# ali-vilab/VGen

Measured on AMD Instinct MI355X. Metric: denoise_steps_per_sec, higher is better.
Workload: dtype fp16

## Files before the change

### include/vgen_hip.h

```cpp
#ifndef VGEN_HIP_H
#define VGEN_HIP_H

#include <stddef.h>
#include <stdint.h>

#ifdef __cplusplus
extern "C" {
#endif

#define VGEN_ABI_VERSION 7

enum { VGEN_BF16 = 0, VGEN_F16 = 1, VGEN_F32 = 2 };

enum {
  VGEN_E_BADARG = -1,
  VGEN_E_UNSUPPORTED = -2,
  VGEN_E_WORKSPACE = -3
};

int vgen_version(void);
const char* vgen_last_error(void);

size_t vgen_groupnorm_ws_bytes(int64_t nb, int64_t S);
int vgen_groupnorm(const float* x1, int32_t C1, const float* x2, int32_t C2,
                   int64_t nb, int64_t S, int32_t groups, float eps,
                   const float* gamma, const float* beta, int32_t silu,
                   void* y, void* raw, int32_t raw_split, int32_t dtype,
                   float* ws, size_t ws_bytes, void* stream);

int vgen_groupnorm_cs(const float* x1, int32_t C1, const float* cs1,
                      const float* x2, int32_t C2, const float* cs2,
                      int64_t nb, int64_t S, int32_t groups, float eps,
                      const float* gamma, const float* beta, int32_t silu,
                      void* y, void* raw, int32_t raw_split, int32_t dtype,
                      float* ws, size_t ws_bytes, void* stream);

int vgen_embed_tokens(const int64_t* tokens, int64_t rows, int32_t L, int32_t d, int32_t vocab,
                      const float* table, const float* pos, float* out, void* stream);

int vgen_layernorm(const float* x, int64_t M, int32_t d, float eps,
                   const float* gamma, const float* beta,
                   void* y, int32_t dtype, void* stream);

enum { VGEN_TAP_LINEAR = 0, VGEN_TAP_CONV3X3 = 1, VGEN_TAP_TEMPORAL3 = 2 };
enum { VGEN_EPI_NONE = 0, VGEN_EPI_GEGLU = 1 };

typedef struct vgen_tapgemm_args {
  int64_t M;
  int32_t N;
  int32_t dtype;
  const void* A;
  int64_t lda;
  int32_t C1;
  int32_t taps;
  int32_t mode;
  int32_t Hi, Wi, Ho, Wo, stride, pad_t, pad_l, ups;
  int32_t F;
  int64_t S;
  const void* A2;
  int64_t lda2;
  int32_t C2;
  const void* W;
  int64_t ldw;
  const float* bias;
  const float* rowbias;
  int64_t rowbias_ld;
  int64_t rows_per_rb;
  const float* residual;
  int64_t ldr;
  void* out;
  int64_t ldo;
  int32_t out_dtype;
  int32_t epilogue;
  void* ws;
  size_t ws_bytes;
  int32_t crop_t;
  float* colstats;
  int32_t dualw;
  int32_t split_out;
} vgen_tapgemm_args;

size_t vgen_tapgemm_ws_bytes(const vgen_tapgemm_args* args);
int vgen_tapgemm(const vgen_tapgemm_args* args, void* stream);

int vgen_tapgemm_query_plan(const vgen_tapgemm_args* args, int32_t* out3);
int vgen_tapgemm_set_plans(const int64_t* rows, int32_t n);

typedef struct vgen_attn_args {
  const void* q;
  const void* k;
  const void* v;
  void* out;
  int32_t dtype;
  int32_t heads;
  int32_t nq, nk;
  int64_t nbatch;
  int64_t inner;
  int64_t q_rs, q_bo, q_bi;
  int64_t k_rs, k_bo, k_bi;
  int64_t v_rs, v_bo, v_bi;
  int64_t o_rs, o_bo, o_bi;
  float scale;
  int32_t causal;
} vgen_attn_args;

int vgen_attention(const vgen_attn_args* args, void* stream);

int vgen_attention_d80(const vgen_attn_args* args, void* stream);

int vgen_softmax_rows(const float* S, int64_t rows, int32_t cols, int64_t lds, float scale,
                      void* P, int64_t ldp, int32_t dtype, void* stream);


int vgen_act_cast(const float* x, void* y, int64_t n, int32_t act, int32_t dtype, void* stream);

int vgen_cast_split(const float* x, int64_t M, int32_t C, int64_t ldx, void* out, int64_t ldo, int32_t lo_off,
                    int32_t dtype, void* stream);

int vgen_timestep_embedding(const float* t, int32_t B, int32_t dim, void* out, int32_t dtype,
                            void* stream);

int vgen_linear_f32(const float* x, int32_t n, int32_t K, const float* W, const float* bias, int32_t N,
                    int32_t act_in, const float* add, float* out, void* stream);

int vgen_im2col3x3_small(const float* src, int64_t nimg, int32_t Fi, int32_t Cin, int32_t H,
                         int32_t W, int64_t s_bo, int64_t s_fi, int64_t s_c, int64_t s_y,
                         int64_t s_x, void* out, int32_t Kpad, int32_t dtype, int32_t split, void* stream);

int vgen_pointwise_small(const float* src, int64_t nimg, int32_t Fi, int32_t Cin, int32_t H,
                         int32_t W, int64_t s_bo, int64_t s_fi, int64_t s_c, int64_t s_y,
                         int64_t s_x, const float* Wm, const float* b, int32_t Cout, float* dst,
                         int64_t d_bo, int64_t d_fi, int64_t d_c, int64_t d_y, int64_t d_x,
                         void* stream);

int vgen_cfg_ddim_step(const float* xt, const float* y, const float* u, const float* noise,
                       const float* coef, float guide, int32_t use_guide, int32_t mean_type,
                       int64_t B, int64_t per_b, float* xt_1, float* x0_out, void* stream);

int vgen_cfg_ddim_step_units(const float* xt, int64_t xt_bstride, const float* y, const float* u,
                             const float* noise, const float* coef, const int64_t* t_idx, float guide,
                             int32_t use_guide, int32_t mean_type, int64_t B, int64_t per_b, float* xt_1,
                             float* x0_out, float* rep, int32_t nrep, int64_t rep_gstride,
                             int64_t rep_bstride, void* stream);

int vgen_gaussian_sample(const float* moments, const float* noise, int64_t nimg, int32_t zc,
                         int64_t HW, float scale, float* z, void* stream);

int vgen_lowfreq_filter(const float* x, int64_t nimg, int32_t H, int32_t W, int32_t C, float scale,
                        float* y, float* ws, size_t ws_bytes, void* stream);
int vgen_scale_channels(float* x, int64_t M, int32_t C, int32_t c0, int32_t c1, float s, void* stream);

int vgen_patchify(const float* x, int64_t B, int32_t C, int32_t H, int32_t W, int32_t P, int32_t Kpad, int32_t cls,
                  void* out, int32_t dtype, void* stream);

int vgen_conv3x3_small(const float* x, int64_t n, int32_t Cin, int32_t H, int32_t W, const float* w,
                       const float* b, int32_t Cout, int32_t stride, int32_t act, float* y, void* stream);
int vgen_adaptive_avgpool2d(const float* x, int64_t planes, int32_t H, int32_t W, int32_t Ho, int32_t Wo,
                            float* y, void* stream);
int vgen_frame_transformer(const float* x, int64_t B, int32_t F, int32_t d, int64_t HW, int32_t heads,
                           int32_t dim_head, int32_t hidden, const float* ln_w, const float* ln_b,
                           const float* wqkv, const float* wout, const float* bout, const float* w1,
                           const float* b1, const float* w2, const float* b2, float* y, int32_t last,
                           float out_scale, int32_t accumulate, void* stream);

int vgen_frames_u8(const float* x, int64_t rows, int32_t C, int64_t ldx, const float* mean,
                   const float* stdv, void* out, void* stream);

int vgen_adapter(const float* x, int64_t ldx, int64_t M, int32_t d, int32_t h, int32_t hp, const void* Wd,
                 const void* Wu, const float* bu, const float* hb, int64_t ldhb, int64_t rows_per_hb, float* out,
                 int64_t ldo, int32_t dtype, void* stream);

int vgen_sketch_stem(const float* x, int64_t n, int32_t H, int32_t W, int32_t flip, float mean, float stdv,
                     const float* w, const float* b, void* out, int64_t ldo, int32_t dtype, void* stream);
int vgen_relu_shuffle16(const void* in, int64_t ldi, int64_t M, int32_t C, int32_t g, int32_t Hin, int32_t Win,
                        void* out, int64_t ldo, int32_t dtype, void* stream);
int vgen_sketch_head(const void* a, int64_t lda, int64_t n, int32_t H, int32_t W, int32_t C, const float* w,
                     float bias, int32_t flip, float* out, int32_t dtype, void* stream);

int vgen_dwconv_relu(const float* x, int64_t ldx, int64_t n, int32_t H, int32_t W, int32_t Cp, const float* w,
                     int32_t k, int32_t pool, float* xp, void* xp16, void* y, int32_t dtype, void* stream);
int vgen_cdcm_head(const void* t, int64_t ldt, int64_t n, int32_t H, int32_t W, const void* Wd, const float* Wa,
                   const float* ba, const float* wr, float* out, int64_t ldo, int32_t dtype, void* stream);
int vgen_pidinet_emap(const float* mr, int64_t ld, int64_t n, int32_t H, int32_t W, const float* w2, float br,
                      float* e, void* stream);
int vgen_pidinet_fuse(const float* e0, const float* e1, const float* e2, const float* e3, int64_t n, int32_t H,
                      int32_t W, float wc0, float wc1, float wc2, float wc3, float bc, float* out, void* stream);

int vgen_repeat_rows(const void* src, int64_t bytes, int32_t G, void* dst, void* stream);
int vgen_gather_rows_f32(const float* table, int64_t nrows_table, int64_t cols, const int64_t* idx, int64_t rows,
                         float* out, void* stream);

size_t vgen_cfg_stats_ws_bytes(int64_t B);
int vgen_cfg_stats(const float* y, const float* u, float guide, int32_t use_guide, int64_t B,
                   int64_t per_b, float* out, void* ws, size_t ws_bytes, void* stream);
int vgen_gauss_x0(const float* xt, const float* out, const void* ws, float rescale, const float* coef,
                  int32_t pred_type, int64_t B, int64_t per_b, float* x0, float* eps, void* stream);
int vgen_lincomb4(const float* a, const float* b, const float* c, const float* d, float ca, float cb,
                  float cc, float cd, float* out, int64_t n, void* stream);
int vgen_dpmpp2m_sde_step(const float* x, const float* denoised, const float* old_denoised, const float* noise,
                          float ca, float cb, float cc, float cn1, float cn2, float cn3, float* out, int64_t n,
                          void* stream);

#ifdef __cplusplus
}
#endif
#endif
```

### vgen_amd/csrc/norms.hip

```cpp
#include "common.h"
#include <stdlib.h>
#include <type_traits>

namespace {

constexpr int GN_THREADS = 256;
constexpr int GN_MAX_SLOTS = 3;
constexpr int GN_G = 32;

struct GnGeom {
  int C, C1, C2;
  int nslots;
  int tpr;
  int rpb;
  int spt;
  int cpg;
};

__device__ __forceinline__ GnGeom gn_geom(int C1, int C2, int groups) {
  GnGeom g;
  g.C1 = C1;
  g.C2 = C2;
  g.C = C1 + C2;
  g.nslots = g.C >> 2;
  if (g.nslots <= GN_THREADS) {
    g.tpr = g.nslots;
    g.rpb = GN_THREADS / g.nslots;
    g.spt = 1;
  } else {
    g.tpr = GN_THREADS;
    g.rpb = 1;
    g.spt = (g.nslots + GN_THREADS - 1) / GN_THREADS;
  }
  g.cpg = g.C / groups;
  return g;
}

__device__ __forceinline__ f32x4 gn_load(const float* x1, const float* x2, const GnGeom& g,
                                         int64_t row, int c) {
  if (c < g.C1) return *(const f32x4*)(x1 + row * g.C1 + c);
  return *(const f32x4*)(x2 + row * g.C2 + (c - g.C1));
}

__global__ __launch_bounds__(GN_THREADS) void gn_stats_kernel(
    const float* __restrict__ x1, int C1, const float* __restrict__ x2, int C2, int64_t S,
    int groups, int nsplit, float* __restrict__ part) {
  __shared__ float red[2][3072];
  const GnGeom g = gn_geom(C1, C2, groups);
  const int tid = threadIdx.x;
  const int split = blockIdx.x;
  const int64_t nb = blockIdx.y;
  const int64_t rows_per = (S + nsplit - 1) / nsplit;
  const int64_t r_begin = (int64_t)split * rows_per;
  const int64_t r_end = min(S, r_begin + rows_per);
  const int nrows = r_end > r_begin ? (int)(r_end - r_begin) : 0;
  const int rowlane = tid / g.tpr;
  const int slot0 = tid - rowlane * g.tpr;

  if (rowlane < g.rpb) {
    const int cnt = nrows > rowlane ? (nrows - rowlane + g.rpb - 1) / g.rpb : 0;
    f32x4 s[GN_MAX_SLOTS], ss[GN_MAX_SLOTS], pv[GN_MAX_SLOTS];
#pragma unroll
    for (int k = 0; k < GN_MAX_SLOTS; ++k) {
      s[k] = f32x4{0, 0, 0, 0};
      ss[k] = f32x4{0, 0, 0, 0};
      pv[k] = f32x4{0, 0, 0, 0};
    }
    bool first = true;
#pragma unroll 4
    for (int64_t r = r_begin + rowlane; r < r_end; r += g.rpb) {
      const int64_t row = nb * S + r;
#pragma unroll
      for (int k = 0; k < GN_MAX_SLOTS; ++k) {
        const int slot = slot0 + k * GN_THREADS;
        if (k < g.spt && slot < g.nslots) {
          const f32x4 x = gn_load(x1, x2, g, row, slot * 4);
          if (first) pv[k] = x;
          const f32x4 v = x - pv[k];
          s[k] += v;
          ss[k] += v * v;
        }
      }
      first = false;
    }
    const float inv = cnt > 0 ? 1.0f / (float)cnt : 0.f;
#pragma unroll
    for (int k = 0; k < GN_MAX_SLOTS; ++k) {
      const int slot = slot0 + k * GN_THREADS;
      if (k < g.spt && slot < g.nslots) {
        const int o = rowlane * g.C + slot * 4;
        const f32x4 dm = s[k] * inv;
        f32x4 m2 = ss[k] - s[k] * dm;
#pragma unroll
        for (int e = 0; e < 4; ++e) m2[e] = fmaxf(m2[e], 0.f);
        *(f32x4*)&red[0][o] = pv[k] + dm;
        *(f32x4*)&red[1][o] = m2;
      }
    }
  }
  __syncthreads();
  if (tid < groups) {
    const float n = (float)nrows * (float)g.cpg;
    float mean = 0.f, m2 = 0.f;
    if (nrows > 0) {
      const float ref = red[0][tid * g.cpg];
      float a = 0.f;
      for (int rl = 0; rl < g.rpb; ++rl) {
        const float cnt = nrows > rl ? (float)((nrows - rl + g.rpb - 1) / g.rpb) : 0.f;
        const int o = rl * g.C + tid * g.cpg;
        float t = 0.f;
        for (int c = 0; c < g.cpg; ++c) t += red[0][o + c] - ref;
        a += cnt * t;
      }
      mean = ref + a / n;
      for (int rl = 0; rl < g.rpb; ++rl) {
        const float cnt = nrows > rl ? (float)((nrows - rl + g.rpb - 1) / g.rpb) : 0.f;
        const int o = rl * g.C + tid * g.cpg;
        float t = 0.f, q = 0.f;
        for (int c = 0; c < g.cpg; ++c) {
          const float d = red[0][o + c] - mean;
          t += d * d;
          q += red[1][o + c];
        }
        m2 += q + cnt * t;
      }
    }
    float* o = part + ((nb * nsplit + split) * groups + tid) * 3;
    o[0] = n;
    o[1] = mean;
    o[2] = m2;
  }
}

__global__ __launch_bounds__(64) void gn_finalize_kernel(const float* __restrict__ part,
                                                         int groups, int nsplit, float eps, int C,
                                                         const float* __restrict__ gamma,
                                                         const float* __restrict__ beta,
                                                         float* __restrict__ stat) {
  const int lane = threadIdx.x;
  const int grp = blockIdx.x;
  const int64_t nb = blockIdx.y;
  float n = 0.f, mean = 0.f, m2 = 0.f;
  for (int sp = lane; sp < nsplit; sp += 64) {
    const float* p = part + ((nb * nsplit + sp) * groups + grp) * 3;
    const float nb_ = p[0], mb = p[1], m2b = p[2];
    if (nb_ > 0.f) {
      const float nt = n + nb_;
      const float d = mb - mean;
      mean += d * (nb_ / nt);
      m2 += m2b + d * d * (n * nb_ / nt);
      n = nt;
    }
  }
#pragma unroll
  for (int o = 1; o < 64; o <<= 1) {
    const float n2 = __shfl_xor(n, o, 64), mean2 = __shfl_xor(mean, o, 64),
                m22 = __shfl_xor(m2, o, 64);
    const float nt = n + n2;
    if (nt > 0.f) {
      const float lo_n = (lane & o) ? n2 : n, hi_n = (lane & o) ? n : n2;
      const float lo_m = (lane & o) ? mean2 : mean, hi_m = (lane & o) ? mean : mean2;
      const float d = hi_m - lo_m;
      const float w = hi_n / nt;
      m2 = m2 + m22 + d * d * (lo_n * w);
      mean = lo_m + d * w;
    }
    n = nt;
  }
  const float rstd = 1.0f / sqrtf((n > 0.f ? m2 / n : 0.f) + eps);
  const int cpg = C / groups;
  for (int j = lane; j < cpg; j += 64) {
    const int c = grp * cpg + j;
    const float a = gamma[c] * rstd;
    stat[(nb * C + c) * 2 + 0] = a;
    stat[(nb * C + c) * 2 + 1] = beta[c] - mean * a;
  }
}

__device__ __forceinline__ void chan_merge(float& n, float& mean, float& m2, float nb_, float mb, float m2b) {
  const float nt = n + nb_;
  if (nt > 0.f) {
    const float d = mb - mean;
    const float w = nb_ / nt;
    m2 = m2 + m2b + d * d * (n * w);
    mean = mean + d * w;
  }
  n = nt;
}

constexpr float GN_CS_GUARD = 128.f;

template <int NT>
__global__ __launch_bounds__(NT) void gn_finalize_cs_kernel(const float* __restrict__ cs1, int C1,
                                                             const float* __restrict__ cs2, int C2,
                                                             const float* __restrict__ x1, const float* __restrict__ x2,
                                                             int64_t S, int groups, float eps,
                                                             const float* __restrict__ gamma,
                                                             const float* __restrict__ beta,
                                                             float* __restrict__ stat) {
  constexpr int NW = NT / 64;
  __shared__ float red[NW][3];
  __shared__ float mr[3];
  const int tid = threadIdx.x, lane = tid & 63, w = tid >> 6;
  const int grp = blockIdx.x;
  const int64_t nb = blockIdx.y;
  const int cpg = (C1 + C2) / groups;
  const int slabs = (int)(S / 64);
  const int items = slabs * cpg;
  const int64_t srow0 = nb * slabs;
  float n = 0.f, mean = 0.f, m2 = 0.f;
  auto fetch = [&](int it, float& sm, float& sq) __attribute__((always_inline)) {
    const int sl = it / cpg;
    const int c = grp * cpg + (it - sl * cpg);
    const int64_t srow = srow0 + sl;
    if (c < C1) {
      sm = cs1[(srow * 2) * C1 + c];
      sq = cs1[(srow * 2 + 1) * C1 + c];
    } else {
      sm = cs2[(srow * 2) * C2 + (c - C1)];
      sq = cs2[(srow * 2 + 1) * C2 + (c - C1)];
    }
  };
  int it = tid;
  for (; it + 3 * NT < items; it += 4 * NT) {
    float sm[4], sq[4];
#pragma unroll
    for (int u = 0; u < 4; ++u) fetch(it + u * NT, sm[u], sq[u]);
#pragma unroll
    for (int u = 0; u < 4; ++u) {
      const float mb = sm[u] * (1.0f / 64.f);
      chan_merge(n, mean, m2, 64.f, mb, fmaxf(sq[u] - sm[u] * mb, 0.f));
    }
  }
  for (; it < items; it += NT) {
    float sm, sq;
    fetch(it, sm, sq);
    const float mb = sm * (1.0f / 64.f);
    chan_merge(n, mean, m2, 64.f, mb, fmaxf(sq - sm * mb, 0.f));
  }
#pragma unroll
  for (int o = 1; o < 64; o <<= 1) {
    const float n2 = __shfl_xor(n, o, 64), mean2 = __shfl_xor(mean, o, 64),
                m22 = __shfl_xor(m2, o, 64);
    const float nt = n + n2;
    if (nt > 0.f) {
      const float lo_n = (lane & o) ? n2 : n, hi_n = (lane & o) ? n : n2;
      const float lo_m = (lane & o) ? mean2 : mean, hi_m = (lane & o) ? mean : mean2;
      const float d = hi_m - lo_m;
      const float wgt = hi_n / nt;
      m2 = m2 + m22 + d * d * (lo_n * wgt);
      mean = lo_m + d * wgt;
    }
    n = nt;
  }
  if (lane == 0) {
    red[w][0] = n;
    red[w][1] = mean;
    red[w][2] = m2;
  }
  __syncthreads();
  if (tid == 0) {
    float N = red[0][0], M = red[0][1], Q = red[0][2];
    for (int k = 1; k < NW; ++k) chan_merge(N, M, Q, red[k][0], red[k][1], red[k][2]);
    const float var = N > 0.f ? Q / N : 0.f;
    mr[0] = M;
    mr[1] = 1.0f / sqrtf(var + eps);
    mr[2] = N * M * M > GN_CS_GUARD * Q ? 1.f : 0.f;
  }
  __syncthreads();
  if (mr[2] != 0.f) {
    const float M = mr[0];
    const int64_t tot = S * cpg;
    float d = 0.f, q = 0.f;
    for (int64_t i = tid; i < tot; i += NT) {
      const int64_t r = i / cpg;
      const int c = grp * cpg + (int)(i - r * cpg);
      const int64_t row = nb * S + r;
      const float e = (c < C1 ? x1[row * C1 + c] : x2[row * C2 + (c - C1)]) - M;
      d += e;
      q += e * e;
    }
#pragma unroll
    for (int o = 1; o < 64; o <<= 1) {
      d += __shfl_xor(d, o, 64);
      q += __shfl_xor(q, o, 64);
    }
    __syncthreads();
    if (lane == 0) {
      red[w][0] = d;
      red[w][1] = q;
    }
    __syncthreads();
    if (tid == 0) {
      float D = red[0][0], Q = red[0][1];
      for (int k = 1; k < NW; ++k) {
        D += red[k][0];
        Q += red[k][1];
      }
      const float nf = (float)tot;
      const float dm = D / nf;
      mr[0] = M + dm;
      mr[1] = 1.0f / sqrtf(fmaxf(Q - D * dm, 0.f) / nf + eps);
    }
    __syncthreads();
  }
  const int C = C1 + C2;
  for (int j = tid; j < cpg; j += NT) {
    const int c = grp * cpg + j;
    const float a = gamma[c] * mr[1];
    stat[(nb * C + c) * 2 + 0] = a;
    stat[(nb * C + c) * 2 + 1] = beta[c] - mr[0] * a;
  }
}

template <typename T>
__device__ __forceinline__ void store_raw4(uint16_t* raw, int64_t off, int raw_lo, const f32x4& v) {
  const u32x2 h = pack4<T>(v.x, v.y, v.z, v.w);
  *(u32x2*)(raw + off) = h;
  if (raw_lo > 0) {
    *(u32x2*)(raw + off + raw_lo) =
        pack4<T>(v.x - T::to_f32((uint16_t)(h.x & 0xffffu)), v.y - T::to_f32((uint16_t)(h.x >> 16)),
                 v.z - T::to_f32((uint16_t)(h.y & 0xffffu)), v.w - T::to_f32((uint16_t)(h.y >> 16)));
  }
}
template <typename T>
__device__ __forceinline__ void store_raw2(uint16_t* raw, int64_t off, int raw_lo, float a, float b) {
  const uint32_t h = T::pack2(a, b);
  *(uint32_t*)(raw + off) = h;
  if (raw_lo > 0) *(uint32_t*)(raw + off + raw_lo) = T::pack2(a - T::to_f32((uint16_t)(h & 0xffffu)), b - T::to_f32((uint16_t)(h >> 16)));
}

template <typename T>
__global__ __launch_bounds__(GN_THREADS) void gn_apply_kernel(
    const float* __restrict__ x1, int C1, const float* __restrict__ x2, int C2, int64_t S,
    int groups, int nsplit, const float* __restrict__ stat, const float* __restrict__ gamma,
    const float* __restrict__ beta, int silu, uint16_t* __restrict__ y,
    uint16_t* __restrict__ raw, int raw_lo) {
  const GnGeom g = gn_geom(C1, C2, groups);
  const int raw_ld = raw_lo > 0 ? 2 * g.C : g.C;
  const int tid = threadIdx.x;
  const int split = blockIdx.x;
  const int64_t nb = blockIdx.y;
  const int64_t rows_per = (S + nsplit - 1) / nsplit;
  const int64_t r_begin = (int64_t)split * rows_per;
  const int64_t r_end = min(S, r_begin + rows_per);
  const int rowlane = tid / g.tpr;
  const int slot0 = tid - rowlane * g.tpr;
  if (rowlane >= g.rpb) return;

  f32x4 sc[GN_MAX_SLOTS], sh[GN_MAX_SLOTS];
#pragma unroll
  for (int k = 0; k < GN_MAX_SLOTS; ++k) {
    const int slot = slot0 + k * GN_THREADS;
    if (k < g.spt && slot < g.nslots) {
      const f32x4 p0 = *(const f32x4*)(stat + (nb * g.C + slot * 4) * 2);
      const f32x4 p1 = *(const f32x4*)(stat + (nb * g.C + slot * 4) * 2 + 4);
      sc[k] = f32x4{p0.x, p0.z, p1.x, p1.z};
      sh[k] = f32x4{p0.y, p0.w, p1.y, p1.w};
    }
  }
  if (g.spt == 1) {
    constexpr int U = 4;
    const int c = slot0 * 4;
    const bool from1 = c < g.C1;
    const float* src = from1 ? x1 + c : x2 + (c - g.C1);
    const int64_t ld = from1 ? g.C1 : g.C2;
    f32x4 cur[U], nxt[U];
    int64_t r = r_begin + rowlane;
    auto load = [&](int64_t r0, f32x4* dst) __attribute__((always_inline)) {
#pragma unroll
      for (int u = 0; u < U; ++u) {
        const int64_t rr = r0 + (int64_t)u * g.rpb;
        const int64_t row = nb * S + (rr < r_end ? rr : r_end - 1);
        dst[u] = *(const f32x4*)(src + row * ld);
      }
    };
    if (r < r_end) load(r, nxt);
    for (; r < r_end; r += (int64_t)U * g.rpb) {
#pragma unroll
      for (int u = 0; u < U; ++u) cur[u] = nxt[u];
      if (r + (int64_t)U * g.rpb < r_end) load(r + (int64_t)U * g.rpb, nxt);
#pragma unroll
      for (int u = 0; u < U; ++u) {
        const int64_t rr = r + (int64_t)u * g.rpb;
        if (rr < r_end) {
          const int64_t row = nb * S + rr;
          f32x4 o = cur[u] * sc[0] + sh[0];
          if (silu) {
#pragma unroll
            for (int e = 0; e < 4; ++e) o[e] = silu_f(o[e]);
          }
          *(u32x2*)(y + row * g.C + c) = pack4<T>(o.x, o.y, o.z, o.w);
          if (raw) store_raw4<T>(raw, row * raw_ld + c, raw_lo, cur[u]);
        }
      }
    }
    return;
  }
#pragma unroll 4
  for (int64_t r = r_begin + rowlane; r < r_end; r += g.rpb) {
    const int64_t row = nb * S + r;
#pragma unroll
    for (int k = 0; k < GN_MAX_SLOTS; ++k) {
      const int slot = slot0 + k * GN_THREADS;
      if (k < g.spt && slot < g.nslots) {
        const f32x4 v = gn_load(x1, x2, g, row, slot * 4);
        f32x4 o = v * sc[k] + sh[k];
        if (silu) {
#pragma unroll
          for (int e = 0; e < 4; ++e) o[e] = silu_f(o[e]);
        }
        *(u32x2*)(y + row * g.C + slot * 4) = pack4<T>(o.x, o.y, o.z, o.w);
        if (raw) store_raw4<T>(raw, row * raw_ld + slot * 4, raw_lo, v);
      }
    }
  }
}

constexpr int GNF_THREADS = 512;
constexpr int GNF_LDS_FLOATS = 24576;

__device__ __forceinline__ float gnf_block_sum(float v, float* red) {
  v = wave_sum(v);
  const int lane = threadIdx.x & 63, w = threadIdx.x >> 6;
  __syncthreads();
  if (lane == 0) red[w] = v;
  __syncthreads();
  float t = 0.f;
#pragma unroll
  for (int i = 0; i < GNF_THREADS / 64; ++i) t += red[i];
  return t;
}

template <typename T>
__global__ __launch_bounds__(GNF_THREADS) void gn_fused_kernel(
    const float* __restrict__ x1, int C1, const float* __restrict__ x2, int C2, int64_t S, int groups,
    float eps, const float* __restrict__ gamma, const float* __restrict__ beta, int silu,
    uint16_t* __restrict__ y, uint16_t* __restrict__ raw, int raw_lo) {
  extern __shared__ __attribute__((aligned(16))) float gnf_stage[];
  __shared__ float red[GNF_THREADS / 64];
  const int C = C1 + C2;
  const int cpg = C / groups;
  const int I = cpg >> 1;
  const int rpi = GNF_THREADS / I;
  const int tid = threadIdx.x;
  const int r0 = tid / I;
  const int i = tid - r0 * I;
  const bool active = r0 < rpi;
  const int c = blockIdx.x * cpg + 2 * i;
  const int64_t row0 = (int64_t)blockIdx.y * S;
  const bool from1 = c < C1;
  const float* src = from1 ? x1 + row0 * C1 + c : x2 + row0 * C2 + (c - C1);
  const int64_t lds = from1 ? C1 : C2;
  const int nit = active ? (int)((S - r0 + rpi - 1) / rpi) : 0;
  f32x2* const st = (f32x2*)gnf_stage + r0 * I + i;
  const int sstep = rpi * I;

  float a = 0.f;
  {
    const float* p = src + (int64_t)r0 * lds;
    const int64_t step = (int64_t)rpi * lds;
#pragma unroll 8
    for (int k = 0; k < nit; ++k) {
      const f32x2 v = *(const f32x2*)(p + k * step);
      st[k * sstep] = v;
      a += v.x + v.y;
    }
  }
  const float n = (float)S * (float)cpg;
  const float mean = gnf_block_sum(a, red) / n;
  float q = 0.f;
  for (int k = 0; k < nit; ++k) {
    const f32x2 v = st[k * sstep];
    const float d0 = v.x - mean, d1 = v.y - mean;
    q += d0 * d0 + d1 * d1;
  }
  const float rstd = 1.0f / sqrtf(gnf_block_sum(q, red) / n + eps);
  if (!active) return;
  const float sc0 = gamma[c] * rstd, sc1 = gamma[c + 1] * rstd;
  const float sh0 = beta[c] - mean * sc0, sh1 = beta[c + 1] - mean * sc1;
  const int raw_ld = raw_lo > 0 ? 2 * C : C;
  uint16_t* yo = y + (row0 + r0) * C + c;
  uint16_t* ro = raw ? raw + (row0 + r0) * raw_ld + c : nullptr;
  const int64_t ostep = (int64_t)rpi * C, rstep = (int64_t)rpi * raw_ld;
#pragma unroll 4
  for (int k = 0; k < nit; ++k) {
    const f32x2 v = st[k * sstep];
    float o0 = v.x * sc0 + sh0, o1 = v.y * sc1 + sh1;
    if (silu) {
      o0 = silu_f(o0);
      o1 = silu_f(o1);
    }
    *(uint32_t*)(yo + k * ostep) = T::pack2(o0, o1);
    if (ro) store_raw2<T>(ro, k * rstep, raw_lo, v.x, v.y);
  }
}

constexpr int GNR_THREADS = 1024;
constexpr int GNR_NIT = 36;

__device__ __forceinline__ float gnr_block_sum(float v, float* red) {
  v = wave_sum(v);
  const int lane = threadIdx.x & 63, w = threadIdx.x >> 6;
  __syncthreads();
  if (lane == 0) red[w] = v;
  __syncthreads();
  float t = 0.f;
#pragma unroll
  for (int i = 0; i < GNR_THREADS / 64; ++i) t += red[i];
  return t;
}

template <typename T>
__global__ __launch_bounds__(GNR_THREADS) void gn_regs_kernel(
    const float* __restrict__ x1, int C1, const float* __restrict__ x2, int C2, int64_t S, int groups,
    float eps, const float* __restrict__ gamma, const float* __restrict__ beta, int silu,
    uint16_t* __restrict__ y, uint16_t* __restrict__ raw, int raw_lo) {
  __shared__ float red[GNR_THREADS / 64];
  const int C = C1 + C2;
  const int cpg = C / groups;
  const int I = cpg >> 1;
  const int rpi = GNR_THREADS / I;
  const int tid = threadIdx.x;
  const int r0 = tid / I;
  const int i = tid - r0 * I;
  const bool active = r0 < rpi;
  const int c = blockIdx.x * cpg + 2 * i;
  const int64_t row0 = (int64_t)blockIdx.y * S;
  const bool from1 = c < C1;
  const float* src = from1 ? x1 + row0 * C1 + c : x2 + row0 * C2 + (c - C1);
  const int64_t lds = from1 ? C1 : C2;
  const int nit = active ? (int)((S - r0 + rpi - 1) / rpi) : 0;

  f32x2 v[GNR_NIT];
  float a = 0.f;
  {
    const float* p = src + (int64_t)r0 * lds;
    const int64_t step = (int64_t)rpi * lds;
#pragma unroll
    for (int k = 0; k < GNR_NIT; ++k) {
      v[k] = f32x2{0.f, 0.f};
      if (k < nit) v[k] = *(const f32x2*)(p + k * step);
    }
#pragma unroll
    for (int k = 0; k < GNR_NIT; ++k) a += v[k].x + v[k].y;
  }
  const float n = (float)S * (float)cpg;
  const float mean = gnr_block_sum(a, red) / n;
  float q = 0.f;
#pragma unroll
  for (int k = 0; k < GNR_NIT; ++k) {
    if (k < nit) {
      const float d0 = v[k].x - mean, d1 = v[k].y - mean;
      q += d0 * d0 + d1 * d1;
    }
  }
  const float rstd = 1.0f / sqrtf(gnr_block_sum(q, red) / n + eps);
  if (!active) return;
  const float sc0 = gamma[c] * rstd, sc1 = gamma[c + 1] * rstd;
  const float sh0 = beta[c] - mean * sc0, sh1 = beta[c + 1] - mean * sc1;
  const int raw_ld = raw_lo > 0 ? 2 * C : C;
  uint16_t* yo = y + (row0 + r0) * C + c;
  uint16_t* ro = raw ? raw + (row0 + r0) * raw_ld + c : nullptr;
  const int64_t ostep = (int64_t)rpi * C, rstep = (int64_t)rpi * raw_ld;
#pragma unroll
  for (int k = 0; k < GNR_NIT; ++k) {
    if (k < nit) {
      float o0 = v[k].x * sc0 + sh0, o1 = v[k].y * sc1 + sh1;
      if (silu) {
        o0 = silu_f(o0);
        o1 = silu_f(o1);
      }
      *(uint32_t*)(yo + k * ostep) = T::pack2(o0, o1);
      if (ro) store_raw2<T>(ro, k * rstep, raw_lo, v[k].x, v[k].y);
    }
  }
}

int gn_nsplit(int64_t nb, int64_t S, int C) {
  int64_t rows = 16384 / C;
  if (rows < 2) rows = 2;
  int64_t ns = (S + rows - 1) / rows;
  const int64_t want = (1024 + nb - 1) / nb;
  if (ns < want) ns = want;
  const int64_t cap = (S + 1) / 2;
  if (ns > cap) ns = cap;
  if (ns < 1) ns = 1;
  if (ns > 1024) ns = 1024;
  return (int)ns;
}

constexpr int LN_MAX_SLOTS = 8;

template <typename T, int LPR>
__global__ __launch_bounds__(256) void layernorm_kernel(const float* __restrict__ x, int64_t M,
                                                        int d, float eps,
                                                        const float* __restrict__ gamma,
                                                        const float* __restrict__ beta,
                                                        void* __restrict__ y) {
  constexpr int RPB = 256 / LPR;
  const int sub = threadIdx.x % LPR;
  const int64_t row = (int64_t)blockIdx.x * RPB + threadIdx.x / LPR;
  const bool live = row < M;
  const int nslots = d >> 2;
  const float* xr = x + (live ? row : 0) * d;
  f32x4 v[LN_MAX_SLOTS];
  float s = 0.f;
#pragma unroll
  for (int k = 0; k < LN_MAX_SLOTS; ++k) {
    const int slot = sub + LPR * k;
    v[k] = f32x4{0, 0, 0, 0};
    if (slot < nslots) {
      v[k] = *(const f32x4*)(xr + slot * 4);
      s += (v[k].x + v[k].y) + (v[k].z + v[k].w);
    }
  }
#pragma unroll
  for (int o = LPR / 2; o > 0; o >>= 1) s += __shfl_xor(s, o, 64);
  const float mean = s / (float)d;
  float q = 0.f;
#pragma unroll
  for (int k = 0; k < LN_MAX_SLOTS; ++k) {
    const int slot = sub + LPR * k;
    if (slot < nslots) {
      const f32x4 c = v[k] - mean;
      q += (c.x * c.x + c.y * c.y) + (c.z * c.z + c.w * c.w);
    }
  }
#pragma unroll
  for (int o = LPR / 2; o > 0; o >>= 1) q += __shfl_xor(q, o, 64);
  const float rstd = 1.0f / sqrtf(q / (float)d + eps);
  if (!live) return;
#pragma unroll
  for (int k = 0; k < LN_MAX_SLOTS; ++k) {
    const int slot = sub + LPR * k;
    if (slot < nslots) {
      const f32x4 ga = *(const f32x4*)(gamma + slot * 4);
      const f32x4 be = *(const f32x4*)(beta + slot * 4);
      const f32x4 o = (v[k] - mean) * rstd * ga + be;
      if constexpr (std::is_same<T, F32Out>::value) {
        *(f32x4*)((float*)y + row * d + slot * 4) = o;
      } else {
        *(u32x2*)((uint16_t*)y + row * d + slot * 4) = pack4<T>(o.x, o.y, o.z, o.w);
      }
    }
  }
}

template <typename T, int LPR, int NS>
__global__ __launch_bounds__(256) void layernorm_stream_kernel(const float* __restrict__ x, int64_t M,
                                                               float eps, const float* __restrict__ gamma,
                                                               const float* __restrict__ beta,
                                                               uint16_t* __restrict__ y) {
  constexpr int RPB = 256 / LPR;
  constexpr int D = NS * 4 * LPR;
  const int sub = threadIdx.x % LPR;
  const int rl = threadIdx.x / LPR;
  const int64_t ngroups = (M + RPB - 1) / RPB;
  f32x4 ga[NS], be[NS], v[NS], nx[NS];
#pragma unroll
  for (int k = 0; k < NS; ++k) {
    ga[k] = *(const f32x4*)(gamma + (sub + LPR * k) * 4);
    be[k] = *(const f32x4*)(beta + (sub + LPR * k) * 4);
  }
  int64_t g = blockIdx.x;
  auto load = [&](int64_t grp, f32x4* dst) __attribute__((always_inline)) {
    const int64_t row = grp * RPB + rl;
    const float* xr = x + (row < M ? row : M - 1) * D;
#pragma unroll
    for (int k = 0; k < NS; ++k) dst[k] = *(const f32x4*)(xr + (sub + LPR * k) * 4);
  };
  if (g < ngroups) load(g, nx);
  for (; g < ngroups; g += gridDim.x) {
#pragma unroll
    for (int k = 0; k < NS; ++k) v[k] = nx[k];
    if (g + gridDim.x < ngroups) load(g + gridDim.x, nx);
    float s = 0.f;
#pragma unroll
    for (int k = 0; k < NS; ++k) s += (v[k].x + v[k].y) + (v[k].z + v[k].w);
#pragma unroll
    for (int o = LPR / 2; o > 0; o >>= 1) s += __shfl_xor(s, o, 64);
    const float mean = s / (float)D;
    float q = 0.f;
#pragma unroll
    for (int k = 0; k < NS; ++k) {
      const f32x4 c = v[k] - mean;
      q += (c.x * c.x + c.y * c.y) + (c.z * c.z + c.w * c.w);
    }
#pragma unroll
    for (int o = LPR / 2; o > 0; o >>= 1) q += __shfl_xor(q, o, 64);
    const float rstd = 1.0f / sqrtf(q / (float)D + eps);
    const int64_t row = g * RPB + rl;
    if (row < M) {
      uint16_t* yr = y + row * D;
#pragma unroll
      for (int k = 0; k < NS; ++k) {
        const f32x4 o = (v[k] - mean) * rstd * ga[k] + be[k];
        *(u32x2*)(yr + (sub + LPR * k) * 4) = pack4<T>(o.x, o.y, o.z, o.w);
      }
    }
  }
}

template <typename T, int LPR, int NS>
void launch_ln_stream(const float* x, int64_t M, float eps, const float* gamma, const float* beta,
                      uint16_t* y, hipStream_t s) {
  const int64_t ngroups = (M + 256 / LPR - 1) / (256 / LPR);
  const int64_t grid = ngroups < 2048 ? ngroups : 2048;
  hipLaunchKernelGGL((layernorm_stream_kernel<T, LPR, NS>), dim3((unsigned)grid), dim3(256), 0, s, x, M, eps,
                     gamma, beta, y);
}

template <typename T, int LPR>
void launch_ln(const float* x, int64_t M, int d, float eps, const float* gamma, const float* beta,
               void* y, hipStream_t s) {
  const int64_t grid = (M + 256 / LPR - 1) / (256 / LPR);
  hipLaunchKernelGGL((layernorm_kernel<T, LPR>), dim3((unsigned)grid), dim3(256), 0, s, x, M, d, eps,
                     gamma, beta, y);
}

template <typename T>
void dispatch_ln(const float* x, int64_t M, int d, float eps, const float* gamma, const float* beta,
                 uint16_t* y, hipStream_t s) {
  switch (d) {
    case 320: return launch_ln_stream<T, 16, 5>(x, M, eps, gamma, beta, y, s);
    case 512: return launch_ln_stream<T, 16, 8>(x, M, eps, gamma, beta, y, s);
    case 640: return launch_ln_stream<T, 32, 5>(x, M, eps, gamma, beta, y, s);
    case 1024: return launch_ln_stream<T, 32, 8>(x, M, eps, gamma, beta, y, s);
    case 1280: return launch_ln_stream<T, 64, 5>(x, M, eps, gamma, beta, y, s);
    case 2048: return launch_ln_stream<T, 64, 8>(x, M, eps, gamma, beta, y, s);
    default: break;
  }
  if (d <= 512) launch_ln<T, 16>(x, M, d, eps, gamma, beta, y, s);
  else if (d <= 1024) launch_ln<T, 32>(x, M, d, eps, gamma, beta, y, s);
  else launch_ln<T, 64>(x, M, d, eps, gamma, beta, y, s);
}

}

extern "C" size_t vgen_groupnorm_ws_bytes(int64_t nb, int64_t S) {
  const int ns = 1024;
  return (size_t)(nb * ns * GN_G * 3 + nb * 3072 * 2) * sizeof(float);
}

static int groupnorm_impl(const float* x1, int32_t C1, const float* cs1, const float* x2, int32_t C2,
                          const float* cs2, int64_t nb, int64_t S, int32_t groups, float eps,
                          const float* gamma, const float* beta, int32_t silu, void* y,
                          void* raw, int32_t raw_split, int32_t dtype, float* ws, size_t ws_bytes,
                          void* stream) {
  const int C = C1 + C2;
  const int raw_lo = (raw != nullptr && raw_split) ? C : 0;
  VGEN_REQUIRE(dtype == VGEN_BF16 || dtype == VGEN_F16, "groupnorm: dtype");
  VGEN_REQUIRE(groups > 0 && groups <= GN_G && C % groups == 0, "groupnorm: C=%d groups=%d", C,
               groups);
  VGEN_REQUIRE(C1 > 0 && C1 % 4 == 0 && C2 >= 0 && C2 % 4 == 0 && C <= 3072,
               "groupnorm: C1=%d C2=%d (need %%4, total <= 3072)", C1, C2);
  VGEN_REQUIRE(C2 == 0 || x2 != nullptr, "groupnorm: x2 null with C2 > 0");
  VGEN_REQUIRE(vgen_aligned16(x1) && vgen_aligned16(x2) && vgen_aligned16(y) &&
                   vgen_aligned16(raw) && vgen_aligned16(ws),
               "groupnorm: alignment");
  VGEN_REQUIRE(nb > 0 && S > 0 && nb <= 65535, "groupnorm: nb=%lld S=%lld", (long long)nb,
               (long long)S);
  if (ws_bytes < vgen_groupnorm_ws_bytes(nb, S)) {
    vgen_set_error("groupnorm: workspace %zu < %zu", ws_bytes, vgen_groupnorm_ws_bytes(nb, S));
    return VGEN_E_WORKSPACE;
  }
  hipStream_t s = (hipStream_t)stream;
  {
    static const int env_max = getenv("VGEN_GN_FUSED_MAX_MB") ? atoi(getenv("VGEN_GN_FUSED_MAX_MB")) : -1;
    const int64_t fused_max = (int64_t)(env_max >= 0 ? env_max : (C / groups >= 16 ? 96 : 24)) << 20;
    const int cpg = C / groups;
    if (nb * S * C * 4 <= fused_max && cpg % 2 == 0 && C1 % 2 == 0 && cpg / 2 <= GNF_THREADS && S * cpg <= GNF_LDS_FLOATS) {
      const size_t lds = (size_t)S * cpg * sizeof(float);
      static bool done_bf16[VGEN_MAX_DEVICES] = {false}, done_f16[VGEN_MAX_DEVICES] = {false};
      if (vgen_lds_optin((const void*)gn_fused_kernel<BF16>, GNF_LDS_FLOATS * 4, done_bf16, "groupnorm") ||
          vgen_lds_optin((const void*)gn_fused_kernel<F16>, GNF_LDS_FLOATS * 4, done_f16, "groupnorm"))
        return VGEN_E_BADARG;
      dim3 fgrid((unsigned)groups, (unsigned)nb);
      if (dtype == VGEN_BF16) {
        hipLaunchKernelGGL(gn_fused_kernel<BF16>, fgrid, dim3(GNF_THREADS), lds, s, x1, C1, x2, C2, S, groups, eps,
                           gamma, beta, silu, (uint16_t*)y, (uint16_t*)raw, raw_lo);
      } else {
        hipLaunchKernelGGL(gn_fused_kernel<F16>, fgrid, dim3(GNF_THREADS), lds, s, x1, C1, x2, C2, S, groups, eps,
                           gamma, beta, silu, (uint16_t*)y, (uint16_t*)raw, raw_lo);
      }
      return vgen_check_launch("gn_fused");
    }
  }
  {
    static const int regs_on = getenv("VGEN_GN_REGS") ? atoi(getenv("VGEN_GN_REGS")) : 1;
    const int cpg = C / groups;
    const int I = cpg / 2;
    if (regs_on && cs1 == nullptr && cpg % 2 == 0 && C1 % 2 == 0 && I > 0 && I <= GNR_THREADS &&
        (S + (GNR_THREADS / I) - 1) / (GNR_THREADS / I) <= GNR_NIT && nb * groups <= 1024 && S * cpg > GNF_LDS_FLOATS) {
      dim3 fgrid((unsigned)groups, (unsigned)nb);
      if (dtype == VGEN_BF16) {
        hipLaunchKernelGGL(gn_regs_kernel<BF16>, fgrid, dim3(GNR_THREADS), 0, s, x1, C1, x2, C2, S, groups, eps, gamma, beta,
                           silu, (uint16_t*)y, (uint16_t*)raw, raw_lo);
      } else {
        hipLaunchKernelGGL(gn_regs_kernel<F16>, fgrid, dim3(GNR_THREADS), 0, s, x1, C1, x2, C2, S, groups, eps, gamma, beta,
                           silu, (uint16_t*)y, (uint16_t*)raw, raw_lo);
      }
      return vgen_check_launch("gn_regs");
    }
  }
  const int nslots = C / 4;
  const int rpb = nslots <= GN_THREADS ? GN_THREADS / nslots : 1;
  VGEN_REQUIRE(rpb * C <= 3072, "groupnorm: internal LDS bound");
  const int ns = gn_nsplit(nb, S, C);
  float* part = ws;
  float* stat = ws + nb * ns * GN_G * 3;
  dim3 grid((unsigned)ns, (unsigned)nb);
  int rc;
  if (cs1 != nullptr) {
    if ((S / 64) * (C / groups) > 2048) {
      hipLaunchKernelGGL(gn_finalize_cs_kernel<1024>, dim3((unsigned)groups, (unsigned)nb), dim3(1024), 0, s, cs1, C1,
                         cs2, C2, x1, x2, S, groups, eps, gamma, beta, stat);
    } else {
      hipLaunchKernelGGL(gn_finalize_cs_kernel<256>, dim3((unsigned)groups, (unsigned)nb), dim3(256), 0, s, cs1, C1,
                         cs2, C2, x1, x2, S, groups, eps, gamma, beta, stat);
    }
    rc = vgen_check_launch("gn_finalize_cs");
    if (rc) return rc;
  } else {
    hipLaunchKernelGGL(gn_stats_kernel, grid, dim3(GN_THREADS), 0, s, x1, C1, x2, C2, S, groups, ns,
                       part);
    rc = vgen_check_launch("gn_stats");
    if (rc) return rc;
    hipLaunchKernelGGL(gn_finalize_kernel, dim3((unsigned)groups, (unsigned)nb), dim3(64), 0, s, part,
                       groups, ns, eps, C, gamma, beta, stat);
    rc = vgen_check_launch("gn_finalize");
    if (rc) return rc;
  }
  if (dtype == VGEN_BF16) {
    hipLaunchKernelGGL(gn_apply_kernel<BF16>, grid, dim3(GN_THREADS), 0, s, x1, C1, x2, C2, S,
                       groups, ns, stat, gamma, beta, silu, (uint16_t*)y, (uint16_t*)raw, raw_lo);
  } else {
    hipLaunchKernelGGL(gn_apply_kernel<F16>, grid, dim3(GN_THREADS), 0, s, x1, C1, x2, C2, S,
                       groups, ns, stat, gamma, beta, silu, (uint16_t*)y, (uint16_t*)raw, raw_lo);
  }
  return vgen_check_launch("gn_apply");
}

extern "C" int vgen_groupnorm(const float* x1, int32_t C1, const float* x2, int32_t C2,
                              int64_t nb, int64_t S, int32_t groups, float eps,
                              const float* gamma, const float* beta, int32_t silu, void* y,
                              void* raw, int32_t raw_split, int32_t dtype, float* ws, size_t ws_bytes,
                              void* stream) {
  return groupnorm_impl(x1, C1, nullptr, x2, C2, nullptr, nb, S, groups, eps, gamma, beta, silu, y, raw, raw_split,
                        dtype, ws, ws_bytes, stream);
}

extern "C" int vgen_groupnorm_cs(const float* x1, int32_t C1, const float* cs1, const float* x2,
                                 int32_t C2, const float* cs2, int64_t nb, int64_t S, int32_t groups,
                                 float eps, const float* gamma, const float* beta, int32_t silu,
                                 void* y, void* raw, int32_t raw_split, int32_t dtype, float* ws, size_t ws_bytes,
                                 void* stream) {
  VGEN_REQUIRE(cs1 != nullptr && (C2 == 0 || cs2 != nullptr), "groupnorm_cs: missing column statistics");
  VGEN_REQUIRE(S % 64 == 0, "groupnorm_cs: S=%lld must be a multiple of the 64-row slab", (long long)S);
  return groupnorm_impl(x1, C1, cs1, x2, C2, cs2, nb, S, groups, eps, gamma, beta, silu, y, raw, raw_split, dtype,
                        ws, ws_bytes, stream);
}

extern "C" int vgen_layernorm(const float* x, int64_t M, int32_t d, float eps, const float* gamma,
                              const float* beta, void* y, int32_t dtype, void* stream) {
  VGEN_REQUIRE(dtype == VGEN_BF16 || dtype == VGEN_F16 || dtype == VGEN_F32, "layernorm: dtype");
  VGEN_REQUIRE(d > 0 && d % 4 == 0 && d <= 64 * 4 * LN_MAX_SLOTS, "layernorm: d=%d", d);
  VGEN_REQUIRE(vgen_aligned16(x) && vgen_aligned16(y) && vgen_aligned16(gamma) &&
                   vgen_aligned16(beta),
               "layernorm: alignment");
  if (M <= 0) return 0;
  VGEN_REQUIRE(M < (1LL << 32), "layernorm: M too large");
  hipStream_t s = (hipStream_t)stream;
  if (dtype == VGEN_F32) {
    if (d <= 512) launch_ln<F32Out, 16>(x, M, d, eps, gamma, beta, y, s);
    else if (d <= 1024) launch_ln<F32Out, 32>(x, M, d, eps, gamma, beta, y, s);
    else launch_ln<F32Out, 64>(x, M, d, eps, gamma, beta, y, s);
    return vgen_check_launch("layernorm");
  }
  if (dtype == VGEN_BF16) dispatch_ln<BF16>(x, M, d, eps, gamma, beta, (uint16_t*)y, s);
  else dispatch_ln<F16>(x, M, d, eps, gamma, beta, (uint16_t*)y, s);
  return vgen_check_launch("layernorm");
}
```

### vgen_amd/csrc/tapgemm.hip

```cpp
#include "common.h"
#include "tapgemm_plan.h"
#include <stdio.h>
#include <stdlib.h>
#include <type_traits>

int vgen_panel_launch(const vgen_tapgemm_args& a, hipStream_t s);

namespace {

struct RowState {
  int base;
  int a;
  int b;
};

constexpr int INVALID = -(1 << 24);

__device__ __attribute__((aligned(128))) unsigned char g_zeros[ZERO_BYTES];

typedef const __attribute__((address_space(1))) void* gptr_t;
typedef __attribute__((address_space(3))) void* lptr_t;


__device__ __forceinline__ void glds16(const void* src, unsigned char* lds_wave_base) {
  __builtin_amdgcn_global_load_lds((gptr_t)src, (lptr_t)lds_wave_base, 16, 0, 0);
}


template <int N>
__device__ __forceinline__ void wait_vmcnt() {
  asm volatile("s_waitcnt vmcnt(%0)" ::"n"(N) : "memory");
}

template <int CPR>
__device__ __forceinline__ int swz_key(int row) {
  if constexpr (CPR == 8) {
    return row & 7;
  } else {
    const int q = (row >> 2) & 3;
    return (4 - q) & 3;
  }
}

#ifdef VGEN_TUNING
#define VGEN_ABLATE_ARG(x) (x)
#else
#define VGEN_ABLATE_ARG(x) 0
#endif

template <typename T, int BM, int BN, int BK, int WM, int WN, int STAGES, bool PP, bool DW>
__global__ __launch_bounds__(WM* WN * 64, (WM * WN == 4) ? 2 : 1) void tapgemm_kernel(
    const vgen_tapgemm_args p, const int splitk, float* __restrict__ ws, const int ablate_arg, const int stagger,
    const int first_round) {
  static_assert(!PP || (WM * WN == 8 && STAGES == 3), "ping-pong needs 8 waves and a 3-stage ring");
  static_assert(!DW || (PP && BK == 64), "dual-W K-steps are built on the ping-pong schedule, 64-element K-tiles");
  const int ablate = VGEN_ABLATE_ARG(ablate_arg);
  constexpr int WPA = DW ? 2 : 1;
  constexpr int NT = WM * WN * 64;
  constexpr int ROW_BYTES = BK * 2;
  constexpr int CPR = ROW_BYTES / 16;
  constexpr int RPI = 64 / CPR;
  constexpr int RPP = NT / CPR;
  constexpr int KS = BK / 32;
  constexpr int WTM = BM / WM, WTN = BN / WN;
  constexpr int MF = WTM / 16, NF = WTN / 16;
  constexpr int RA = BM / RPP;
  constexpr int RBF = BN / RPP;
  constexpr int RBT = BN % RPP;
  constexpr int STAGE_BYTES = (BM + BN) * ROW_BYTES;
  constexpr int LPT = RA + RBF;
  static_assert(BM % RPP == 0 && RBT % RPI == 0, "tile rows must split into whole DMA instructions");

  extern __shared__ __attribute__((aligned(16))) unsigned char smem[];

  const int tid = threadIdx.x;
  const int lane = tid & 63;
  const int wave = __builtin_amdgcn_readfirstlane(tid >> 6);
  const int wm = wave / WN;
  const int wn = wave % WN;
  const int lr = lane & 15;
  const int lq = lane >> 4;
  const bool w_tail = RBT > 0 && wave * RPI < RBT;

  if (stagger > 0 && (int)(blockIdx.x + gridDim.x * blockIdx.y) < first_round && wave == 0) {
    const unsigned hw = __builtin_amdgcn_s_getreg((3 << 11) | ((WM * WN == 8 ? 8 : 0) << 6) | 4);
    if (hw & 1u)
      for (int i = 0; i < stagger; ++i) __builtin_amdgcn_s_sleep(16);
  }

  const int tiles_n = (p.N + BN - 1) / BN;
  int64_t tile;
  {
    const unsigned nwg = gridDim.x, bid = blockIdx.x;
    const unsigned xcd = bid & 7u, q = nwg >> 3, r = nwg & 7u;
    tile = (xcd < r ? xcd * (q + 1) : r * (q + 1) + (xcd - r) * q) + (bid >> 3);
  }
  const int64_t m0 = (tile / tiles_n) * BM;
  const int n0 = (int)(tile % tiles_n) * BN;
  const int64_t lm0 = (ablate & 8) ? 0 : m0;
  const int ln0 = (ablate & 8) ? 0 : n0;

  const uint16_t* __restrict__ A = (const uint16_t*)p.A;
  const uint16_t* __restrict__ A2 = (const uint16_t*)p.A2;
  const uint16_t* __restrict__ W = (const uint16_t*)p.W;
  const int64_t ldw = p.ldw ? p.ldw : ((int64_t)p.taps * p.C1 + p.C2) * WPA;

  const int ld_c = tid % CPR;
  const int ld_r = tid / CPR;

  RowState rs[RA];
  unsigned mvalid = 0;
#pragma unroll
  for (int i = 0; i < RA; ++i) {
    const unsigned m = (unsigned)lm0 + ld_r + RPP * i;
    const bool ok = m < (unsigned)p.M;
    if (ok) mvalid |= 1u << i;
    if (p.mode == VGEN_TAP_CONV3X3) {
      const unsigned hw = p.Ho * p.Wo;
      const unsigned img = m / hw;
      const unsigned rem = m - img * hw;
      const unsigned oy = rem / (unsigned)p.Wo;
      const unsigned ox = rem - oy * p.Wo;
      rs[i].base = img * p.Hi * p.Wi;
      rs[i].a = ok ? (int)oy * p.stride - p.pad_t : INVALID;
      rs[i].b = (int)ox * p.stride - p.pad_l;
    } else if (p.mode == VGEN_TAP_TEMPORAL3) {
      const unsigned fs = m / (unsigned)p.S;
      rs[i].base = (int)m;
      rs[i].a = ok ? (int)(fs % (unsigned)p.F) : INVALID;
      rs[i].b = 0;
    } else {
      rs[i].base = ok ? (int)m : -1;
      rs[i].a = 0;
      rs[i].b = 0;
    }
  }

  const int cpt1 = p.C1 / BK;
  const int T1 = p.taps * cpt1;
  const int KT = T1 + p.C2 / BK;
  const int split = blockIdx.y;
  const int kt_begin = (int)(((int64_t)KT * split) / splitk);
  const int kt_end = (int)(((int64_t)KT * (split + 1)) / splitk);
  const int nk = (ablate & 1) ? 0 : (kt_end - kt_begin) * WPA;

  constexpr int NP = LPT + (RBT > 0 ? 1 : 0);
  const char* pc[NP];
  const char* const zline = (const char*)g_zeros;
  const int src_cb = (ld_c ^ swz_key<CPR>(ld_r)) * 16;
  const int wave_row0 = wave * RPI;
  int kt_next = kt_begin;
  int left;

  const unsigned lda_b = (unsigned)p.lda * 2u, lda2_b = (unsigned)p.lda2 * 2u;
  const char* const zl = zline + src_cb;
  auto gather_a = [&](int kt) __attribute__((always_inline)) {
    if (kt < T1) {
      const int tap = kt / cpt1;
      const int cch = kt - tap * cpt1;
      left = cpt1 - cch;
      const char* const a_cb = (const char*)A + (cch * BK * 2 + src_cb);
      if (p.mode == VGEN_TAP_CONV3X3) {
        const int d0 = tap / 3, d1 = tap - 3 * d0;
        const unsigned Hv = (unsigned)((p.Hi << p.ups) - 2 * p.crop_t), Wv = (unsigned)(p.Wi << p.ups);
#pragma unroll
        for (int i = 0; i < RA; ++i) {
          const int iy = rs[i].a + d0, ix = rs[i].b + d1;
          const bool ok = ((unsigned)iy < Hv) & ((unsigned)ix < Wv);
          const unsigned row = (unsigned)rs[i].base + (unsigned)((iy + p.crop_t) >> p.ups) * (unsigned)p.Wi + (unsigned)(ix >> p.ups);
          const char* const real = a_cb + (uint64_t)row * lda_b;
          pc[i] = ok ? real : zl;
        }
      } else if (p.mode == VGEN_TAP_TEMPORAL3) {
        const int dt_ = tap - 1;
#pragma unroll
        for (int i = 0; i < RA; ++i) {
          const bool ok = (unsigned)(rs[i].a + dt_) < (unsigned)p.F;
          const unsigned row = (unsigned)(rs[i].base + dt_ * p.S);
          const char* const real = a_cb + (uint64_t)row * lda_b;
          pc[i] = ok ? real : zl;
        }
      } else {
#pragma unroll
        for (int i = 0; i < RA; ++i) {
          const bool ok = rs[i].base >= 0;
          const char* const real = a_cb + (uint64_t)(unsigned)rs[i].base * lda_b;
          pc[i] = ok ? real : zl;
        }
      }
    } else {
      left = KT - kt + 1;
      const char* const a_cb = (const char*)A2 + ((kt - T1) * BK * 2 + src_cb);
#pragma unroll
      for (int i = 0; i < RA; ++i) {
        const bool ok = (mvalid >> i) & 1u;
        const char* const real = a_cb + (uint64_t)((unsigned)lm0 + ld_r + RPP * i) * lda2_b;
        pc[i] = ok ? real : zl;
      }
    }
  };
  gather_a(kt_begin);
#pragma unroll
  for (int i = 0; i < NP - RA; ++i) {
    const int n = ln0 + ld_r + RPP * i;
    const bool ok = n < p.N;
    pc[RA + i] = (ok ? (const char*)(W + (int64_t)n * ldw + (int64_t)kt_begin * WPA * BK) : zline) + src_cb;
  }
  auto advance_a = [&]() __attribute__((always_inline)) {
    ++kt_next;
    if (--left == 0) {
      if (kt_next < KT) gather_a(kt_next);
    } else {
#pragma unroll
      for (int i = 0; i < RA; ++i) pc[i] += ROW_BYTES;
    }
  };
  auto advance_w = [&]() __attribute__((always_inline)) {
#pragma unroll
    for (int i = RA; i < NP; ++i) pc[i] += ROW_BYTES;
  };
  auto advance = [&]() __attribute__((always_inline)) {
    advance_a();
    advance_w();
  };
  auto piece_dst = [&](int stage, int j) __attribute__((always_inline)) -> unsigned char* {
    unsigned char* const base = smem + stage * STAGE_BYTES + wave_row0 * ROW_BYTES;
    return j < RA ? base + j * RPP * ROW_BYTES : base + (BM + (j - RA) * RPP) * ROW_BYTES;
  };
  auto dma = [&](int j, int stage) __attribute__((always_inline)) {
    glds16(pc[j], piece_dst(stage, j));
  };
  auto load_tile = [&](int stage) __attribute__((always_inline)) {
#pragma unroll
    for (int j = 0; j < LPT; ++j)
      dma(j, stage);
    if (RBT > 0 && w_tail) dma(NP - 1, stage);
    advance();
  };
  auto load_tile_w = [&](int stage) __attribute__((always_inline)) {
#pragma unroll
    for (int j = RA; j < LPT; ++j) dma(j, stage);
    if (RBT > 0 && w_tail) dma(NP - 1, stage);
    advance_w();
  };

  const bool geglu = p.epilogue == VGEN_EPI_GEGLU;
  const int n_out = geglu ? p.N / 2 : p.N;
  const bool vec = ((n_out & 3) == 0) && ((p.ldo & 3) == 0) &&
                   (p.residual == nullptr || (p.ldr & 3) == 0) &&
                   (p.rowbias == nullptr || (p.rowbias_ld & 3) == 0);
  const bool res_folded = p.residual != nullptr && splitk == 1 && vec && !geglu;
  f32x4 acc[NF][MF];
#pragma unroll
  for (int ni = 0; ni < NF; ++ni)
#pragma unroll
    for (int mi = 0; mi < MF; ++mi) acc[ni][mi] = f32x4{0.f, 0.f, 0.f, 0.f};
  if (res_folded) {
#pragma unroll
    for (int mi = 0; mi < MF; ++mi) {
      const int64_t m = m0 + wm * WTM + mi * 16 + lr;
#pragma unroll
      for (int ni = 0; ni < NF; ++ni) {
        const int n = n0 + wn * WTN + ni * 16 + lq * 4;
        if (m < p.M && n < p.N) acc[ni][mi] = *(const f32x4*)(p.residual + m * p.ldr + n);
      }
    }
  }

  const int rd_row = lr * ROW_BYTES;
  const int sw = swz_key<CPR>(lr);

  constexpr int MH = MF > 4 ? MF / 4 : 1;
  constexpr int MFH = MF / MH;
  u32x4 wf[KS][NF], xf[KS][MFH];
  auto read_w = [&](int stage) __attribute__((always_inline)) {
    const unsigned char* b = smem + stage * STAGE_BYTES + BM * ROW_BYTES + wn * WTN * ROW_BYTES + rd_row;
#pragma unroll
    for (int ks = 0; ks < KS; ++ks) {
      const int co = ((ks * 4 + lq) ^ sw) << 4;
#pragma unroll
      for (int ni = 0; ni < NF; ++ni) wf[ks][ni] = *(const u32x4*)(b + ni * 16 * ROW_BYTES + co);
    }
  };
  auto read_x = [&](int stage, int mh) __attribute__((always_inline)) {
    const unsigned char* a = smem + stage * STAGE_BYTES + (wm * WTM + mh * MFH * 16) * ROW_BYTES + rd_row;
#pragma unroll
    for (int ks = 0; ks < KS; ++ks) {
      const int co = ((ks * 4 + lq) ^ sw) << 4;
#pragma unroll
      for (int mi = 0; mi < MFH; ++mi) xf[ks][mi] = *(const u32x4*)(a + mi * 16 * ROW_BYTES + co);
    }
  };

  auto compute = [&](int stage, auto prefetch_tag, int stage_pf) __attribute__((always_inline)) {
    constexpr bool prefetch = decltype(prefetch_tag)::value;
    constexpr int NMF = KS * NF * MF;
    constexpr int NMH = NMF / MH;
    constexpr int GRP = NMF / NP;
    static_assert(GRP >= 1 && (NMF + GRP - 1) / GRP >= NP, "not enough MFMA groups for the DMA pieces");
    read_w(stage);
    int piece = 0;
#pragma unroll
    for (int mh = 0; mh < MH; ++mh) {
      read_x(stage, mh);
#pragma unroll
      for (int j = 0; j < NMH; ++j) {
        const int i = mh * NMH + j;
        const int ks = j / (NF * MFH), r = j % (NF * MFH), ni = r / MFH, mi = r % MFH;
        if (i % GRP == 0) {
          if (prefetch) {
            if (piece < LPT) {
              dma(piece, stage_pf);
            } else if (RBT > 0 && piece == NP - 1 && w_tail) {
              dma(NP - 1, stage_pf);
            }
          }
          ++piece;
          __builtin_amdgcn_sched_barrier(0);
        }
        acc[ni][mh * MFH + mi] = T::mfma32(wf[ks][ni], xf[ks][mi], acc[ni][mh * MFH + mi]);
      }
      if (MH > 1) __builtin_amdgcn_sched_barrier(0);
    }
    if (prefetch) advance();
  };

  auto read_phase = [&](int stage, auto prefetch_tag, int stage_pf, auto odd_tag) __attribute__((always_inline)) {
    constexpr bool prefetch = decltype(prefetch_tag)::value;
    constexpr bool odd = decltype(odd_tag)::value;
    static_assert(!PP || MH == 1, "ping-pong keeps a whole K-tile of fragments in registers");
    const unsigned char* bw = smem + stage * STAGE_BYTES + BM * ROW_BYTES + wn * WTN * ROW_BYTES + rd_row;
    const unsigned char* bx = smem + stage * STAGE_BYTES + (wm * WTM) * ROW_BYTES + rd_row;
    constexpr int P0 = odd ? RA : 0;
    constexpr int NPI = NP - P0;
    constexpr int NRF = odd ? NF : NF + MF;
    constexpr int NR = KS * NRF;
    constexpr int EVERY = (NR + NPI) / (NPI + 1) > 0 ? (NR + NPI) / (NPI + 1) : 1;
    int piece = P0;
#pragma unroll
    for (int r = 0; r < NR; ++r) {
      const int ks = r / NRF, q = r % NRF;
      const int co = ((ks * 4 + lq) ^ sw) << 4;
      if (q < NF) wf[ks][q] = *(const u32x4*)(bw + q * 16 * ROW_BYTES + co);
      else xf[ks][q - NF] = *(const u32x4*)(bx + (q - NF) * 16 * ROW_BYTES + co);
      if (prefetch && (r % EVERY) == EVERY - 1 && piece < NP) {
        __builtin_amdgcn_sched_barrier(0);
        if (piece < LPT) {
          dma(piece, stage_pf);
        } else if (RBT > 0 && w_tail) {
          dma(NP - 1, stage_pf);
        }
        ++piece;
        __builtin_amdgcn_sched_barrier(0);
      }
    }
    if (prefetch) {
#pragma unroll
      for (int j = 0; j < NP; ++j)
        if (j >= piece) {
          if (j < LPT) {
            dma(j, stage_pf);
          } else if (RBT > 0 && w_tail) {
            dma(NP - 1, stage_pf);
          }
        }
    }
  };
  auto mfma_phase = [&]() __attribute__((always_inline)) {
#pragma unroll
    for (int ks = 0; ks < KS; ++ks)
#pragma unroll
      for (int ni = 0; ni < NF; ++ni)
#pragma unroll
        for (int mi = 0; mi < MF; ++mi) acc[ni][mi] = T::mfma32(wf[ks][ni], xf[ks][mi], acc[ni][mi]);
  };

  constexpr int AHEAD = STAGES - 1;
  if constexpr (DW) {
    if (nk > 0) {
      load_tile(0);
      load_tile_w(1);
    }
  } else {
    for (int i = 0; i < AHEAD; ++i)
      if (nk > i) load_tile(i);
  }
  int st_c = 0, st_l = AHEAD;
  const int nk_main = nk > AHEAD ? nk - AHEAD : 0;
  auto rotate = [&]() __attribute__((always_inline)) {
    st_c = st_c == STAGES - 1 ? 0 : st_c + 1;
    st_l = st_l == STAGES - 1 ? 0 : st_l + 1;
  };
  auto wait_next = [&]() __attribute__((always_inline)) {
    if (w_tail) wait_vmcnt<LPT + 1>();
    else wait_vmcnt<LPT>();
  };
  auto wait_next_w = [&]() __attribute__((always_inline)) {
    if (w_tail) wait_vmcnt<LPT - RA + 1>();
    else wait_vmcnt<LPT - RA>();
  };
  if constexpr (PP && DW) {
    const bool follower = wave >= 4;
    if (nk > 0) {
      wait_next_w();
      __builtin_amdgcn_s_barrier();
      if (follower) __builtin_amdgcn_s_barrier();
      asm volatile("" ::: "memory");
      auto dw_step = [&](auto prefetch_tag, auto odd_tag) __attribute__((always_inline)) {
        constexpr bool pf = decltype(prefetch_tag)::value;
        constexpr bool odd = decltype(odd_tag)::value;
        read_phase(st_c, prefetch_tag, st_l, odd_tag);
        if constexpr (pf) {
          if constexpr (odd) wait_next_w();
          else wait_next();
        } else {
          wait_vmcnt<0>();
        }
        asm volatile("s_waitcnt lgkmcnt(0)" ::: "memory");
        __builtin_amdgcn_s_barrier();
        __builtin_amdgcn_sched_barrier(0);
        mfma_phase();
        __builtin_amdgcn_sched_barrier(0);
        if constexpr (pf) {
          if constexpr (!odd) advance_a();
          advance_w();
        }
        __builtin_amdgcn_s_barrier();
        asm volatile("" ::: "memory");
        rotate();
      };
      for (int it = 0; it + 2 < nk; it += 2) {
        dw_step(std::true_type{}, std::false_type{});
        dw_step(std::true_type{}, std::true_type{});
      }
      dw_step(std::false_type{}, std::false_type{});
      dw_step(std::false_type{}, std::true_type{});
      if (!follower) __builtin_amdgcn_s_barrier();
    }
  } else if constexpr (PP) {
    const bool follower = wave >= 4;
    if (nk > 1) wait_next();
    else wait_vmcnt<0>();
    __builtin_amdgcn_s_barrier();
    if (follower) __builtin_amdgcn_s_barrier();
    asm volatile("" ::: "memory");
    auto pp_step = [&](auto prefetch_tag, bool more) __attribute__((always_inline)) {
      read_phase(st_c, prefetch_tag, st_l, std::false_type{});
      if (more) wait_next();
      else wait_vmcnt<0>();
      asm volatile("s_waitcnt lgkmcnt(0)" ::: "memory");
      __builtin_amdgcn_s_barrier();
      __builtin_amdgcn_sched_barrier(0);
      mfma_phase();
      __builtin_amdgcn_sched_barrier(0);
      if (decltype(prefetch_tag)::value) advance();
      __builtin_amdgcn_s_barrier();
      asm volatile("" ::: "memory");
      rotate();
    };
    for (int it = 0; it < nk_main; ++it) pp_step(std::true_type{}, true);
    for (int it = nk_main; it < nk; ++it) pp_step(std::false_type{}, false);
    if (!follower) __builtin_amdgcn_s_barrier();
  } else {
    for (int it = 0; it < nk_main; ++it) {
      if (STAGES == 3) wait_next();
      else wait_vmcnt<0>();
      __builtin_amdgcn_s_barrier();
      asm volatile("" ::: "memory");
      compute(st_c, std::true_type{}, st_l);
      rotate();
    }
    for (int it = nk_main; it < nk; ++it) {
      if (STAGES == 3 && it + 1 < nk) wait_next();
      else wait_vmcnt<0>();
      __builtin_amdgcn_s_barrier();
      asm volatile("" ::: "memory");
      compute(st_c, std::false_type{}, st_l);
      rotate();
    }
  }

  if (splitk > 1) {
    float* const wsp = ws + (int64_t)split * p.M * p.N;
#pragma unroll
    for (int mi = 0; mi < MF; ++mi) {
      const int64_t m = m0 + wm * WTM + mi * 16 + lr;
      if (m >= p.M) continue;
#pragma unroll
      for (int ni = 0; ni < NF; ++ni) {
        const int n = n0 + wn * WTN + ni * 16 + lq * 4;
        if (n < p.N) *(f32x4*)(wsp + m * p.N + n) = acc[ni][mi];
      }
    }
    return;
  }

  if (ablate & 2) {
    f32x4 t = {0.f, 0.f, 0.f, 0.f};
#pragma unroll
    for (int ni = 0; ni < NF; ++ni)
#pragma unroll
      for (int mi = 0; mi < MF; ++mi) t += acc[ni][mi];
    if (t.x + t.y + t.z + t.w == 1.2345e30f) ((float*)p.out)[0] = t.x;
    return;
  }
  float* const of = (float*)p.out;
  uint16_t* const oh = (uint16_t*)p.out;

  f32x4 bv[NF];
  if (vec || geglu) {
#pragma unroll
    for (int ni = 0; ni < NF; ++ni) {
      const int n = n0 + wn * WTN + ni * 16 + lq * 4;
      bv[ni] = (p.bias && n < p.N) ? *(const f32x4*)(p.bias + n) : f32x4{0.f, 0.f, 0.f, 0.f};
    }
  }
  if (vec && p.out_dtype != VGEN_F32 && (p.ldo & 7) == 0 && (!geglu || NF % 4 == 0) && !(ablate & 4)) {
#pragma unroll
    for (int mi = 0; mi < MF; ++mi) {
      __builtin_amdgcn_sched_barrier(0);
      const int64_t m = m0 + wm * WTM + mi * 16 + lr;
      if (m >= p.M) continue;
      const float* rbp = p.rowbias ? p.rowbias + (m / p.rows_per_rb) * p.rowbias_ld : nullptr;
    auto store_pair16 = [&](int frag0_col, bool pair_ok, const f32x4& va, const f32x4& vb, int64_t m_) __attribute__((always_inline)) {
      u32x2 pa = pack4<T>(va.x, va.y, va.z, va.w);
      u32x2 pb = pack4<T>(vb.x, vb.y, vb.z, vb.w);
      if (pair_ok) {
        const auto sx = __builtin_amdgcn_permlane16_swap(pa.x, pb.x, false, false);
        const auto sy = __builtin_amdgcn_permlane16_swap(pa.y, pb.y, false, false);
        const u32x4 q = {sx[0], sy[0], sx[1], sy[1]};
        *(u32x4*)(oh + m_ * p.ldo + frag0_col + (lq & 1) * 16 + (lq >> 1) * 8) = q;
      } else {
        if (frag0_col + lq * 4 < n_out) *(u32x2*)(oh + m_ * p.ldo + frag0_col + lq * 4) = pa;
        if (frag0_col + 16 + lq * 4 < n_out) *(u32x2*)(oh + m_ * p.ldo + frag0_col + 16 + lq * 4) = pb;
      }
    };
      if (!geglu) {
        auto final_val = [&](int ni) __attribute__((always_inline)) -> f32x4 {
          const int n = n0 + wn * WTN + ni * 16 + lq * 4;
          f32x4 v = acc[ni][mi];
          if (n < p.N) {
            v += bv[ni];
            if (rbp) v += *(const f32x4*)(rbp + n);
            if (p.residual && !res_folded) v += *(const f32x4*)(p.residual + m * p.ldr + n);
          }
          return v;
        };
        auto lo_of = [&](const f32x4& v) __attribute__((always_inline)) -> f32x4 {
          const u32x2 h = pack4<T>(v.x, v.y, v.z, v.w);
          return f32x4{v.x - T::to_f32((uint16_t)(h.x & 0xffffu)), v.y - T::to_f32((uint16_t)(h.x >> 16)),
                       v.z - T::to_f32((uint16_t)(h.y & 0xffffu)), v.w - T::to_f32((uint16_t)(h.y >> 16))};
        };
#pragma unroll
        for (int ni = 0; ni + 1 < NF; ni += 2) {
          const int c0 = n0 + wn * WTN + ni * 16;
          const f32x4 va = final_val(ni), vb = final_val(ni + 1);
          store_pair16(c0, c0 + 32 <= p.N, va, vb, m);
          if (p.split_out) store_pair16(p.N + c0, c0 + 32 <= p.N, lo_of(va), lo_of(vb), m);
        }
        if constexpr (NF % 2 == 1) {
          const int n = n0 + wn * WTN + (NF - 1) * 16 + lq * 4;
          if (n < p.N) {
            const f32x4 v = final_val(NF - 1);
            *(u32x2*)(oh + m * p.ldo + n) = pack4<T>(v.x, v.y, v.z, v.w);
            if (p.split_out) {
              const f32x4 l = lo_of(v);
              *(u32x2*)(oh + m * p.ldo + p.N + n) = pack4<T>(l.x, l.y, l.z, l.w);
            }
          }
        }
      } else if constexpr (NF % 4 == 0) {
        auto gated = [&](int np) __attribute__((always_inline)) -> f32x4 {
          const int pn = n0 + wn * WTN + np * 32 + lq * 4;
          const int j = (n0 + wn * WTN) / 2 + np * 16 + lq * 4;
          f32x4 o = {0.f, 0.f, 0.f, 0.f};
          if (pn < p.N) {
            const f32x4 val = acc[2 * np][mi] + bv[2 * np];
            const f32x4 gat = acc[2 * np + 1][mi] + bv[2 * np + 1];
            o = geglu4(val, gat);
            if (p.residual) o += *(const f32x4*)(p.residual + m * p.ldr + j);
          }
          return o;
        };
#pragma unroll
        for (int np = 0; np < NF / 2; np += 2) {
          const int j0 = (n0 + wn * WTN) / 2 + np * 16;
          store_pair16(j0, j0 + 32 <= n_out, gated(np), gated(np + 1), m);
        }
      }
    }
    return;
  }
  if constexpr (NF > 5) return;
  const bool do_cs = p.colstats != nullptr && vec && !geglu;
  f32x4 cs_s[NF], cs_q[NF];
#pragma unroll
  for (int ni = 0; ni < NF; ++ni) cs_s[ni] = cs_q[ni] = f32x4{0.f, 0.f, 0.f, 0.f};
  if (do_cs) __syncthreads();
  auto flush_cs = [&](int slab) __attribute__((always_inline)) {
    constexpr int NC = NF * 16;
    constexpr int NRES = 2 * NC;
    float* const cb = (float*)smem + wave * (NRES * 16);
    const int64_t srow = (m0 + wm * WTM) / 64 + slab;
    const bool slab_live = srow * 64 < p.M;
#pragma unroll
    for (int ni = 0; ni < NF; ++ni) {
#pragma unroll
      for (int r = 0; r < 4; ++r) {
        const int cw = ni * 16 + lq * 4 + r;
        cb[cw * 16 + lr] = cs_s[ni][r];
        cb[(NC + cw) * 16 + lr] = cs_q[ni][r];
      }
      cs_s[ni] = cs_q[ni] = f32x4{0.f, 0.f, 0.f, 0.f};
    }
    asm volatile("s_waitcnt lgkmcnt(0)" ::: "memory");
#pragma unroll
    for (int res = lane; res < NRES; res += 64) {
      const f32x4* q = (const f32x4*)(cb + res * 16);
      const f32x4 a = q[0], b = q[1], c = q[2], d = q[3];
      const float t = (((a.x + a.y) + (a.z + a.w)) + ((b.x + b.y) + (b.z + b.w))) +
                      (((c.x + c.y) + (c.z + c.w)) + ((d.x + d.y) + (d.z + d.w)));
      const int plane = res >= NC ? 1 : 0;
      const int n = n0 + wn * WTN + (res - plane * NC);
      if (slab_live && n < p.N) p.colstats[(srow * 2 + plane) * (int64_t)p.N + n] = t;
    }
    asm volatile("s_waitcnt lgkmcnt(0)" ::: "memory");
  };
#pragma unroll
  for (int mi = 0; mi < MF; ++mi) {
    __builtin_amdgcn_sched_barrier(0);
    const int64_t m = m0 + wm * WTM + mi * 16 + lr;
    if constexpr (MF % 4 == 0) {
      if (do_cs && mi % 4 == 0 && mi > 0) flush_cs(mi / 4 - 1);
    }
    if (m >= p.M) continue;
    const float* rbp = p.rowbias ? p.rowbias + (m / p.rows_per_rb) * p.rowbias_ld : nullptr;
    if (!geglu) {
#pragma unroll
      for (int ni = 0; ni < NF; ++ni) {
        const int n = n0 + wn * WTN + ni * 16 + lq * 4;
        if (n >= p.N) continue;
        f32x4 v = acc[ni][mi];
        if (vec) {
          v += bv[ni];
          if (rbp) v += *(const f32x4*)(rbp + n);
          if (p.residual && !res_folded) v += *(const f32x4*)(p.residual + m * p.ldr + n);
          if (do_cs) {
            cs_s[ni] += v;
            cs_q[ni] += v * v;
          }
          if (p.out_dtype == VGEN_F32) {
            *(f32x4*)(of + m * p.ldo + n) = v;
          } else {
            *(u32x2*)(oh + m * p.ldo + n) = pack4<T>(v.x, v.y, v.z, v.w);
          }
        } else {
#pragma unroll
          for (int r = 0; r < 4; ++r) {
            if (n + r >= p.N) break;
            float s = v[r];
            if (p.bias) s += p.bias[n + r];
            if (rbp) s += rbp[n + r];
            if (p.residual) s += p.residual[m * p.ldr + n + r];
            if (p.out_dtype == VGEN_F32) of[m * p.ldo + n + r] = s;
            else oh[m * p.ldo + n + r] = T::from_f32(s);
          }
        }
      }
    } else if constexpr (NF % 2 == 0) {
      auto gated = [&](int np) __attribute__((always_inline)) -> f32x4 {
        const int pn = n0 + wn * WTN + np * 32 + lq * 4;
        const int j = (n0 + wn * WTN) / 2 + np * 16 + lq * 4;
        f32x4 o = {0.f, 0.f, 0.f, 0.f};
        if (pn < p.N) {
          const f32x4 val = acc[2 * np][mi] + bv[2 * np];
          const f32x4 gat = acc[2 * np + 1][mi] + bv[2 * np + 1];
          o = geglu4(val, gat);
          if (p.residual) o += *(const f32x4*)(p.residual + m * p.ldr + j);
        }
        return o;
      };
#pragma unroll
      for (int np = 0; np < NF / 2; ++np) {
        const int pn = n0 + wn * WTN + np * 32 + lq * 4;
        if (pn >= p.N) continue;
        const int j = (n0 + wn * WTN) / 2 + np * 16 + lq * 4;
        const f32x4 o = gated(np);
        if (p.out_dtype == VGEN_F32) {
          *(f32x4*)(of + m * p.ldo + j) = o;
        } else {
          *(u32x2*)(oh + m * p.ldo + j) = pack4<T>(o.x, o.y, o.z, o.w);
        }
      }
    }
  }
  if constexpr (MF % 4 == 0) {
    if (do_cs) flush_cs(MF / 4 - 1);
  }
}

template <typename T>
__global__ __launch_bounds__(256) void splitk_reduce_kernel(const vgen_tapgemm_args p, const int splitk,
                                                            const float* __restrict__ ws) {
  const bool geglu = p.epilogue == VGEN_EPI_GEGLU;
  const int n_out = geglu ? p.N / 2 : p.N;
  const int ng = n_out >> 2;
  const int64_t idx = (int64_t)blockIdx.x * 256 + threadIdx.x;
  if (idx >= p.M * ng) return;
  const int64_t m = idx / ng;
  const int j = (int)(idx - m * ng) * 4;
  const int64_t plane = p.M * (int64_t)p.N;
  const int pn = geglu ? 32 * (j >> 4) + (j & 15) : j;
  f32x4 v = {0, 0, 0, 0}, gt = {0, 0, 0, 0};
  for (int s = 0; s < splitk; ++s) {
    v += *(const f32x4*)(ws + s * plane + m * p.N + pn);
    if (geglu) gt += *(const f32x4*)(ws + s * plane + m * p.N + pn + 16);
  }
  if (p.bias) {
    v += *(const f32x4*)(p.bias + pn);
    if (geglu) gt += *(const f32x4*)(p.bias + pn + 16);
  }
  if (geglu) {
#pragma unroll
    for (int r = 0; r < 4; ++r) v[r] = v[r] * gelu_erf_f(gt[r]);
  } else if (p.rowbias) {
    v += *(const f32x4*)(p.rowbias + (m / p.rows_per_rb) * p.rowbias_ld + j);
  }
  if (p.residual) v += *(const f32x4*)(p.residual + m * p.ldr + j);
  if (p.out_dtype == VGEN_F32) *(f32x4*)((float*)p.out + m * p.ldo + j) = v;
  else *(u32x2*)((uint16_t*)p.out + m * p.ldo + j) = pack4<T>(v.x, v.y, v.z, v.w);
}

constexpr int STAGGER_PCT_PP = 50;
constexpr int STAGGER_PCT_DUAL = 50;
constexpr int STAGGER_MIN_ROUNDS = 2;

template <typename T, int S, int BN, bool DW>
int launch(const vgen_tapgemm_args& a, int splitk, hipStream_t stream) {
  constexpr ShapeDesc d = kShapes[S];
  constexpr int BM = d.bm, BK = d.bk, WM = d.wm, WN = d.wn, STAGES = 3;
  constexpr int BPC = d.bpc;
  static_assert(BPC == ((WM * WN == 4) ? 2 : 1), "kShapes' blocks per CU is the kernel's __launch_bounds__ rule");
  const auto kernel = tapgemm_kernel<T, BM, BN, BK, WM, WN, STAGES, d.pp, DW>;
  constexpr size_t lds = (size_t)STAGES * (BM + BN) * BK * 2;
  static bool attr_done[VGEN_MAX_DEVICES] = {false};
  if (const int rc = vgen_lds_optin((const void*)kernel, lds, attr_done, "tapgemm")) return rc;
  const int64_t tiles_m = (a.M + BM - 1) / BM;
  const int64_t tiles_n = (a.N + BN - 1) / BN;
  const int64_t grid = tiles_m * tiles_n;
  if (grid <= 0) return 0;
  if (grid > 0x7fffffffLL) {
    vgen_set_error("tapgemm: grid too large");
    return VGEN_E_BADARG;
  }
  if (splitk > 1 && (a.ws == nullptr || a.ws_bytes < (size_t)splitk * a.M * a.N * sizeof(float)))
    splitk = 1;
#ifdef VGEN_TUNING
  const char* ab = getenv("VGEN_TAPGEMM_ABLATE");
  const int ablate = ab ? atoi(ab) : 0;
#else
  const int ablate = 0;
#endif
  const int cus = vgen_device_cus();
  int stagger = 0;
  {
    int pct = BPC == 1 ? STAGGER_PCT_PP : STAGGER_PCT_DUAL, min_rounds = STAGGER_MIN_ROUNDS;
#ifdef VGEN_TUNING
    if (const char* e = getenv("VGEN_TAPGEMM_STAGGER")) {
      int a1 = 0, a2 = 0, a3 = min_rounds;
      if (sscanf(e, "%d,%d,%d", &a1, &a2, &a3) >= 2) {
        pct = BPC == 1 ? a1 : a2;
        min_rounds = a3;
      }
    }
#endif
    const int64_t blocks = grid * splitk;
    const double rounds = (double)blocks / ((double)cus * BPC);
    if (pct > 0 && rounds >= (double)min_rounds) {
      const int kts = (tap_kt(a) + splitk - 1) / splitk;
      const double tile_us = kts * (a.dualw ? DUALW_KSTEP_FACTOR : 1.0) * (d.stagger_us * BN) + 7.0;
      stagger = (int)(tile_us * pct / 100.0 * 2400.0 / 1024.0 + 0.5);
    }
  }
  hipLaunchKernelGGL(kernel, dim3((unsigned)grid, (unsigned)splitk), dim3(WM * WN * 64), lds, stream, a, splitk, (float*)a.ws,
                     ablate, stagger, cus * BPC);
  int rc = vgen_check_launch("tapgemm");
  if (rc || splitk == 1) return rc;
  const int64_t threads = a.M * (tap_n_out(a) / 4);
  hipLaunchKernelGGL((splitk_reduce_kernel<T>), dim3((unsigned)((threads + 255) / 256)), dim3(256), 0,
                     stream, a, splitk, (const float*)a.ws);
  return vgen_check_launch("tapgemm(splitk reduce)");
}

template <typename T, int S, bool DW>
int launch_bn(const vgen_tapgemm_args& a, const Plan& pl, hipStream_t s) {
  switch (pl.bn) {
    case 128: return launch<T, S, 128, DW>(a, pl.splitk, s);
    case 160: return launch<T, S, 160, DW>(a, pl.splitk, s);
    default: return launch<T, S, 64, DW>(a, pl.splitk, s);
  }
}

template <typename T>
int dispatch(const vgen_tapgemm_args& a, hipStream_t s) {
  const Plan pl = full_plan(a);
  if (pl.shape == SHAPE_PANEL) return vgen_panel_launch(a, s);
  if (a.dualw)
    return pl.shape == SHAPE_PP128 ? launch_bn<T, SHAPE_PP128, true>(a, pl, s) : launch_bn<T, SHAPE_PP, true>(a, pl, s);
  switch (pl.shape) {
    case SHAPE_PP: return launch_bn<T, SHAPE_PP, false>(a, pl, s);
    case SHAPE_PP128: return launch_bn<T, SHAPE_PP128, false>(a, pl, s);
    case SHAPE_PP256: return launch<T, SHAPE_PP256, 256, false>(a, pl.splitk, s);
    case SHAPE_Q128: return launch_bn<T, SHAPE_Q128, false>(a, pl, s);
    default: return launch_bn<T, SHAPE_DUAL, false>(a, pl, s);
  }
}

}

extern "C" int vgen_tapgemm(const vgen_tapgemm_args* args, void* stream) {
  if (!args) {
    vgen_set_error("tapgemm: null args");
    return VGEN_E_BADARG;
  }
  if (const int rc = vgen_tapgemm_validate(*args)) return rc;
  hipStream_t s = (hipStream_t)stream;
  return args->dtype == VGEN_BF16 ? dispatch<BF16>(*args, s) : dispatch<F16>(*args, s);
}
```

### vgen_amd/lib.py

```python
from __future__ import annotations

import ctypes as C
import os

HERE = os.path.dirname(os.path.abspath(__file__))
LIB_PATH = os.environ.get("VGEN_HIP_LIB") or os.path.join(HERE, "libvgen_hip.so")

VGEN_BF16, VGEN_F16, VGEN_F32 = 0, 1, 2
TAP_LINEAR, TAP_CONV3X3, TAP_TEMPORAL3 = 0, 1, 2
EPI_NONE, EPI_GEGLU = 0, 1
ABI_VERSION = 7


class VgenHipError(RuntimeError):
    pass


class TapGemmArgs(C.Structure):
    _fields_ = [
        ("M", C.c_int64), ("N", C.c_int32), ("dtype", C.c_int32),
        ("A", C.c_void_p), ("lda", C.c_int64), ("C1", C.c_int32), ("taps", C.c_int32),
        ("mode", C.c_int32),
        ("Hi", C.c_int32), ("Wi", C.c_int32), ("Ho", C.c_int32), ("Wo", C.c_int32),
        ("stride", C.c_int32), ("pad_t", C.c_int32), ("pad_l", C.c_int32), ("ups", C.c_int32),
        ("F", C.c_int32), ("S", C.c_int64),
        ("A2", C.c_void_p), ("lda2", C.c_int64), ("C2", C.c_int32),
        ("W", C.c_void_p), ("ldw", C.c_int64),
        ("bias", C.c_void_p), ("rowbias", C.c_void_p), ("rowbias_ld", C.c_int64),
        ("rows_per_rb", C.c_int64), ("residual", C.c_void_p), ("ldr", C.c_int64),
        ("out", C.c_void_p), ("ldo", C.c_int64), ("out_dtype", C.c_int32),
        ("epilogue", C.c_int32),
        ("ws", C.c_void_p), ("ws_bytes", C.c_size_t), ("crop_t", C.c_int32),
        ("colstats", C.c_void_p), ("dualw", C.c_int32), ("split_out", C.c_int32),
    ]


class AttnArgs(C.Structure):
    _fields_ = [
        ("q", C.c_void_p), ("k", C.c_void_p), ("v", C.c_void_p), ("out", C.c_void_p),
        ("dtype", C.c_int32), ("heads", C.c_int32), ("nq", C.c_int32), ("nk", C.c_int32),
        ("nbatch", C.c_int64), ("inner", C.c_int64),
        ("q_rs", C.c_int64), ("q_bo", C.c_int64), ("q_bi", C.c_int64),
        ("k_rs", C.c_int64), ("k_bo", C.c_int64), ("k_bi", C.c_int64),
        ("v_rs", C.c_int64), ("v_bo", C.c_int64), ("v_bi", C.c_int64),
        ("o_rs", C.c_int64), ("o_bo", C.c_int64), ("o_bi", C.c_int64),
        ("scale", C.c_float), ("causal", C.c_int32),
    ]


_i32, _i64, _f32, _vp, _sz = C.c_int32, C.c_int64, C.c_float, C.c_void_p, C.c_size_t
SYMBOLS = {
    "vgen_version": (C.c_int, []),
    "vgen_last_error": (C.c_char_p, []),
    "vgen_groupnorm_ws_bytes": (_sz, [_i64, _i64]),
    "vgen_groupnorm": (C.c_int, [_vp, _i32, _vp, _i32, _i64, _i64, _i32, _f32, _vp, _vp, _i32,
                                 _vp, _vp, _i32, _i32, _vp, _sz, _vp]),
    "vgen_groupnorm_cs": (C.c_int, [_vp, _i32, _vp, _vp, _i32, _vp, _i64, _i64, _i32, _f32, _vp, _vp, _i32,
                                    _vp, _vp, _i32, _i32, _vp, _sz, _vp]),
    "vgen_layernorm": (C.c_int, [_vp, _i64, _i32, _f32, _vp, _vp, _vp, _i32, _vp]),
    "vgen_tapgemm_ws_bytes": (_sz, [C.POINTER(TapGemmArgs)]),
    "vgen_tapgemm": (C.c_int, [C.POINTER(TapGemmArgs), _vp]),
    "vgen_tapgemm_query_plan": (C.c_int, [C.POINTER(TapGemmArgs), _vp]),
    "vgen_tapgemm_set_plans": (C.c_int, [_vp, _i32]),
    "vgen_attention": (C.c_int, [C.POINTER(AttnArgs), _vp]),
    "vgen_attention_d80": (C.c_int, [C.POINTER(AttnArgs), _vp]),
    "vgen_softmax_rows": (C.c_int, [_vp, _i64, _i32, _i64, _f32, _vp, _i64, _i32, _vp]),
    "vgen_act_cast": (C.c_int, [_vp, _vp, _i64, _i32, _i32, _vp]),
    "vgen_cast_split": (C.c_int, [_vp, _i64, _i32, _i64, _vp, _i64, _i32, _i32, _vp]),
    "vgen_timestep_embedding": (C.c_int, [_vp, _i32, _i32, _vp, _i32, _vp]),
    "vgen_conv3x3_small": (C.c_int, [_vp, _i64, _i32, _i32, _i32, _vp, _vp, _i32, _i32, _i32, _vp, _vp]),
    "vgen_patchify": (C.c_int, [_vp, _i64, _i32, _i32, _i32, _i32, _i32, _i32, _vp, _i32, _vp]),
    "vgen_adaptive_avgpool2d": (C.c_int, [_vp, _i64, _i32, _i32, _i32, _i32, _vp, _vp]),
    "vgen_frame_transformer": (C.c_int, [_vp, _i64, _i32, _i32, _i64, _i32, _i32, _i32, _vp, _vp, _vp, _vp, _vp, _vp,
                                         _vp, _vp, _vp, _vp, _i32, _f32, _i32, _vp]),
    "vgen_embed_tokens": (C.c_int, [_vp, _i64, _i32, _i32, _i32, _vp, _vp, _vp, _vp]),
    "vgen_linear_f32": (C.c_int, [_vp, _i32, _i32, _vp, _vp, _i32, _i32, _vp, _vp, _vp]),
    "vgen_im2col3x3_small": (C.c_int, [_vp, _i64, _i32, _i32, _i32, _i32, _i64, _i64, _i64, _i64,
                                       _i64, _vp, _i32, _i32, _i32, _vp]),
    "vgen_pointwise_small": (C.c_int, [_vp, _i64, _i32, _i32, _i32, _i32, _i64, _i64, _i64, _i64,
                                       _i64, _vp, _vp, _i32, _vp, _i64, _i64, _i64, _i64, _i64,
                                       _vp]),
    "vgen_cfg_ddim_step_units": (C.c_int, [_vp, _i64, _vp, _vp, _vp, _vp, _vp, _f32, _i32, _i32, _i64, _i64, _vp,
                                           _vp, _vp, _i32, _i64, _i64, _vp]),
    "vgen_cfg_ddim_step": (C.c_int, [_vp, _vp, _vp, _vp, _vp, _f32, _i32, _i32, _i64, _i64, _vp,
                                     _vp, _vp]),
    "vgen_gaussian_sample": (C.c_int, [_vp, _vp, _i64, _i32, _i64, _f32, _vp, _vp]),
    "vgen_lowfreq_filter": (C.c_int, [_vp, _i64, _i32, _i32, _i32, _f32, _vp, _vp, _sz, _vp]),
    "vgen_scale_channels": (C.c_int, [_vp, _i64, _i32, _i32, _i32, _f32, _vp]),
    "vgen_frames_u8": (C.c_int, [_vp, _i64, _i32, _i64, _vp, _vp, _vp, _vp]),
    "vgen_cfg_stats_ws_bytes": (_sz, [_i64]),
    "vgen_cfg_stats": (C.c_int, [_vp, _vp, _f32, _i32, _i64, _i64, _vp, _vp, _sz, _vp]),
    "vgen_gauss_x0": (C.c_int, [_vp, _vp, _vp, _f32, _vp, _i32, _i64, _i64, _vp, _vp, _vp]),
    "vgen_lincomb4": (C.c_int, [_vp, _vp, _vp, _vp, _f32, _f32, _f32, _f32, _vp, _i64, _vp]),
    "vgen_repeat_rows": (C.c_int, [_vp, _i64, _i32, _vp, _vp]),
    "vgen_gather_rows_f32": (C.c_int, [_vp, _i64, _i64, _vp, _i64, _vp, _vp]),
    "vgen_adapter": (C.c_int, [_vp, _i64, _i64, _i32, _i32, _i32, _vp, _vp, _vp, _vp, _i64, _i64, _vp, _i64, _i32, _vp]),
    "vgen_sketch_stem": (C.c_int, [_vp, _i64, _i32, _i32, _i32, _f32, _f32, _vp, _vp, _vp, _i64, _i32, _vp]),
    "vgen_relu_shuffle16": (C.c_int, [_vp, _i64, _i64, _i32, _i32, _i32, _i32, _vp, _i64, _i32, _vp]),
    "vgen_sketch_head": (C.c_int, [_vp, _i64, _i64, _i32, _i32, _i32, _vp, _f32, _i32, _vp, _i32, _vp]),
    "vgen_dwconv_relu": (C.c_int, [_vp, _i64, _i64, _i32, _i32, _i32, _vp, _i32, _i32, _vp, _vp, _vp, _i32, _vp]),
    "vgen_cdcm_head": (C.c_int, [_vp, _i64, _i64, _i32, _i32, _vp, _vp, _vp, _vp, _vp, _i64, _i32, _vp]),
    "vgen_pidinet_emap": (C.c_int, [_vp, _i64, _i64, _i32, _i32, _vp, _f32, _vp, _vp]),
    "vgen_pidinet_fuse": (C.c_int, [_vp, _vp, _vp, _vp, _i64, _i32, _i32, _f32, _f32, _f32, _f32, _f32, _vp, _vp]),
    "vgen_dpmpp2m_sde_step": (C.c_int, [_vp, _vp, _vp, _vp, _f32, _f32, _f32, _f32, _f32, _f32, _vp, _i64, _vp]),
}

_lib = None


def load(path: str | None = None):
    global _lib
    if _lib is not None and path is None:
        return _lib
    p = path or LIB_PATH
    import torch
    if not os.path.exists(p):
        raise VgenHipError(
            f"{p} not found: build it with `python -m vgen_amd.build` (hipcc, gfx950). "
            "There is no CPU fallback for the hot path.")
    try:
        lib = C.CDLL(p)
    except OSError as e:
        raise VgenHipError(f"cannot load {p}: {e}") from e
    for name, (res, args) in SYMBOLS.items():
        try:
            fn = getattr(lib, name)
        except AttributeError as e:
            raise VgenHipError(f"{p} does not export {name}") from e
        fn.restype = res
        fn.argtypes = args
    v = lib.vgen_version()
    if v != ABI_VERSION:
        raise VgenHipError(f"ABI version mismatch: library {v}, binding {ABI_VERSION}")
    _lib = lib
    return lib


def check(rc: int, what: str):
    if rc != 0:
        msg = _lib.vgen_last_error().decode("utf-8", "replace") if _lib is not None else "?"
        raise VgenHipError(f"{what} failed (rc={rc}): {msg}")
```

### vgen_amd/ops.py

```python
from __future__ import annotations

import os

import ctypes as C
from dataclasses import dataclass
from typing import Optional

import torch

from . import lib as _lib

_ENUM = {torch.bfloat16: _lib.VGEN_BF16, torch.float16: _lib.VGEN_F16, torch.float32: _lib.VGEN_F32}


_COLSTATS_ON = os.environ.get("VGEN_COLSTATS", "1") != "0"
COLSTATS_MIN_ROWS = int(os.environ.get("VGEN_COLSTATS_MIN_ROWS", "8192"))
CS_ROWS = 64


def colstats_of(t, rows):
    cs = getattr(t, "vgen_cs", None)
    if cs is None or t.dim() != 2 or not t.is_contiguous():
        return None
    if cs.shape != ((rows + CS_ROWS - 1) // CS_ROWS, 2, t.shape[1]) or t.shape[0] != rows:
        return None
    return cs


def drop_colstats(t):
    if hasattr(t, "vgen_cs"):
        del t.vgen_cs


@dataclass
class TapGemm:
    A: torch.Tensor
    W: torch.Tensor
    M: int
    N: int
    C1: int
    mode: int = _lib.TAP_LINEAR
    taps: int = 1
    Hi: int = 0
    Wi: int = 0
    Ho: int = 0
    Wo: int = 0
    stride: int = 1
    pad_t: int = 1
    pad_l: int = 1
    ups: int = 0
    crop_t: int = 0
    F: int = 0
    S: int = 0
    A2: Optional[torch.Tensor] = None
    C2: int = 0
    bias: Optional[torch.Tensor] = None
    rowbias: Optional[torch.Tensor] = None
    rows_per_rb: int = 0
    residual: Optional[torch.Tensor] = None
    out_dtype: torch.dtype = torch.float32
    epilogue: int = _lib.EPI_NONE
    out: Optional[torch.Tensor] = None
    colstats: bool = False
    split_out: bool = False
    ws: Optional[torch.Tensor] = None
    alg_k: int = 0


@dataclass
class Attn:
    q: torch.Tensor
    k: torch.Tensor
    v: torch.Tensor
    out: torch.Tensor
    heads: int
    nq: int
    nk: int
    nbatch: int
    inner: int
    q_s: tuple
    k_s: tuple
    v_s: tuple
    o_s: tuple
    scale: float
    causal: bool = False


def _ptr(t: Optional[torch.Tensor]):
    return None if t is None else C.c_void_p(t.data_ptr())


def _mat(t: torch.Tensor, name: str):
    if t.dim() != 2 or t.stride(1) != 1:
        raise ValueError(f"{name}: expected a 2-D view with unit inner stride, got {tuple(t.shape)} "
                         f"strides {t.stride()}")
    return t


DW_TILE = 64


def split_weight(p32: torch.Tensor, dt) -> torch.Tensor:
    N, K = p32.shape
    assert K % DW_TILE == 0, f"packed K = {K} must be a multiple of {DW_TILE}"
    hi = p32.to(dt).contiguous()
    lo = (p32.float() - hi.float()).to(dt)
    hi.vgen_dw = torch.stack([hi.view(N, K // DW_TILE, DW_TILE), lo.view(N, K // DW_TILE, DW_TILE)], 2) \
        .reshape(N, 2 * K).contiguous()
    return hi


def dw_terms(dw: torch.Tensor):
    N, K2 = dw.shape
    v = dw.view(N, K2 // (2 * DW_TILE), 2, DW_TILE)
    return v[:, :, 0].reshape(N, K2 // 2), v[:, :, 1].reshape(N, K2 // 2)


class HipBackend:
    name = "hip"

    def __init__(self):
        self.lib = _lib.load()

    @staticmethod
    def _stream(t: torch.Tensor):
        if not t.is_cuda:
            raise _lib.VgenHipError(
                "vgen_amd hot path needs device tensors (got %s); there is no CPU fallback" % t.device)
        return C.c_void_p(torch.cuda.current_stream(t.device).cuda_stream)

    class _Prof:
        def __init__(self, name, work, meta, extra=None):
            self.rec = KERNEL_PROFILE
            self.name, self.work, self.meta, self.extra = name, work, meta, extra

        def __enter__(self):
            if self.rec is not None:
                self.e0 = torch.cuda.Event(enable_timing=True)
                self.e1 = torch.cuda.Event(enable_timing=True)
                self.e0.record()
            return self

        def __exit__(self, *exc):
            if self.rec is not None:
                self.e1.record()
                self.rec.append((self.name, self.e0, self.e1, self.work, self.meta, self.extra))
            return False

    def groupnorm(self, x1, x2, nb, S, groups, eps, gamma, beta, silu, want_raw, dt):
        C1 = x1.shape[1]
        C2 = 0 if x2 is None else x2.shape[1]
        rows = nb * S
        assert x1.dtype == torch.float32 and x1.is_contiguous() and x1.shape[0] == rows
        assert x2 is None or (x2.dtype == torch.float32 and x2.is_contiguous() and x2.shape[0] == rows)
        y = torch.empty((rows, C1 + C2), dtype=dt, device=x1.device)
        rsplit = want_raw == "split"
        raw = (torch.empty((rows, 2 * (C1 + C2)), dtype=dt, device=x1.device) if rsplit else torch.empty_like(y)) if want_raw else None
        nbytes = self.lib.vgen_groupnorm_ws_bytes(nb, S)
        ws = torch.empty((nbytes + 3) // 4, dtype=torch.float32, device=x1.device)
        cs1 = colstats_of(x1, rows)
        cs2 = colstats_of(x2, rows) if x2 is not None else None
        use_cs = S % CS_ROWS == 0 and cs1 is not None and (x2 is None or cs2 is not None)
        nbytes_moved = rows * (C1 + C2) * ((4 if use_cs else 8) + 2 + ((4 if rsplit else 2) if want_raw else 0))
        with self._Prof("groupnorm", nbytes_moved, (nb, S, C1 + C2, int(bool(want_raw)) + int(rsplit))):
            if use_cs:
                rc = self.lib.vgen_groupnorm_cs(_ptr(x1), C1, _ptr(cs1), _ptr(x2), C2, _ptr(cs2), nb, S, groups,
                                                float(eps), _ptr(gamma), _ptr(beta), int(bool(silu)), _ptr(y),
                                                _ptr(raw), int(rsplit), _ENUM[dt], _ptr(ws), nbytes, self._stream(x1))
            else:
                rc = self.lib.vgen_groupnorm(_ptr(x1), C1, _ptr(x2), C2, nb, S, groups, float(eps),
                                             _ptr(gamma), _ptr(beta), int(bool(silu)), _ptr(y), _ptr(raw), int(rsplit),
                                             _ENUM[dt], _ptr(ws), nbytes, self._stream(x1))
        _lib.check(rc, "vgen_groupnorm")
        return y, raw

    def layernorm(self, x, gamma, beta, eps, dt):
        assert x.dtype == torch.float32 and x.is_contiguous() and x.dim() == 2
        y = torch.empty(x.shape, dtype=dt, device=x.device)
        with self._Prof("layernorm", x.numel() * 6, tuple(x.shape)):
            rc = self.lib.vgen_layernorm(_ptr(x), x.shape[0], x.shape[1], float(eps), _ptr(gamma),
                                         _ptr(beta), _ptr(y), _ENUM[dt], self._stream(x))
        _lib.check(rc, "vgen_layernorm")
        return y

    def tapgemm_plan(self, g: TapGemm):
        a = self._tapgemm_args(g, alloc=False)[0]
        pl = (C.c_int32 * 3)()
        _lib.check(self.lib.vgen_tapgemm_query_plan(C.byref(a), pl), "vgen_tapgemm_query_plan")
        return tuple(pl)

    def tapgemm(self, g: TapGemm):
        a, out, cs, A, W, dw, K, n_out, _keep = self._tapgemm_args(g)
        meta = (g.mode, g.M, g.N, K, g.epilogue, str(g.out_dtype) + ("+dw" if dw is not None else ""))
        if KERNEL_PROFILE is not None and PROFILE_PLANS:
            pl = (C.c_int32 * 3)()
            self.lib.vgen_tapgemm_query_plan(C.byref(a), pl)
            flags = (1 if g.residual is not None else 0) | (2 if g.rowbias is not None else 0) | (4 if cs is not None else 0)
            meta = meta + ((g.mode, g.M, g.N, g.C1, g.C2, g.taps, g.epilogue, _ENUM[g.out_dtype], flags), tuple(pl))
        src_rows = A.shape[0] if g.mode != _lib.TAP_LINEAR else g.M
        abytes = (2.0 * src_rows * g.C1 + 2.0 * g.M * g.C2 + 2.0 * g.N * K * (2 if dw is not None else 1) +
                  float(g.M) * n_out * ((4 if g.out_dtype == torch.float32 else 2) + (4 if g.residual is not None else 0)))
        k_alg = g.alg_k or K
        assert 0 < k_alg <= K
        with self._Prof("tapgemm", 2.0 * g.M * g.N * k_alg, meta, (abytes, 2.0 * g.M * g.N * K * (2 if dw is not None else 1))):
            rc = self.lib.vgen_tapgemm(C.byref(a), self._stream(A))
        _lib.check(rc, "vgen_tapgemm")
        if cs is not None:
            out.vgen_cs = cs
        return out

    _PLAN_ONLY = 0x1000

    def _tapgemm_args(self, g: TapGemm, alloc: bool = True):
        A = _mat(g.A, "A")
        dw = getattr(g.W, "vgen_dw", None)
        W = _mat(g.W if dw is None else dw, "W")
        K = g.taps * g.C1 + g.C2
        n_out = g.N // 2 if g.epilogue == _lib.EPI_GEGLU else g.N
        out = g.out
        w_out = 2 * n_out if g.split_out else n_out
        if out is None and alloc:
            out = torch.empty((g.M, w_out), dtype=g.out_dtype, device=A.device)
        if out is not None:
            _mat(out, "out")
            assert out.dtype == g.out_dtype and out.shape[0] == g.M and out.shape[1] >= w_out
        a = _lib.TapGemmArgs()
        a.M, a.N, a.dtype = g.M, g.N, _ENUM[A.dtype]
        a.A, a.lda, a.C1, a.taps, a.mode = A.data_ptr(), A.stride(0), g.C1, g.taps, g.mode
        a.Hi, a.Wi, a.Ho, a.Wo = g.Hi, g.Wi, g.Ho, g.Wo
        a.stride, a.pad_t, a.pad_l, a.ups, a.crop_t = g.stride, g.pad_t, g.pad_l, g.ups, g.crop_t
        a.F, a.S = g.F, g.S
        if g.A2 is not None:
            A2 = _mat(g.A2, "A2")
            assert A2.dtype == A.dtype
            a.A2, a.lda2, a.C2 = A2.data_ptr(), A2.stride(0), g.C2
        assert W.dtype == A.dtype and W.shape[0] >= g.N
        a.W = W.data_ptr()
        if dw is not None:
            assert W.shape[1] == 2 * K, (tuple(W.shape), K)
            a.dualw = 1
        a.ldw = 0 if W.stride(0) == K * (2 if dw is not None else 1) else W.stride(0)
        if g.bias is not None:
            assert g.bias.dtype == torch.float32 and g.bias.is_contiguous()
            a.bias = g.bias.data_ptr()
        if g.rowbias is not None:
            rb = _mat(g.rowbias, "rowbias")
            assert rb.dtype == torch.float32
            a.rowbias, a.rowbias_ld, a.rows_per_rb = rb.data_ptr(), rb.stride(0), g.rows_per_rb
        if g.residual is not None:
            r = _mat(g.residual, "residual")
            assert r.dtype == torch.float32 and r.shape[0] == g.M
            a.residual, a.ldr = r.data_ptr(), r.stride(0)
        a.out, a.ldo = (out.data_ptr(), out.stride(0)) if out is not None else (self._PLAN_ONLY, w_out)
        a.out_dtype, a.epilogue = _ENUM[g.out_dtype], g.epilogue
        a.split_out = int(bool(g.split_out))
        cs = None
        if g.colstats and _COLSTATS_ON:
            if alloc:
                cs = torch.empty(((g.M + CS_ROWS - 1) // CS_ROWS, 2, g.N), dtype=torch.float32, device=A.device)
            a.colstats = cs.data_ptr() if alloc else self._PLAN_ONLY
        need = self.lib.vgen_tapgemm_ws_bytes(C.byref(a))
        ws = g.ws
        if g.ws is not None:
            assert g.ws.is_contiguous() and g.ws.numel() * g.ws.element_size() >= need
            a.ws, a.ws_bytes = g.ws.data_ptr(), g.ws.numel() * g.ws.element_size()
        elif need:
            if alloc:
                ws = torch.empty(need // 4, dtype=torch.float32, device=A.device)
            a.ws, a.ws_bytes = (ws.data_ptr() if alloc else self._PLAN_ONLY), need
        return a, out, cs, A, W, dw, K, n_out, ws

    def attention(self, g: Attn):
        a = _lib.AttnArgs()
        a.q, a.k, a.v, a.out = g.q.data_ptr(), g.k.data_ptr(), g.v.data_ptr(), g.out.data_ptr()
        a.dtype, a.heads, a.nq, a.nk = _ENUM[g.q.dtype], g.heads, g.nq, g.nk
        a.nbatch, a.inner = g.nbatch, g.inner
        a.q_rs, a.q_bo, a.q_bi = g.q_s
        a.k_rs, a.k_bo, a.k_bi = g.k_s
        a.v_rs, a.v_bo, a.v_bi = g.v_s
        a.o_rs, a.o_bo, a.o_bi = g.o_s
        a.scale = float(g.scale)
        a.causal = int(bool(g.causal))
        with self._Prof("attention", 4.0 * g.nbatch * g.heads * g.nq * g.nk * 64,
                        (g.nbatch, g.heads, g.nq, g.nk)):
            rc = self.lib.vgen_attention(C.byref(a), self._stream(g.q))
        _lib.check(rc, "vgen_attention")
        return g.out

    def attention_d80(self, g: Attn):
        a = _lib.AttnArgs()
        a.q, a.k, a.v, a.out = g.q.data_ptr(), g.k.data_ptr(), g.v.data_ptr(), g.out.data_ptr()
        a.dtype, a.heads, a.nq, a.nk = _ENUM[g.q.dtype], g.heads, g.nq, g.nk
        a.nbatch, a.inner = g.nbatch, g.inner
        a.q_rs, a.q_bo, a.q_bi = g.q_s
        a.k_rs, a.k_bo, a.k_bi = g.k_s
        a.v_rs, a.v_bo, a.v_bi = g.v_s
        a.o_rs, a.o_bo, a.o_bi = g.o_s
        a.scale = float(g.scale)
        a.causal = int(bool(g.causal))
        with self._Prof("attention_d80", 4.0 * g.nbatch * g.heads * g.nq * g.nk * 80,
                        (g.nbatch, g.heads, g.nq, g.nk)):
            rc = self.lib.vgen_attention_d80(C.byref(a), self._stream(g.q))
        _lib.check(rc, "vgen_attention_d80")
        return g.out

    def softmax_rows(self, S, cols, scale, dt, out=None):
        S = _mat(S, "S")
        rows = S.shape[0]
        if out is None:
            out = torch.empty((rows, cols), dtype=dt, device=S.device)
        _mat(out, "P")
        rc = self.lib.vgen_softmax_rows(_ptr(S), rows, cols, S.stride(0), float(scale), _ptr(out),
                                        out.stride(0), _ENUM[dt], self._stream(S))
        _lib.check(rc, "vgen_softmax_rows")
        return out

    def act_cast(self, x, act, dt):
        assert x.dtype == torch.float32 and x.is_contiguous()
        y = torch.empty(x.shape, dtype=dt, device=x.device)
        with self._Prof("act_cast", x.numel() * 6, (x.numel(),)):
            rc = self.lib.vgen_act_cast(_ptr(x), _ptr(y), x.numel(), int(act), _ENUM[dt], self._stream(x))
        _lib.check(rc, "vgen_act_cast")
        return y

    def cast_split(self, x, dt, out=None, col=0, lo_off=None):
        assert x.dtype == torch.float32 and x.dim() == 2 and x.stride(1) == 1
        M, Cc = x.shape
        lo_off = Cc if lo_off is None else lo_off
        if out is None:
            out = torch.empty((M, col + lo_off + Cc), dtype=dt, device=x.device)
        _mat(out, "out")
        assert out.dtype == dt and out.shape[0] == M and out.shape[1] >= col + lo_off + Cc
        rc = self.lib.vgen_cast_split(_ptr(x), M, Cc, x.stride(0), C.c_void_p(out.data_ptr() + 2 * col), out.stride(0),
                                      int(lo_off), _ENUM[dt], self._stream(x))
        _lib.check(rc, "vgen_cast_split")
        return out

    def adapter(self, x, Wd, Wu, bu, hb, rows_per_hb, h, out=None):
        x = _mat(x, "x")
        hb = _mat(hb, "hb")
        M, d = x.shape
        hp = Wd.shape[0]
        assert x.dtype == torch.float32 and hb.dtype == torch.float32 and bu.dtype == torch.float32 and bu.is_contiguous()
        assert Wd.dtype == Wu.dtype and Wd.is_contiguous() and Wu.is_contiguous()
        assert Wd.shape == (hp, d) and Wu.shape == (d, hp) and bu.shape == (d,) and hb.shape[1] == hp
        assert hb.shape[0] * int(rows_per_hb) >= M, (tuple(hb.shape), rows_per_hb, M)
        if out is None:
            out = torch.empty((M, d), dtype=torch.float32, device=x.device)
        _mat(out, "out")
        assert out.dtype == torch.float32 and out.shape == (M, d)
        with self._Prof("adapter", 4.0 * M * d * hp, (M, d, hp), (8.0 * M * d + 4.0 * d * hp, 4.0 * M * d * hp)):
            rc = self.lib.vgen_adapter(_ptr(x), x.stride(0), M, d, int(h), hp, _ptr(Wd), _ptr(Wu), _ptr(bu), _ptr(hb),
                                       hb.stride(0), int(rows_per_hb), _ptr(out), out.stride(0), _ENUM[Wd.dtype],
                                       self._stream(x))
        _lib.check(rc, "vgen_adapter")
        return out

    def sketch_stem(self, x, flip, mean, std, w, b, dt):
        assert x.dtype == torch.float32 and x.is_contiguous() and x.dim() == 4 and x.shape[1] == 1
        assert w.dtype == torch.float32 and w.is_contiguous() and w.shape == (25, 64)
        assert b.dtype == torch.float32 and b.is_contiguous() and b.shape == (64,)
        n, _, H, W = x.shape
        out = torch.empty((n * (H // 2) * (W // 2), 64), dtype=dt, device=x.device)
        with self._Prof("sketch_stem", 4.0 * x.numel() + 2.0 * out.numel(), (n, H, W)):
            rc = self.lib.vgen_sketch_stem(_ptr(x), n, H, W, int(bool(flip)), float(mean), float(std), _ptr(w), _ptr(b),
                                           _ptr(out), out.stride(0), _ENUM[dt], self._stream(x))
        _lib.check(rc, "vgen_sketch_stem")
        return out

    def relu_shuffle16(self, a, C, g=1, Hin=0, Win=0, out=None):
        a = _mat(a, "a")
        M = a.shape[0]
        assert a.dtype in (torch.float16, torch.bfloat16) and a.shape[1] >= g * g * C
        if out is None:
            out = a if g == 1 else torch.empty((M * g * g, C), dtype=a.dtype, device=a.device)
        _mat(out, "out")
        assert out.dtype == a.dtype and out.shape[0] == M * g * g and out.shape[1] >= C
        with self._Prof("relu_shuffle16", 4.0 * M * g * g * C, (M, C, g)):
            rc = self.lib.vgen_relu_shuffle16(_ptr(a), a.stride(0), M, int(C), int(g), int(Hin), int(Win), _ptr(out),
                                              out.stride(0), _ENUM[a.dtype], self._stream(a))
        _lib.check(rc, "vgen_relu_shuffle16")
        return out

    def sketch_head(self, a, n, H, W, C, w, bias, flip):
        a = _mat(a, "a")
        assert a.dtype in (torch.float16, torch.bfloat16) and a.shape[0] == n * H * W and a.shape[1] >= C
        assert w.dtype == torch.float32 and w.is_contiguous() and w.shape == (9, C)
        out = torch.empty((n, 1, H, W), dtype=torch.float32, device=a.device)
        with self._Prof("sketch_head", 2.0 * a.shape[0] * C * 9 + 4.0 * out.numel(), (n, H, W, C)):
            rc = self.lib.vgen_sketch_head(_ptr(a), a.stride(0), n, H, W, int(C), _ptr(w), float(bias), int(bool(flip)),
                                           _ptr(out), _ENUM[a.dtype], self._stream(a))
        _lib.check(rc, "vgen_sketch_head")
        return out

    def dwconv_relu(self, x, n, H, W, w, k, dt, pool=False):
        x = _mat(x, "x")
        Cp = x.shape[1]
        assert x.dtype == torch.float32 and x.shape[0] == n * H * W
        assert (w is None) == (k == 1) and (w is None or (w.dtype == torch.float32 and w.is_contiguous() and w.shape == (k * k, Cp)))
        M = n * (H // 2) * (W // 2) if pool else n * H * W
        y = torch.empty((M, Cp), dtype=dt, device=x.device)
        xp = torch.empty((M, Cp), dtype=torch.float32, device=x.device) if pool else None
        xp16 = torch.empty((M, Cp), dtype=dt, device=x.device) if pool else None
        nbytes = 4.0 * x.numel() + 2.0 * y.numel() + (10.0 * M * Cp if pool else 0.0)
        with self._Prof("dwconv_relu", nbytes, (n, H, W, Cp, k, int(bool(pool)))):
            rc = self.lib.vgen_dwconv_relu(_ptr(x), x.stride(0), n, H, W, Cp, _ptr(w), int(k), int(bool(pool)), _ptr(xp),
                                           _ptr(xp16), _ptr(y), _ENUM[dt], self._stream(x))
        _lib.check(rc, "vgen_dwconv_relu")
        return (xp, xp16, y) if pool else y

    def cdcm_head(self, t, n, H, W, Wd, Wa, ba, wr, out=None):
        t = _mat(t, "t")
        assert t.dtype in (torch.float16, torch.bfloat16) and t.shape[0] == n * H * W and t.shape[1] >= 32
        assert Wd.dtype == t.dtype and Wd.is_contiguous() and Wd.shape == (4, 9, 32, 32)
        assert Wa.dtype == torch.float32 and Wa.is_contiguous() and Wa.shape == (4, 32)
        assert ba.dtype == torch.float32 and ba.shape == (4,) and wr.dtype == torch.float32 and wr.shape == (32,)
        if out is None:
            out = torch.empty((n * H * W, 8), dtype=torch.float32, device=t.device)
        _mat(out, "out")
        assert out.dtype == torch.float32 and out.shape[0] == n * H * W and out.shape[1] >= 5
        with self._Prof("cdcm_head", 2.0 * n * H * W * 36 * 32 * 32, (n, H, W)):
            rc = self.lib.vgen_cdcm_head(_ptr(t), t.stride(0), n, H, W, _ptr(Wd), _ptr(Wa), _ptr(ba), _ptr(wr), _ptr(out),
                                         out.stride(0), _ENUM[t.dtype], self._stream(t))
        _lib.check(rc, "vgen_cdcm_head")
        return out

    def pidinet_emap(self, mr, n, H, W, w2, br):
        mr = _mat(mr, "mr")
        assert mr.dtype == torch.float32 and mr.shape[0] == n * H * W and mr.shape[1] >= 5
        assert w2.dtype == torch.float32 and w2.is_contiguous() and w2.shape == (9, 4)
        e = torch.empty((n, H, W), dtype=torch.float32, device=mr.device)
        rc = self.lib.vgen_pidinet_emap(_ptr(mr), mr.stride(0), n, H, W, _ptr(w2), float(br), _ptr(e), self._stream(mr))
        _lib.check(rc, "vgen_pidinet_emap")
        return e

    def pidinet_fuse(self, es, n, H, W, wc, bc):
        assert len(es) == 4 and len(wc) == 4
        for i, e in enumerate(es):
            assert e.dtype == torch.float32 and e.is_contiguous() and tuple(e.shape) == (n, H >> i, W >> i), (i, tuple(e.shape))
        out = torch.empty((n, 1, H, W), dtype=torch.float32, device=es[0].device)
        rc = self.lib.vgen_pidinet_fuse(_ptr(es[0]), _ptr(es[1]), _ptr(es[2]), _ptr(es[3]), n, H, W, float(wc[0]),
                                        float(wc[1]), float(wc[2]), float(wc[3]), float(bc), _ptr(out), self._stream(es[0]))
        _lib.check(rc, "vgen_pidinet_fuse")
        return out

    def conv3x3_small(self, x, w, b, stride=1, act=0):
        assert x.dtype == torch.float32 and x.is_contiguous() and x.dim() == 4
        assert w.dtype == torch.float32 and w.is_contiguous() and w.shape[1] == x.shape[1] and tuple(w.shape[2:]) == (3, 3)
        n, cin, H, W = x.shape
        cout = w.shape[0]
        Ho, Wo = (H + 2 - 3) // stride + 1, (W + 2 - 3) // stride + 1
        y = torch.empty((n, cout, Ho, Wo), dtype=torch.float32, device=x.device)
        rc = self.lib.vgen_conv3x3_small(_ptr(x), n, cin, H, W, _ptr(w), _ptr(b), cout, int(stride), int(act), _ptr(y),
                                         self._stream(x))
        _lib.check(rc, "vgen_conv3x3_small")
        return y

    def patchify(self, x, P, Kpad, cls, dt):
        assert x.dtype == torch.float32 and x.is_contiguous() and x.dim() == 4
        B, Cin, H, W = x.shape
        out = torch.empty((B * (int(cls) + (H // P) * (W // P)), Kpad), dtype=dt, device=x.device)
        rc = self.lib.vgen_patchify(_ptr(x), B, Cin, H, W, int(P), int(Kpad), int(cls), _ptr(out), _ENUM[dt],
                                    self._stream(x))
        _lib.check(rc, "vgen_patchify")
        return out

    def adaptive_avgpool2d(self, x, Ho, Wo):
        assert x.dtype == torch.float32 and x.is_contiguous() and x.dim() == 4
        n, c, H, W = x.shape
        y = torch.empty((n, c, Ho, Wo), dtype=torch.float32, device=x.device)
        rc = self.lib.vgen_adaptive_avgpool2d(_ptr(x), n * c, H, W, int(Ho), int(Wo), _ptr(y), self._stream(x))
        _lib.check(rc, "vgen_adaptive_avgpool2d")
        return y

    def frame_transformer(self, x, B, F, d, HW, p, out=None, last=False, out_scale=1.0, accumulate=False):
        assert x.dtype == torch.float32 and x.is_contiguous() and x.numel() == B * F * d * HW
        if out is None:
            out = torch.empty_like(x) if not last else torch.empty((B * d * F * HW,), dtype=torch.float32, device=x.device)
        assert out.dtype == torch.float32 and out.is_contiguous() and out.numel() == x.numel()
        for k in ("ln_w", "ln_b", "wqkv", "wout", "bout", "w1", "b1", "w2", "b2"):
            assert p[k] is None or (p[k].dtype == torch.float32 and p[k].is_contiguous()), k
        rc = self.lib.vgen_frame_transformer(_ptr(x), B, F, d, HW, p["heads"], p["dim_head"], p["hidden"], _ptr(p["ln_w"]),
                                             _ptr(p["ln_b"]), _ptr(p["wqkv"]), _ptr(p["wout"]), _ptr(p["bout"]),
                                             _ptr(p["w1"]), _ptr(p["b1"]), _ptr(p["w2"]), _ptr(p["b2"]), _ptr(out),
                                             int(bool(last)), float(out_scale), int(bool(accumulate)), self._stream(x))
        _lib.check(rc, "vgen_frame_transformer")
        return out

    def embed_tokens(self, tokens, table, pos):
        assert tokens.dtype == torch.int64 and tokens.is_contiguous() and tokens.dim() == 2
        assert table.dtype == torch.float32 and table.is_contiguous() and pos.dtype == torch.float32 and pos.is_contiguous()
        B, Lk = tokens.shape
        d = table.shape[1]
        assert pos.shape == (Lk, d)
        out = torch.empty((B * Lk, d), dtype=torch.float32, device=table.device)
        rc = self.lib.vgen_embed_tokens(_ptr(tokens), B * Lk, Lk, d, table.shape[0], _ptr(table), _ptr(pos), _ptr(out),
                                        self._stream(table))
        _lib.check(rc, "vgen_embed_tokens")
        return out

    def linear_f32(self, x, W, b, act_in=0, add=None):
        for t in (x, W, b, add):
            assert t is None or (t.dtype == torch.float32 and t.is_contiguous())
        n, K = x.shape
        N = W.shape[0]
        assert W.shape[1] == K and (add is None or add.shape == (n, N))
        out = torch.empty((n, N), dtype=torch.float32, device=x.device)
        rc = self.lib.vgen_linear_f32(_ptr(x), n, K, _ptr(W), _ptr(b), N, int(act_in), _ptr(add), _ptr(out),
                                      self._stream(x))
        _lib.check(rc, "vgen_linear_f32")
        return out

    def timestep_embedding(self, t, dim, dt):
        assert t.dtype == torch.float32 and t.is_contiguous() and t.dim() == 1
        out = torch.empty((t.shape[0], dim), dtype=dt, device=t.device)
        rc = self.lib.vgen_timestep_embedding(_ptr(t), t.shape[0], dim, _ptr(out), _ENUM[dt],
                                              self._stream(t))
        _lib.check(rc, "vgen_timestep_embedding")
        return out

    def im2col3x3_small(self, src, nimg, Fi, Cin, H, W, strides, Kpad, dt, split=False):
        assert src.dtype == torch.float32
        out = torch.empty((nimg * H * W, Kpad), dtype=dt, device=src.device)
        rc = self.lib.vgen_im2col3x3_small(_ptr(src), nimg, Fi, Cin, H, W, *strides, _ptr(out), Kpad,
                                           _ENUM[dt], int(bool(split)), self._stream(src))
        _lib.check(rc, "vgen_im2col3x3_small")
        return out

    def pointwise_small(self, src, nimg, Fi, Cin, H, W, s_strides, Wm, b, Cout, dst, d_strides):
        assert src.dtype == torch.float32 and dst.dtype == torch.float32
        assert Wm.dtype == torch.float32 and Wm.is_contiguous()
        rc = self.lib.vgen_pointwise_small(_ptr(src), nimg, Fi, Cin, H, W, *s_strides, _ptr(Wm),
                                           _ptr(b), Cout, _ptr(dst), *d_strides, self._stream(src))
        _lib.check(rc, "vgen_pointwise_small")
        return dst

    def cfg_ddim_step(self, xt, y, u, noise, coef, guide, use_guide, mean_type, want_x0):
        for t in (xt, y, u, noise, coef):
            assert t is None or (t.dtype == torch.float32 and t.is_contiguous())
        B = xt.shape[0]
        per_b = xt.numel() // B
        out = torch.empty_like(xt)
        x0 = torch.empty_like(xt) if want_x0 else None
        rc = self.lib.vgen_cfg_ddim_step(_ptr(xt), _ptr(y), _ptr(u), _ptr(noise), _ptr(coef),
                                         float(guide), int(use_guide), int(mean_type), B, per_b,
                                         _ptr(out), _ptr(x0), self._stream(xt))
        _lib.check(rc, "vgen_cfg_ddim_step")
        return out, x0

    def ddim_update_units(self, x_units, G, B, C_lat, y, u, noise, coef_tab, t_idx, guide, use_guide, mean_type,
                          xt_1, x0, replicate=True):
        assert x_units.dtype == torch.float32 and x_units.is_contiguous() and x_units.shape[0] == G * B
        unit = x_units[0].numel()
        per_b = C_lat * x_units[0, 0].numel()
        for t in (y, u, noise, xt_1, x0):
            assert t is None or (t.dtype == torch.float32 and t.is_contiguous() and t.numel() == B * per_b)
        assert coef_tab.dtype == torch.float32 and coef_tab.is_contiguous() and coef_tab.shape[-1] == 7
        assert t_idx is None or (t_idx.dtype == torch.int64 and t_idx.is_contiguous() and t_idx.numel() == B)
        rc = self.lib.vgen_cfg_ddim_step_units(
            _ptr(x_units), unit, _ptr(y), _ptr(u), _ptr(noise), _ptr(coef_tab), _ptr(t_idx), float(guide),
            int(use_guide), int(mean_type), B, per_b, _ptr(xt_1), _ptr(x0),
            _ptr(x_units) if replicate else None, G if replicate else 0, B * unit, unit, self._stream(x_units))
        _lib.check(rc, "vgen_cfg_ddim_step_units")
        return xt_1, x0

    def ddim_update_strided(self, xt_rows, y, u, coef_tab, t_idx, guide, use_guide, mean_type, out_rows=None, x0_out=None,
                            rep_units=None, G=0, C_lat=0):
        B = xt_rows.shape[0]
        per_b = xt_rows[0].numel()
        assert xt_rows.dtype == torch.float32 and xt_rows[0].is_contiguous()
        for t_ in (y, u, x0_out):
            assert t_ is None or (t_.dtype == torch.float32 and t_.is_contiguous() and t_.numel() == B * per_b)
        assert coef_tab.dtype == torch.float32 and coef_tab.is_contiguous() and coef_tab.shape[-1] == 7
        assert t_idx.dtype == torch.int64 and t_idx.is_contiguous() and t_idx.numel() == B
        assert (out_rows is None) != (rep_units is None)
        if out_rows is not None:
            assert out_rows.dtype == torch.float32 and out_rows.shape[0] == B and out_rows[0].is_contiguous()
            rep, nrep, gs, bs = out_rows, 1, 0, (out_rows.stride(0) if B > 1 else per_b)
        else:
            assert rep_units.dtype == torch.float32 and rep_units.is_contiguous() and rep_units.shape[0] == G * B
            assert C_lat * rep_units[0, 0].numel() == per_b
            unit = rep_units[0].numel()
            rep, nrep, gs, bs = rep_units, G, B * unit, unit
        rc = self.lib.vgen_cfg_ddim_step_units(
            _ptr(xt_rows), xt_rows.stride(0) if B > 1 else per_b, _ptr(y), _ptr(u), None, _ptr(coef_tab), _ptr(t_idx),
            float(guide), int(use_guide), int(mean_type), B, per_b, None, _ptr(x0_out), _ptr(rep), nrep, gs, bs,
            self._stream(xt_rows))
        _lib.check(rc, "vgen_cfg_ddim_step_units")

    def lowfreq_filter(self, x, nimg, H, W, scale):
        assert x.dtype == torch.float32 and x.is_contiguous() and x.shape[0] == nimg * H * W
        C_ = x.shape[1]
        y = torch.empty_like(x)
        ws = torch.empty(7 * nimg * C_, dtype=torch.float32, device=x.device)
        rc = self.lib.vgen_lowfreq_filter(_ptr(x), nimg, H, W, C_, float(scale), _ptr(y), _ptr(ws), ws.numel() * 4,
                                          self._stream(x))
        _lib.check(rc, "vgen_lowfreq_filter")
        return y

    def scale_channels(self, x, c0, c1, s):
        assert x.dtype == torch.float32 and x.is_contiguous() and x.dim() == 2
        rc = self.lib.vgen_scale_channels(_ptr(x), x.shape[0], x.shape[1], c0, c1, float(s), self._stream(x))
        _lib.check(rc, "vgen_scale_channels")
        drop_colstats(x)
        return x

    def frames_u8(self, x, mean, std):
        x = _mat(x, "x")
        assert x.dtype == torch.float32 and mean.dtype == torch.float32 and std.dtype == torch.float32
        out = torch.empty((x.shape[0], x.shape[1]), dtype=torch.uint8, device=x.device)
        rc = self.lib.vgen_frames_u8(_ptr(x), x.shape[0], x.shape[1], x.stride(0), _ptr(mean), _ptr(std), _ptr(out),
                                     self._stream(x))
        _lib.check(rc, "vgen_frames_u8")
        return out

    def gauss_denoise(self, xt, y, u, guide, rescale, coef, pred_type, want_eps):
        for t in (xt, y, u, coef):
            assert t is None or (t.dtype == torch.float32 and t.is_contiguous())
        B = xt.shape[0]
        per_b = xt.numel() // B
        out = torch.empty_like(xt)
        nbytes = self.lib.vgen_cfg_stats_ws_bytes(B)
        ws = torch.empty(nbytes // 8, dtype=torch.float64, device=xt.device)
        st = self._stream(xt)
        rc = self.lib.vgen_cfg_stats(_ptr(y), _ptr(u), float(guide), int(u is not None), B, per_b, _ptr(out),
                                     _ptr(ws), nbytes, st)
        _lib.check(rc, "vgen_cfg_stats")
        x0 = torch.empty_like(xt)
        eps = torch.empty_like(xt) if want_eps else None
        rc = self.lib.vgen_gauss_x0(_ptr(xt), _ptr(out), _ptr(ws), -1.0 if rescale is None else float(rescale),
                                    _ptr(coef), int(pred_type), B, per_b, _ptr(x0), _ptr(eps), st)
        _lib.check(rc, "vgen_gauss_x0")
        return x0, eps

    def lincomb4(self, a, b, c, d, ca, cb, cc, cd):
        for t in (a, b, c, d):
            assert t is None or (t.dtype == torch.float32 and t.is_contiguous())
        out = torch.empty_like(a)
        rc = self.lib.vgen_lincomb4(_ptr(a), _ptr(b), _ptr(c), _ptr(d), float(ca), float(cb), float(cc), float(cd),
                                    _ptr(out), a.numel(), self._stream(a))
        _lib.check(rc, "vgen_lincomb4")
        return out

    def repeat_rows(self, t, G):
        assert t.is_contiguous() and (t.numel() * t.element_size()) % 16 == 0
        out = torch.empty((G * t.shape[0],) + tuple(t.shape[1:]), dtype=t.dtype, device=t.device)
        rc = self.lib.vgen_repeat_rows(_ptr(t), t.numel() * t.element_size(), int(G), _ptr(out), self._stream(t))
        _lib.check(rc, "vgen_repeat_rows")
        return out

    def gather_rows_f32(self, table, idx):
        assert table.dtype == torch.float32 and table.is_contiguous() and table.dim() == 2
        assert idx.dtype == torch.int64 and idx.is_contiguous() and idx.dim() == 1
        out = torch.empty((idx.shape[0], table.shape[1]), dtype=torch.float32, device=table.device)
        rc = self.lib.vgen_gather_rows_f32(_ptr(table), table.shape[0], table.shape[1], _ptr(idx), idx.shape[0],
                                           _ptr(out), self._stream(table))
        _lib.check(rc, "vgen_gather_rows_f32")
        return out

    def dpmpp2m_sde_step(self, x, denoised, old, noise, ca, cb, cc, cn):
        cn1, cn2, cn3 = cn
        for t in (x, denoised, old, noise):
            assert t is None or (t.dtype == torch.float32 and t.is_contiguous())
        out = torch.empty_like(x)
        rc = self.lib.vgen_dpmpp2m_sde_step(_ptr(x), _ptr(denoised), _ptr(old), _ptr(noise), float(ca), float(cb),
                                            float(cc), float(cn1), float(cn2), float(cn3), _ptr(out), x.numel(),
                                            self._stream(x))
        _lib.check(rc, "vgen_dpmpp2m_sde_step")
        return out

    def gaussian_sample(self, moments, noise, nimg, zc, HW, scale):
        assert moments.dtype == torch.float32 and moments.is_contiguous()
        assert noise.dtype == torch.float32 and noise.is_contiguous()
        z = torch.empty_like(noise)
        rc = self.lib.vgen_gaussian_sample(_ptr(moments), _ptr(noise), nimg, zc, HW, float(scale),
                                           _ptr(z), self._stream(moments))
        _lib.check(rc, "vgen_gaussian_sample")
        return z


_backend = None
KERNEL_PROFILE = None
PROFILE_PLANS = False


def backend():
    global _backend
    if _backend is None:
        _backend = HipBackend()
    return _backend


def set_backend(b):
    global _backend
    prev = _backend
    _backend = b
    return prev


def sixteen(dt) -> torch.dtype:
    if dt in (torch.bfloat16, "bf16", "bfloat16", None):
        return torch.bfloat16
    if dt in (torch.float16, "fp16", "f16", "float16", "half"):
        return torch.float16
    raise ValueError(f"compute dtype must be bf16 or fp16, got {dt}")
```

### vgen_amd/unet.py

```python
from __future__ import annotations

import os

import torch
import torch.nn as nn

from . import lib as L
from . import ops
from .ops import Attn, TapGemm

HEAD_DIM = 64


def _seq(*mods):
    return nn.Sequential(*[m if m is not None else nn.Identity() for m in mods])


class _TemporalConvP(nn.Module):
    def __init__(self, dim):
        super().__init__()
        self.conv1 = _seq(nn.GroupNorm(32, dim), None, nn.Conv3d(dim, dim, (3, 1, 1), padding=(1, 0, 0)))
        for i in (2, 3, 4):
            setattr(self, f"conv{i}", _seq(nn.GroupNorm(32, dim), None, None,
                                           nn.Conv3d(dim, dim, (3, 1, 1), padding=(1, 0, 0))))
        nn.init.zeros_(self.conv4[-1].weight)
        nn.init.zeros_(self.conv4[-1].bias)


class _ResBlockP(nn.Module):
    def __init__(self, cin, emb, cout):
        super().__init__()
        self.cin, self.cout = cin, cout
        self.in_layers = _seq(nn.GroupNorm(32, cin), None, nn.Conv2d(cin, cout, 3, padding=1))
        self.emb_layers = _seq(None, nn.Linear(emb, cout))
        self.out_layers = _seq(nn.GroupNorm(32, cout), None, None, nn.Conv2d(cout, cout, 3, padding=1))
        for p in self.out_layers[3].parameters():
            nn.init.zeros_(p)
        self.skip_connection = nn.Identity() if cin == cout else nn.Conv2d(cin, cout, 1)
        self.temopral_conv = _TemporalConvP(cout)


class _AttnP(nn.Module):
    def __init__(self, qdim, ctx_dim, heads):
        super().__init__()
        inner = heads * HEAD_DIM
        self.heads = heads
        self.to_q = nn.Linear(qdim, inner, bias=False)
        self.to_k = nn.Linear(ctx_dim or qdim, inner, bias=False)
        self.to_v = nn.Linear(ctx_dim or qdim, inner, bias=False)
        self.to_out = _seq(nn.Linear(inner, qdim), None)


class _GEGLUP(nn.Module):
    def __init__(self, d, inner):
        super().__init__()
        self.proj = nn.Linear(d, inner * 2)


class _FFP(nn.Module):
    def __init__(self, d):
        super().__init__()
        self.net = _seq(_GEGLUP(d, 4 * d), None, nn.Linear(4 * d, d))


class _TBlockP(nn.Module):
    def __init__(self, d, heads, ctx_dim):
        super().__init__()
        self.attn1 = _AttnP(d, None, heads)
        self.ff = _FFP(d)
        self.attn2 = _AttnP(d, ctx_dim, heads)
        self.norm1, self.norm2, self.norm3 = nn.LayerNorm(d), nn.LayerNorm(d), nn.LayerNorm(d)


class _SpatialTransformerP(nn.Module):
    def __init__(self, c, heads, ctx_dim):
        super().__init__()
        inner = heads * HEAD_DIM
        self.c, self.inner, self.heads = c, inner, heads
        self.norm = nn.GroupNorm(32, c, eps=1e-6)
        self.proj_in = nn.Linear(c, inner)
        self.transformer_blocks = nn.ModuleList([_TBlockP(inner, heads, ctx_dim)])
        self.proj_out = nn.Linear(c, inner)
        for p in self.proj_out.parameters():
            nn.init.zeros_(p)


class _TemporalTransformerP(nn.Module):
    def __init__(self, c, heads):
        super().__init__()
        inner = heads * HEAD_DIM
        self.c, self.inner, self.heads = c, inner, heads
        self.norm = nn.GroupNorm(32, c, eps=1e-6)
        self.proj_in = nn.Conv1d(c, inner, 1)
        self.transformer_blocks = nn.ModuleList([_TBlockP(inner, heads, None)])
        self.proj_out = nn.Conv1d(inner, c, 1)
        for p in self.proj_out.parameters():
            nn.init.zeros_(p)


class _DownP(nn.Module):
    def __init__(self, c, padding=1):
        super().__init__()
        self.pad = (padding, padding) if isinstance(padding, int) else tuple(padding)
        self.op = nn.Conv2d(c, c, 3, stride=2, padding=padding)


class _UpP(nn.Module):
    def __init__(self, c, crop=0):
        super().__init__()
        self.crop = crop
        self.conv = nn.Conv2d(c, c, 3, padding=1)


def _w16(p32: torch.Tensor, dt, split: bool) -> torch.Tensor:
    if split:
        return ops.split_weight(p32.float(), dt)
    return p32.to(dt).contiguous()


def _w16_cat(parts, dt, split: bool) -> torch.Tensor:
    return _w16(torch.cat([p.float() for p in parts], 1), dt, split)


def rows_conv3x3(w: torch.Tensor) -> torch.Tensor:
    return w.detach().permute(0, 2, 3, 1).reshape(w.shape[0], -1)


def rows_linear(w: torch.Tensor) -> torch.Tensor:
    return w.detach().reshape(w.shape[0], -1)


def pack_conv3x3(w: torch.Tensor, dt, split: bool) -> torch.Tensor:
    return _w16(rows_conv3x3(w), dt, split)


def pack_temporal(w: torch.Tensor, dt, split: bool) -> torch.Tensor:
    return _w16(w.detach()[:, :, :, 0, 0].permute(0, 2, 1).reshape(w.shape[0], -1), dt, split)


def pack_linear(w: torch.Tensor, dt, split: bool) -> torch.Tensor:
    return _w16(rows_linear(w), dt, split)


def pack_geglu(w: torch.Tensor, b: torch.Tensor, dt, split: bool):
    inner = w.shape[0] // 2
    assert inner % 16 == 0
    idx = torch.arange(inner, device=w.device).view(-1, 16)
    perm = torch.cat([idx, idx + inner], dim=1).reshape(-1)
    return _w16(w.detach()[perm], dt, split), b.detach()[perm].float().contiguous()


def pack_small_conv3x3(w: torch.Tensor, kpad: int, dt, split: bool = False) -> torch.Tensor:
    p = w.detach().float().permute(0, 2, 3, 1).reshape(w.shape[0], -1)
    out = torch.zeros((w.shape[0], kpad), dtype=dt, device=w.device)
    k = p.shape[1]
    hi = p.to(dt)
    out[:, :k] = hi
    if split:
        out[:, k: 2 * k] = hi
        out[:, 2 * k: 3 * k] = (p - hi.float()).to(dt)
    return out


def _f32(t):
    return t.detach().float().contiguous()


def resolve_precision(precision, calibration):
    mode, tables = precision or "mixed", {}
    if mode.startswith("mixed:"):
        import re
        spec = mode.split(":", 1)[1]
        if spec.endswith(":all") or spec == "all":
            tables.update(MIXED_SINGLE_KINDS=(), MIXED_EXTRA_KINDS={})
            spec = spec[:-4] if spec.endswith(":all") else "e0d0"
        elif spec.endswith(":noextra") or spec == "noextra":
            tables.update(MIXED_EXTRA_KINDS={})
            spec = spec[:-8] if spec.endswith(":noextra") else "e0d0"
        assert re.fullmatch(r"(?:[edmt]\d*)*", spec), f"precision={mode!r}"
        lv = {"e": (), "d": (), "m": (), "t": ()}
        for side, digits in re.findall(r"([edmt])(\d*)", spec):
            lv[side] = tuple(int(c) for c in digits)
        tables["MIXED_LEVELS"] = {"enc": lv["e"], "mid": lv["m"], "dec": lv["d"], "tx": lv["t"]}
        mode = "mixed"
    auto = None
    if isinstance(calibration, str) and (calibration == "auto" or calibration.startswith("auto:")):
        if mode != "calibrated":
            raise ValueError("calibration='auto' is only meaningful with precision='calibrated'")
        auto, calibration, mode = calibration[5:] or True, None, "high"
    if mode == "calibrated" and not calibration:
        raise ValueError("precision='calibrated' needs calibration=<file written by vgen_amd.calibrate.save_calibrated>; "
                         "to calibrate a model, build it with precision='high' and call calibrate_single_pass")
    if calibration and mode != "calibrated":
        raise ValueError(f"calibration={calibration!r} is only meaningful with precision='calibrated'")
    assert mode in ("fast", "high", "mixed", "calibrated")
    return mode, tables, calibration, auto


class UNetSD_T2VBase(nn.Module):
    _down_padding = 1
    _up_crop = 0
    @staticmethod
    def _extra_stem_channels(kwargs):
        return 0

    _freeu = None

    def __init__(self, config=None, in_dim=4, dim=512, y_dim=512, context_dim=512, hist_dim=156,
                 dim_condition=4, out_dim=6, num_tokens=4, dim_mult=[1, 2, 3, 4], num_heads=None,
                 head_dim=64, num_res_blocks=3, attn_scales=[1 / 2, 1 / 4, 1 / 8],
                 use_scale_shift_norm=True, dropout=0.1, temporal_attn_times=1,
                 temporal_attention=True, use_checkpoint=False, use_image_dataset=False,
                 use_sim_mask=False, training=True, inpainting=True, use_fps_condition=False,
                 p_all_zero=0.1, p_all_keep=0.1, zero_y=None, adapter_transformer_layers=1,
                 compute_dtype=None, precision=None, **kwargs):
        super().__init__()
        if head_dim != HEAD_DIM:
            raise NotImplementedError("vgen_amd attention kernels are built for head_dim 64")
        if not temporal_attention:
            raise NotImplementedError("temporal_attention=False is not on the t2v path")
        if use_image_dataset:
            raise NotImplementedError("use_image_dataset=True is a training-only switch")
        embed_dim = dim * 4
        num_heads = num_heads if num_heads else dim // 32
        self.zero_y = zero_y
        self.in_dim, self.dim, self.y_dim, self.context_dim = in_dim, dim, y_dim, context_dim
        self.embed_dim, self.out_dim, self.dim_mult = embed_dim, out_dim, list(dim_mult)
        self.num_heads, self.head_dim, self.num_res_blocks = num_heads, head_dim, num_res_blocks
        self.attn_scales = list(attn_scales)
        self.use_fps_condition = use_fps_condition
        self.compute_dtype = ops.sixteen(compute_dtype)
        mode, tables, self.calibration, self._auto_cal_cfg = resolve_precision(precision, kwargs.pop("calibration", None))
        self.precision, self._auto_cal = mode, self._auto_cal_cfg
        for k, v in tables.items():
            setattr(self, k, v)
        self._asplit = self.precision != "fast"

        enc_dims = [dim * u for u in [1] + list(dim_mult)]
        dec_dims = [dim * u for u in [dim_mult[-1]] + list(dim_mult)[::-1]]
        shortcut_dims = []
        scale = 1.0

        self.time_embed = _seq(nn.Linear(dim, embed_dim), None, nn.Linear(embed_dim, embed_dim))
        if use_fps_condition:
            self.fps_embedding = _seq(nn.Linear(dim, embed_dim), None, nn.Linear(embed_dim, embed_dim))
            nn.init.zeros_(self.fps_embedding[-1].weight)
            nn.init.zeros_(self.fps_embedding[-1].bias)

        self.input_blocks = nn.ModuleList()
        self.input_blocks.append(nn.ModuleList([nn.Conv2d(in_dim + self._extra_stem_channels(kwargs), dim, 3, padding=1),
                                                _TemporalTransformerP(dim, num_heads)]))
        shortcut_dims.append(dim)
        for i, (cin, cout) in enumerate(zip(enc_dims[:-1], enc_dims[1:])):
            for j in range(num_res_blocks):
                block = nn.ModuleList([_ResBlockP(cin, embed_dim, cout)])
                if scale in self.attn_scales:
                    block.append(_SpatialTransformerP(cout, cout // head_dim, context_dim))
                    block.append(_TemporalTransformerP(cout, cout // head_dim))
                cin = cout
                self.input_blocks.append(block)
                shortcut_dims.append(cout)
                if i != len(dim_mult) - 1 and j == num_res_blocks - 1:
                    self.input_blocks.append(_DownP(cout, self._down_padding))
                    shortcut_dims.append(cout)
                    scale /= 2.0
        self.middle_block = nn.ModuleList([
            _ResBlockP(cout, embed_dim, cout),
            _SpatialTransformerP(cout, cout // head_dim, context_dim),
            _TemporalTransformerP(cout, cout // head_dim),
            _ResBlockP(cout, embed_dim, cout)])
        self.output_blocks = nn.ModuleList()
        for i, (cin, cout) in enumerate(zip(dec_dims[:-1], dec_dims[1:])):
            for j in range(num_res_blocks + 1):
                block = nn.ModuleList([_ResBlockP(cin + shortcut_dims.pop(), embed_dim, cout)])
                if scale in self.attn_scales:
                    block.append(_SpatialTransformerP(cout, cout // head_dim, 1024))
                    block.append(_TemporalTransformerP(cout, cout // head_dim))
                cin = cout
                if i != len(dim_mult) - 1 and j == num_res_blocks:
                    block.append(_UpP(cout, self._up_crop))
                    scale *= 2.0
                self.output_blocks.append(block)
        self.out = _seq(nn.GroupNorm(32, cout), None, nn.Conv2d(cout, self.out_dim, 3, padding=1))
        nn.init.zeros_(self.out[-1].weight)

        self._levels = self._block_levels()
        self._packed = None
        self._epoch = 0

    def _stem_channels(self):
        return self.input_blocks[0][0].in_channels

    def _apply(self, fn, *a, **k):
        self.invalidate()
        return super()._apply(fn, *a, **k)

    def load_state_dict(self, *a, **k):
        self.invalidate()
        return super().load_state_dict(*a, **k)

    def invalidate(self):
        self._packed = None
        self._epoch = getattr(self, "_epoch", 0) + 1
        if self.precision == "calibrated" and not getattr(self, "calibration", None):
            self.precision = "high"
        if getattr(self, "_auto_cal_cfg", None) and self.precision == "high":
            self._auto_cal = self._auto_cal_cfg

    def _resblocks(self):
        for blk in list(self.input_blocks) + [self.middle_block] + list(self.output_blocks):
            if isinstance(blk, nn.ModuleList):
                for m in blk:
                    if isinstance(m, _ResBlockP):
                        yield m

    def _spatial(self):
        for blk in list(self.input_blocks) + [self.middle_block] + list(self.output_blocks):
            if isinstance(blk, nn.ModuleList):
                for m in blk:
                    if isinstance(m, _SpatialTransformerP):
                        yield m

    @torch.no_grad()
    def pack(self, device=None):
        P = self._pack(device)
        if self.precision == "calibrated":
            from .calibrate import load_calibrated
            load_calibrated(self, self.calibration)
        return P

    MIXED_LEVELS = {"enc": (0,), "mid": (), "dec": (0,), "tx": ()}
    MIXED_SINGLE_KINDS = ("ff1", "ff2", "q2")
    MIXED_EXTRA_KINDS = {1: ("conv2", "pin", "pout")}

    def _block_levels(self):
        lv, level = {}, 0
        nres, nmult = self.num_res_blocks, len(self.dim_mult)
        idx = 0
        lv["input_blocks.0"] = ("enc", 0)
        for i in range(nmult):
            for j in range(nres):
                idx += 1
                lv[f"input_blocks.{idx}"] = ("enc", level)
                if i != nmult - 1 and j == nres - 1:
                    idx += 1
                    lv[f"input_blocks.{idx}"] = ("enc", level)
                    level += 1
        lv["middle_block"] = ("mid", level)
        idx = 0
        for i in range(nmult):
            for j in range(nres + 1):
                lv[f"output_blocks.{idx}"] = ("dec", level)
                if i != nmult - 1 and j == nres:
                    level -= 1
                idx += 1
        return lv

    def _two_term(self, name, kind):
        if self.precision != "mixed":
            return self.precision == "high"
        levels = self.MIXED_LEVELS
        if name in ("kv_all", "out"):
            return 0 in levels["enc"] or 0 in levels["dec"]
        parts = name.split(".")
        side, level = self._levels[parts[0] if parts[0] == "middle_block" else ".".join(parts[:2])]
        if kind in self.MIXED_SINGLE_KINDS:
            return False
        if level in levels[side]:
            return True
        if level in levels.get("tx", ()) and kind in ("qkv", "o", "pin", "pout"):
            return True
        return side in ("enc", "dec") and kind in self.MIXED_EXTRA_KINDS.get(level, ())

    def _pack(self, device=None):
        dt = self.compute_dtype
        P = {}
        te = self.time_embed
        P["te0"] = (_f32(te[0].weight), _f32(te[0].bias))
        P["te2"] = (_f32(te[2].weight), _f32(te[2].bias))
        if self.use_fps_condition:
            fe = self.fps_embedding
            P["fe0"] = (_f32(fe[0].weight), _f32(fe[0].bias))
            P["fe2"] = (_f32(fe[2].weight), _f32(fe[2].bias))
        ws, bs, off = [], [], 0
        for rb in self._resblocks():
            ws.append(rb.emb_layers[1].weight)
            bs.append(rb.emb_layers[1].bias)
            rb._emb_off = off
            off += rb.cout
        P["emb_all"] = (_f32(torch.cat(ws, 0)), _f32(torch.cat(bs, 0)))
        ws, off = [], 0
        for st in self._spatial():
            a2 = st.transformer_blocks[0].attn2
            ws += [a2.to_k.weight, a2.to_v.weight]
            st._kv_off = off
            off += 2 * st.inner
        P["kv_all"] = pack_linear(torch.cat(ws, 0), dt, self._two_term("kv_all", "kv"))
        P["kv_width"] = off

        conv_in = self.input_blocks[0][0]
        cin0 = self._stem_channels()
        self._kpad_in = ((27 * cin0 + 63) // 64) * 64
        if cin0 % 64 == 0:
            P["conv_in"] = (pack_conv3x3(conv_in.weight, dt, self.precision == "high"), _f32(conv_in.bias))
        else:
            if cin0 > 16:
                raise NotImplementedError("stem conv input channels must be <= 16 or a multiple of 64")
            P["conv_in"] = (pack_small_conv3x3(conv_in.weight, self._kpad_in, dt, split=True), _f32(conv_in.bias))

        def pack_res(rb: _ResBlockP, name):
            d = {}
            on = lambda kind: self._two_term(name, kind)
            d["gn1"] = (_f32(rb.in_layers[0].weight), _f32(rb.in_layers[0].bias))
            d["conv1"] = (pack_conv3x3(rb.in_layers[2].weight, dt, on("conv1")), _f32(rb.in_layers[2].bias))
            d["gn2"] = (_f32(rb.out_layers[0].weight), _f32(rb.out_layers[0].bias))
            b2 = _f32(rb.out_layers[3].bias)
            if isinstance(rb.skip_connection, nn.Conv2d):
                wsk = rows_linear(rb.skip_connection.weight)
                w2 = _w16_cat([rows_conv3x3(rb.out_layers[3].weight), wsk] + ([wsk] if self._asplit else []), dt, on("conv2"))
                b2 = (b2 + _f32(rb.skip_connection.bias)).contiguous()
            else:
                w2 = pack_conv3x3(rb.out_layers[3].weight, dt, on("conv2"))
            d["conv2"] = (w2, b2)
            tc = rb.temopral_conv
            for i in (1, 2, 3, 4):
                sq = getattr(tc, f"conv{i}")
                d[f"tgn{i}"] = (_f32(sq[0].weight), _f32(sq[0].bias))
                d[f"tconv{i}"] = (pack_temporal(sq[-1].weight, dt, on("tconv")), _f32(sq[-1].bias))
            return d

        def pack_tblock(tb: _TBlockP, cross: bool, name):
            d = {}
            on = lambda kind: self._two_term(name, kind)
            for i in (1, 2, 3):
                n = getattr(tb, f"norm{i}")
                d[f"ln{i}"] = (_f32(n.weight), _f32(n.bias))
            a1, a2 = tb.attn1, tb.attn2
            d["qkv1"] = pack_linear(torch.cat([a1.to_q.weight, a1.to_k.weight, a1.to_v.weight], 0), dt, on("qkv"))
            d["o1"] = (pack_linear(a1.to_out[0].weight, dt, on("o")), _f32(a1.to_out[0].bias))
            if cross:
                d["q2"] = pack_linear(a2.to_q.weight, dt, on("q2"))
            else:
                d["qkv2"] = pack_linear(torch.cat([a2.to_q.weight, a2.to_k.weight, a2.to_v.weight], 0), dt, on("qkv"))
            d["o2"] = (pack_linear(a2.to_out[0].weight, dt, on("o")), _f32(a2.to_out[0].bias))
            d["ff1"] = pack_geglu(tb.ff.net[0].proj.weight, tb.ff.net[0].proj.bias, dt, on("ff1"))
            d["ff2"] = (pack_linear(tb.ff.net[2].weight, dt, on("ff2")), _f32(tb.ff.net[2].bias))
            return d

        def pack_tx(m, cross, name):
            d = {"gn": (_f32(m.norm.weight), _f32(m.norm.bias))}
            d["pin"] = (pack_linear(m.proj_in.weight, dt, self._two_term(name, "pin")), _f32(m.proj_in.bias))
            wpo = rows_linear(m.proj_out.weight)
            if self._asplit:
                wpo = torch.cat([wpo, wpo], 1)
            d["pout"] = (_w16(wpo, dt, self._two_term(name, "pout")), _f32(m.proj_out.bias))
            d["tb"] = pack_tblock(m.transformer_blocks[0], cross, name)
            return d

        for name, m in self.named_modules():
            if isinstance(m, _ResBlockP):
                P[name] = pack_res(m, name)
            elif isinstance(m, _SpatialTransformerP):
                P[name] = pack_tx(m, True, name)
            elif isinstance(m, _TemporalTransformerP):
                P[name] = pack_tx(m, False, name)
            elif isinstance(m, _DownP):
                P[name] = (pack_conv3x3(m.op.weight, dt, self._two_term(name, "resample")), _f32(m.op.bias))
            elif isinstance(m, _UpP):
                P[name] = (pack_conv3x3(m.conv.weight, dt, self._two_term(name, "resample")), _f32(m.conv.bias))
            m._pname = name
        P["head_gn"] = (_f32(self.out[0].weight), _f32(self.out[0].bias))
        P["head_conv"] = (pack_conv3x3(self.out[2].weight, dt, self._two_term("out", "head")), _f32(self.out[2].bias))
        eye = torch.eye(self.out_dim, dtype=torch.float32, device=self.out[2].weight.device)
        P["eye"] = eye.contiguous()
        self._packed = P
        return P

    def _linear(self, A, Wb, M, **kw):
        W, b = Wb if isinstance(Wb, tuple) else (Wb, None)
        kw["colstats"] = kw.get("colstats", False) and M >= ops.COLSTATS_MIN_ROWS
        return ops.backend().tapgemm(TapGemm(A=A, W=W, M=M, N=W.shape[0], C1=A.shape[1], bias=b, **kw))

    def _conv3x3(self, A, Wb, nimg, Hi, Wi, C1, stride=1, ups=0, pad=(1, 1), crop=0, **kw):
        W, b = Wb
        Hv, Wv = (Hi << ups) - 2 * crop, Wi << ups
        Ho = (Hv + 2 * pad[0] - 3) // stride + 1
        Wo = (Wv + 2 * pad[1] - 3) // stride + 1
        kw["colstats"] = kw.get("colstats", False) and nimg * Ho * Wo >= ops.COLSTATS_MIN_ROWS
        g = TapGemm(A=A, W=W, M=nimg * Ho * Wo, N=W.shape[0], C1=C1, mode=L.TAP_CONV3X3, taps=9,
                    Hi=Hi, Wi=Wi, Ho=Ho, Wo=Wo, stride=stride, pad_t=pad[0], pad_l=pad[1], ups=ups,
                    crop_t=crop, bias=b, **kw)
        return ops.backend().tapgemm(g), Ho, Wo

    def _resblock(self, rb: _ResBlockP, x1, x2, emb_all, B, F, H, W):
        be = ops.backend()
        dt = self.compute_dtype
        P = self._packed[rb._pname]
        S = H * W
        M = B * F * S
        has_skip = isinstance(rb.skip_connection, nn.Conv2d)
        a1, raw = be.groupnorm(x1, x2, B * F, S, 32, 1e-5, *P["gn1"], True,
                               ("split" if self._asplit else True) if has_skip else False, dt)
        c2 = 2 * rb.cin if self._asplit else rb.cin
        rowbias = emb_all[:, rb._emb_off: rb._emb_off + rb.cout]
        h, _, _ = self._conv3x3(a1, P["conv1"], B * F, H, W, rb.cin, rowbias=rowbias, rows_per_rb=F * S,
                                colstats=True)
        a2, _ = be.groupnorm(h, None, B * F, S, 32, 1e-5, *P["gn2"], True, False, dt)
        if has_skip:
            h, _, _ = self._conv3x3(a2, P["conv2"], B * F, H, W, rb.cout, A2=raw, C2=c2, colstats=True,
                                    alg_k=9 * rb.cout + rb.cin)
        else:
            assert x2 is None
            h, _, _ = self._conv3x3(a2, P["conv2"], B * F, H, W, rb.cout, residual=x1, colstats=True)
        t = h
        for i in (1, 2, 3, 4):
            a, _ = be.groupnorm(t, None, B, F * S, 32, 1e-5, *P[f"tgn{i}"], True, False, dt)
            Wt, bt = P[f"tconv{i}"]
            t = be.tapgemm(TapGemm(A=a, W=Wt, M=M, N=rb.cout, C1=rb.cout, mode=L.TAP_TEMPORAL3, taps=3,
                                   F=F, S=S, bias=bt, residual=h if i == 4 else None,
                                   colstats=M >= ops.COLSTATS_MIN_ROWS))
        return t

    def _adapt(self, T, slot, tok, M, geom=None):
        return tok

    def _attn_branch(self, T, i, tok, M, attn, geom=None):
        n = ops.backend().layernorm(tok, *T[f"ln{i}"], 1e-5, self.compute_dtype)
        return self._linear(attn(n), T[f"o{i}"], M, residual=self._adapt(T, f"a{i}", tok, M, geom))

    def _ff(self, T, tok, M, geom=None):
        dt = self.compute_dtype
        n = ops.backend().layernorm(tok, *T["ln3"], 1e-5, dt)
        g = self._linear(n, T["ff1"], M, out_dtype=dt, epilogue=L.EPI_GEGLU)
        return self._ff_out(g, T["ff2"], M, self._adapt(T, "ff", tok, M, geom))

    def _ff_out(self, g, ff2, M, tok):
        return self._linear(g, ff2, M, residual=tok, out_dtype=self.compute_dtype, split_out=self._asplit)

    def _spatial_tx(self, st: _SpatialTransformerP, x, kv_all, B, F, H, W, Lctx, kv_per_frame=False, share=1,
                    replicate=None):
        be = ops.backend()
        dt = self.compute_dtype
        P = self._packed[st._pname]
        T = P["tb"]
        N = H * W
        M = B * F * N
        d, heads = st.inner, st.heads
        Bp = B // share
        Mp = Bp * F * N
        scale = HEAD_DIM ** -0.5
        a, _ = be.groupnorm(x, None, Bp * F, N, 32, 1e-6, *P["gn"], False, False, dt)
        tok = self._linear(a, P["pin"], Mp)

        def self_attn(n):
            qkv = self._linear(n, T["qkv1"], Mp, out_dtype=dt)
            o = torch.empty((Mp, d), dtype=dt, device=qkv.device)
            ld = 3 * d
            be.attention(Attn(q=qkv, k=qkv[:, d:], v=qkv[:, 2 * d:], out=o, heads=heads, nq=N, nk=N, nbatch=Bp * F, inner=1,
                              q_s=(ld, N * ld, 0), k_s=(ld, N * ld, 0), v_s=(ld, N * ld, 0), o_s=(d, N * d, 0), scale=scale))
            return o

        tok = self._attn_branch(T, 1, tok, Mp, self_attn)
        n = be.layernorm(tok, *T["ln2"], 1e-5, dt)
        q = self._linear(n, T["q2"], Mp, out_dtype=dt)
        if share > 1:
            tok, q, x = replicate(tok), be.repeat_rows(q, share), replicate(x)
        o = torch.empty((M, d), dtype=dt, device=q.device)
        kw = kv_all.shape[1]
        k = kv_all[:, st._kv_off: st._kv_off + d]
        v = kv_all[:, st._kv_off + d: st._kv_off + 2 * d]
        kvs = (kw, F * Lctx * kw, Lctx * kw) if kv_per_frame else (kw, Lctx * kw, 0)
        be.attention(Attn(q=q, k=k, v=v, out=o, heads=heads, nq=N, nk=Lctx, nbatch=B * F, inner=F,
                          q_s=(d, F * N * d, N * d), k_s=kvs, v_s=kvs, o_s=(d, F * N * d, N * d), scale=scale))
        tok = self._linear(o, T["o2"], M, residual=self._adapt(T, "a2", tok, M))
        return self._linear(self._ff(T, tok, M), P["pout"], M, residual=x, colstats=True, alg_k=d)

    def _temporal_tx(self, tt: _TemporalTransformerP, x, B, F, H, W):
        be = ops.backend()
        dt = self.compute_dtype
        P = self._packed[tt._pname]
        S = H * W
        M = B * F * S
        d, heads = tt.inner, tt.heads
        a, _ = be.groupnorm(x, None, B, F * S, 32, 1e-6, *P["gn"], False, False, dt)
        tok = self._linear(a, P["pin"], M)
        scale = HEAD_DIM ** -0.5
        T, geom = P["tb"], (B, F, S)

        def self_attn(key):
            def attn(n):
                qkv = self._linear(n, T[key], M, out_dtype=dt)
                out = torch.empty((M, d), dtype=dt, device=qkv.device)
                ld = 3 * d
                s3 = (S * ld, F * S * ld, ld)
                return be.attention(Attn(q=qkv, k=qkv[:, d:], v=qkv[:, 2 * d:], out=out, heads=heads,
                                         nq=F, nk=F, nbatch=B * S, inner=S, q_s=s3, k_s=s3, v_s=s3,
                                         o_s=(S * d, F * S * d, d), scale=scale))
            return attn

        tok = self._attn_branch(T, 1, tok, M, self_attn("qkv1"), geom)
        tok = self._attn_branch(T, 2, tok, M, self_attn("qkv2"), geom)
        return self._linear(self._ff(T, tok, M, geom), P["pout"], M, residual=x, colstats=True, alg_k=d)

    def _prepare_units(self, shape, device, kwargs_list):
        if any(kw.get("y") is None for kw in kwargs_list):
            return None
        fps = None
        if self.use_fps_condition:
            have = [kw.get("fps") is not None for kw in kwargs_list]
            if any(have) and not all(have):
                return None
            if all(have):
                fps = torch.cat([kw["fps"].reshape(-1).to(device) for kw in kwargs_list], 0)
        ctx = torch.cat([kw["y"].to(device=device, dtype=torch.float32) for kw in kwargs_list], 0)
        return dict(extra=None, ctx=ctx, per_frame=False, fps=fps)

    @torch.no_grad()
    def _maybe_auto_calibrate(self, shape, device, kwargs, t_dtype=torch.long):
        pending = getattr(self, "_auto_cal", None)
        if not pending:
            return
        self._auto_cal = None
        path = pending if isinstance(pending, str) else None
        from . import calibrate as cal
        if path and os.path.exists(path):
            self.precision, self.calibration = "calibrated", path
            self.invalidate()
            return
        B, C, F, H, W = shape
        y0 = kwargs.get("y")
        x, t, y = cal.calibration_batch((C, F, H, W), device=device,
                                        context=tuple(y0.shape[1:]) if torch.is_tensor(y0) else (77, self.context_dim))
        n = x.shape[0]
        kw = {}
        for k, v in kwargs.items():
            if k == "y":
                kw[k] = y if torch.is_tensor(v) else v
            elif torch.is_tensor(v) and v.dim() >= 1 and v.shape[0] == B:
                kw[k] = v[:1].to(device).expand(n, *v.shape[1:]).contiguous()
            else:
                kw[k] = v
        if t_dtype is not None and t_dtype.is_floating_point:
            t = t.to(t_dtype)
        rep = cal.calibrate_single_pass(self, x, t, **kw)
        rep["auto"] = True
        if path:
            import torch.distributed as dist
            if not (dist.is_available() and dist.is_initialized()) or dist.get_rank() == 0:
                cal.save_calibrated(self, path)
                self.calibration = path

    @torch.no_grad()
    def forward_units(self, x, t, kwargs_list):
        G = len(kwargs_list)
        self._maybe_auto_calibrate(tuple(x.shape), x.device, kwargs_list[0], t.dtype)
        prep = self._prepare_units(tuple(x.shape), x.device, kwargs_list)
        if prep is None:
            return tuple(self.forward(x, t, **kw) for kw in kwargs_list)
        xs = x.float().repeat(G, 1, 1, 1, 1)
        if prep["extra"] is not None:
            xs = torch.cat([xs, prep["extra"]], 1)
        out = self._trunk(xs, t.repeat(G), prep["ctx"], prep["fps"], ctx_per_frame=prep["per_frame"],
                          shared_groups=self.shared_prefix_groups(prep, G, x.shape[0]), body_kw=prep.get("body"))
        return tuple(out.chunk(G, 0))

    @staticmethod
    def shared_prefix_groups(prep, G, B):
        if G <= 1 or os.environ.get("VGEN_SHARED_PREFIX", "1") == "0":
            return 1
        ex, fps = prep["extra"], prep["fps"]
        if ex is not None and not all(torch.equal(ex[:B], ex[g * B:(g + 1) * B]) for g in range(1, G)):
            return 1
        if fps is not None and not all(torch.equal(fps[:B], fps[g * B:(g + 1) * B]) for g in range(1, G)):
            return 1
        return G

    @torch.no_grad()
    def forward(self, x, t, y=None, fps=None, masked=None, video_mask=None, focus_present_mask=None,
                prob_focus_present=0., mask_last_frame_num=0, **kwargs):
        self._maybe_auto_calibrate(tuple(x.shape), x.device, dict(y=y, fps=fps), t.dtype)
        ctx = y if y is not None else self.zero_y.repeat(x.shape[0], 1, 1)[:, :1, :]
        return self._trunk(x, t, ctx, fps)

    def _embed_rows(self, tf, fpsf=None):
        be = ops.backend()
        P = self._packed
        dev = P["te0"][0].device

        def mlp(val, w0, w2, add=None):
            s = be.timestep_embedding(val.to(device=dev, dtype=torch.float32).reshape(-1).contiguous(), self.dim,
                                      torch.float32)
            return be.linear_f32(be.linear_f32(s, *w0), *w2, act_in=1, add=add)

        e = mlp(tf, P["te0"], P["te2"])
        if self.use_fps_condition and fpsf is not None:
            e = mlp(fpsf, P["fe0"], P["fe2"], add=e)
        return be.linear_f32(e, *P["emb_all"], act_in=1)

    def _embed(self, t, fps, B, dev):
        return self._embed_rows(t, fps)

    @torch.no_grad()
    def time_embedding_table(self, n, device=None):
        if self._packed is None:
            self.pack()
        P = self._packed
        key = ("emb_tab", n)
        if key not in P:
            P[key] = self._embed_rows(torch.arange(n, dtype=torch.float32))
        return P[key]

    def _context_kv(self, ctx, dev):
        be = ops.backend()
        dt = self.compute_dtype
        nctx, Lctx = ctx.shape[0], ctx.shape[1]
        ctx16 = be.act_cast(ctx.to(device=dev, dtype=torch.float32).reshape(nctx * Lctx, -1).contiguous(), 0, dt)
        return self._linear(ctx16, self._packed["kv_all"], nctx * Lctx, out_dtype=dt)

    def _trunk(self, x, t, ctx, fps=None, ctx_per_frame=False, shared_groups=1, body_kw=None):
        if self._packed is None:
            self.pack()
        B, C, F, H, W = x.shape
        assert ctx.shape[0] == (B * F if ctx_per_frame else B), (tuple(ctx.shape), B, F, ctx_per_frame)
        emb_all = self._embed(t, fps, B, x.device)
        kv_all = self._context_kv(ctx, x.device)
        return self._body(x, emb_all, kv_all, ctx.shape[1], ctx_per_frame, shared_groups=shared_groups, **(body_kw or {}))

    def _body(self, x, emb_all, kv_all, Lctx, ctx_per_frame=False, out=None, shared_groups=1):
        be = ops.backend()
        dt = self.compute_dtype
        P = self._packed
        B, C, F, H, W = x.shape
        assert C == self._stem_channels()
        dev = x.device
        x = x.float().contiguous()
        G = int(shared_groups)
        first = self.input_blocks[1] if len(self.input_blocks) > 1 else None
        if G > 1 and not (B % G == 0 and isinstance(first, nn.ModuleList) and isinstance(first[0], _ResBlockP)):
            G = 1
        Bp = B // G

        if C % 64 == 0:
            raise NotImplementedError("wide input stems are not on the t2v path")
        sFHW = F * H * W
        col = be.im2col3x3_small(x[:Bp], Bp * F, F, C, H, W, (C * sFHW, H * W, sFHW, W, 1), self._kpad_in, dt, split=True)
        h = self._linear(col, P["conv_in"], Bp * F * H * W, colstats=True)

        def run(mod, h, x2, H, W, nB=B):
            if isinstance(mod, _ResBlockP):
                return self._resblock(mod, h, x2, emb_all, nB, F, H, W), H, W
            assert x2 is None
            if isinstance(mod, _SpatialTransformerP):
                return self._spatial_tx(mod, h, kv_all, nB, F, H, W, Lctx, ctx_per_frame), H, W
            if isinstance(mod, _TemporalTransformerP):
                return self._temporal_tx(mod, h, nB, F, H, W), H, W
            if isinstance(mod, _DownP):
                a = be.act_cast(h, 0, dt)
                o, Ho, Wo = self._conv3x3(a, P[mod._pname], nB * F, H, W, h.shape[1], stride=2, pad=mod.pad,
                                          colstats=True)
                return o, Ho, Wo
            if isinstance(mod, _UpP):
                a = be.act_cast(h, 0, dt)
                o, Ho, Wo = self._conv3x3(a, P[mod._pname], nB * F, H, W, h.shape[1], ups=1, crop=mod.crop,
                                          colstats=True)
                return o, Ho, Wo
            raise TypeError(type(mod))

        def replicate(t):
            if G == 1:
                return t
            r = be.repeat_rows(t, G)
            cs = ops.colstats_of(t, t.shape[0])
            if cs is not None and t.shape[0] % ops.CS_ROWS == 0:
                r.vgen_cs = be.repeat_rows(cs, G)
            return r

        xs = []
        h, _, _ = run(self.input_blocks[0][1], h, None, H, W, Bp)
        xs.append((replicate(h), H, W))
        rest = list(self.input_blocks)[1:]
        if G > 1:
            h, H, W = run(first[0], h, None, H, W, Bp)
            tail = list(first)[1:]
            if tail and isinstance(tail[0], _SpatialTransformerP):
                h = self._spatial_tx(tail[0], h, kv_all, B, F, H, W, Lctx, ctx_per_frame, share=G, replicate=replicate)
                tail = tail[1:]
            else:
                h = replicate(h)
            for m in tail:
                h, H, W = run(m, h, None, H, W)
            xs.append((h, H, W))
            rest = rest[1:]
        for blk in rest:
            mods = list(blk) if isinstance(blk, nn.ModuleList) else [blk]
            for m in mods:
                h, H, W = run(m, h, None, H, W)
            xs.append((h, H, W))
        for m in self.middle_block:
            h, H, W = run(m, h, None, H, W)
        for bnum, blk in enumerate(self.output_blocks):
            skip, Hs, Ws = xs.pop()
            assert (Hs, Ws) == (H, W)
            if self._freeu is not None and bnum < len(self._freeu):
                boost, lf = self._freeu[bnum]
                h = be.scale_channels(h, 0, h.shape[1] // 2, boost)
                skip = be.lowfreq_filter(skip, B * F, H, W, lf)
            x2 = skip
            for m in blk:
                h, H, W = run(m, h, x2, H, W)
                x2 = None
        a, _ = be.groupnorm(h, None, B * F, H * W, 32, 1e-5, *P["head_gn"], True, False, dt)
        o, _, _ = self._conv3x3(a, P["head_conv"], B * F, H, W, h.shape[1])
        if out is None:
            out = torch.empty((B, self.out_dim, F, H, W), dtype=torch.float32, device=dev)
        assert out.shape == (B, self.out_dim, F, H, W) and out.dtype == torch.float32 and out.is_contiguous()
        od = self.out_dim
        sFHW = F * H * W
        be.pointwise_small(o, B * F, F, od, H, W, (sFHW * od, H * W * od, 1, W * od, od),
                           P["eye"], None, od, out, (od * sFHW, H * W, sFHW, W, 1))
        return out


class UNetSD_SR600(UNetSD_T2VBase):
    _down_padding = (2, 1)
    _up_crop = 1
    _freeu = ((1.1, 0.6), (1.2, 0.4))

    def __init__(self, in_dim=7, dim=512, y_dim=512, context_dim=512, out_dim=6, dim_mult=[1, 2, 3, 4],
                 num_heads=None, head_dim=64, num_res_blocks=3, attn_scales=[1 / 2, 1 / 4, 1 / 8],
                 use_scale_shift_norm=True, dropout=0.1, temporal_attn_times=1, temporal_attention=True,
                 use_checkpoint=False, use_image_dataset=False, use_sim_mask=False, inpainting=True,
                 compute_dtype=None, **kwargs):
        super().__init__(in_dim=in_dim, dim=dim, y_dim=y_dim, context_dim=context_dim, out_dim=out_dim,
                         dim_mult=dim_mult, num_heads=num_heads, head_dim=head_dim,
                         num_res_blocks=num_res_blocks, attn_scales=attn_scales, dropout=dropout,
                         temporal_attn_times=temporal_attn_times, temporal_attention=temporal_attention,
                         use_checkpoint=use_checkpoint, use_image_dataset=use_image_dataset,
                         use_sim_mask=use_sim_mask, inpainting=inpainting, use_fps_condition=False,
                         compute_dtype=compute_dtype, precision=kwargs.get("precision"),
                         calibration=kwargs.get("calibration"))

    @torch.no_grad()
    def forward(self, x, t, y, x_lr=None, fps=None, video_mask=None, focus_present_mask=None,
                prob_focus_present=0., mask_last_frame_num=0, **kwargs):
        return super().forward(x, t, y=y)
```

Baseline: 32.82.

## Fuse split-K reduction of conv/linear GEMMs into the following groupnorm read

```diff
diff --git a/include/vgen_hip.h b/include/vgen_hip.h
--- a/include/vgen_hip.h
+++ b/include/vgen_hip.h
@@ -34,6 +34,14 @@
                       const float* gamma, const float* beta, int32_t silu,
                       void* y, void* raw, int32_t raw_split, int32_t dtype,
                       float* ws, size_t ws_bytes, void* stream);
+
+int vgen_groupnorm_path(int32_t C1, int32_t C2, int64_t nb, int64_t S, int32_t groups);
+int vgen_groupnorm_partials(const float* planes, int32_t splitk, int64_t plane_stride, int32_t C1,
+                            const float* bias, const float* rowbias, int64_t rowbias_ld, int64_t rows_per_rb,
+                            const float* residual, int64_t ldr, float* x_out, const float* x2, int32_t C2,
+                            int64_t nb, int64_t S, int32_t groups, float eps, const float* gamma,
+                            const float* beta, int32_t silu, void* y, void* raw, int32_t raw_split,
+                            int32_t dtype, float* ws, size_t ws_bytes, void* stream);
 
 int vgen_embed_tokens(const int64_t* tokens, int64_t rows, int32_t L, int32_t d, int32_t vocab,
                       const float* table, const float* pos, float* out, void* stream);
@@ -83,6 +91,9 @@
 size_t vgen_tapgemm_ws_bytes(const vgen_tapgemm_args* args);
 int vgen_tapgemm(const vgen_tapgemm_args* args, void* stream);
 
+int vgen_tapgemm_deferred(const vgen_tapgemm_args* args, int32_t* splitk_used, void* stream);
+int vgen_splitk_materialize(const vgen_tapgemm_args* args, int32_t splitk, void* stream);
+
 int vgen_tapgemm_query_plan(const vgen_tapgemm_args* args, int32_t* out3);
 int vgen_tapgemm_set_plans(const int64_t* rows, int32_t n);
 
diff --git a/vgen_amd/csrc/norms.hip b/vgen_amd/csrc/norms.hip
--- a/vgen_amd/csrc/norms.hip
+++ b/vgen_amd/csrc/norms.hip
@@ -417,6 +417,58 @@
   }
 }
 
+struct GnPart {
+  const float* ws;
+  int splitk;
+  int64_t plane;
+  const float* bias;
+  const float* rowbias;
+  int64_t rowbias_ld, rows_per_rb;
+  const float* residual;
+  int64_t ldr;
+  float* x_out;
+};
+
+struct GnPartLane {
+  f32x2 bias, rb;
+  bool has_rb_lane;
+};
+
+__device__ __forceinline__ GnPartLane gn_part_lane(const GnPart& pp, int64_t row0, int64_t S, int c) {
+  GnPartLane l;
+  l.bias = pp.bias ? *(const f32x2*)(pp.bias + c) : f32x2{0.f, 0.f};
+  l.rb = f32x2{0.f, 0.f};
+  l.has_rb_lane = false;
+  if (pp.rowbias) {
+    const int64_t b0 = row0 / pp.rows_per_rb;
+    if ((row0 + S - 1) / pp.rows_per_rb == b0) {
+      l.rb = *(const f32x2*)(pp.rowbias + b0 * pp.rowbias_ld + c);
+      l.has_rb_lane = true;
+    }
+  }
+  return l;
+}
+
+template <int SK>
+__device__ __forceinline__ f32x2 gn_part_value(const GnPart& pp, const GnPartLane& l, int64_t m, int c, int N) {
+  const float* p = pp.ws + m * N + c;
+  f32x2 v = {0.f, 0.f};
+  if constexpr (SK > 0) {
+    f32x2 t[SK];
+#pragma unroll
+    for (int s = 0; s < SK; ++s) t[s] = *(const f32x2*)(p + s * pp.plane);
+#pragma unroll
+    for (int s = 0; s < SK; ++s) v += t[s];
+  } else {
+    for (int s = 0; s < pp.splitk; ++s) v += *(const f32x2*)(p + s * pp.plane);
+  }
+  if (pp.bias) v += l.bias;
+  if (pp.rowbias) v += l.has_rb_lane ? l.rb : *(const f32x2*)(pp.rowbias + (m / pp.rows_per_rb) * pp.rowbias_ld + c);
+  if (pp.residual) v += *(const f32x2*)(pp.residual + m * pp.ldr + c);
+  if (pp.x_out) *(f32x2*)(pp.x_out + m * N + c) = v;
+  return v;
+}
+
 constexpr int GNF_THREADS = 512;
 constexpr int GNF_LDS_FLOATS = 24576;
 
@@ -432,11 +484,11 @@
   return t;
 }
 
-template <typename T>
+template <typename T, int SK>
 __global__ __launch_bounds__(GNF_THREADS) void gn_fused_kernel(
     const float* __restrict__ x1, int C1, const float* __restrict__ x2, int C2, int64_t S, int groups,
     float eps, const float* __restrict__ gamma, const float* __restrict__ beta, int silu,
-    uint16_t* __restrict__ y, uint16_t* __restrict__ raw, int raw_lo) {
+    uint16_t* __restrict__ y, uint16_t* __restrict__ raw, int raw_lo, const GnPart pp) {
   extern __shared__ __attribute__((aligned(16))) float gnf_stage[];
   __shared__ float red[GNF_THREADS / 64];
   const int C = C1 + C2;
@@ -450,14 +502,24 @@
   const int c = blockIdx.x * cpg + 2 * i;
   const int64_t row0 = (int64_t)blockIdx.y * S;
   const bool from1 = c < C1;
-  const float* src = from1 ? x1 + row0 * C1 + c : x2 + row0 * C2 + (c - C1);
+  const float* src = from1 ? (SK == 0 ? x1 + row0 * C1 + c : nullptr) : x2 + row0 * C2 + (c - C1);
   const int64_t lds = from1 ? C1 : C2;
   const int nit = active ? (int)((S - r0 + rpi - 1) / rpi) : 0;
   f32x2* const st = (f32x2*)gnf_stage + r0 * I + i;
   const int sstep = rpi * I;
 
   float a = 0.f;
-  {
+  if (SK != 0 && from1) {
+    if (active) {
+      const GnPartLane l = gn_part_lane(pp, row0, S, c);
+#pragma unroll 4
+      for (int k = 0; k < nit; ++k) {
+        const f32x2 v = gn_part_value<SK>(pp, l, row0 + r0 + (int64_t)k * rpi, c, C1);
+        st[k * sstep] = v;
+        a += v.x + v.y;
+      }
+    }
+  } else {
     const float* p = src + (int64_t)r0 * lds;
     const int64_t step = (int64_t)rpi * lds;
 #pragma unroll 8
@@ -511,11 +573,11 @@
   return t;
 }
 
-template <typename T>
+template <typename T, int SK>
 __global__ __launch_bounds__(GNR_THREADS) void gn_regs_kernel(
     const float* __restrict__ x1, int C1, const float* __restrict__ x2, int C2, int64_t S, int groups,
     float eps, const float* __restrict__ gamma, const float* __restrict__ beta, int silu,
-    uint16_t* __restrict__ y, uint16_t* __restrict__ raw, int raw_lo) {
+    uint16_t* __restrict__ y, uint16_t* __restrict__ raw, int raw_lo, const GnPart pp) {
   __shared__ float red[GNR_THREADS / 64];
   const int C = C1 + C2;
   const int cpg = C / groups;
@@ -528,19 +590,29 @@
   const int c = blockIdx.x * cpg + 2 * i;
   const int64_t row0 = (int64_t)blockIdx.y * S;
   const bool from1 = c < C1;
-  const float* src = from1 ? x1 + row0 * C1 + c : x2 + row0 * C2 + (c - C1);
+  const float* src = from1 ? (SK == 0 ? x1 + row0 * C1 + c : nullptr) : x2 + row0 * C2 + (c - C1);
   const int64_t lds = from1 ? C1 : C2;
   const int nit = active ? (int)((S - r0 + rpi - 1) / rpi) : 0;
 
   f32x2 v[GNR_NIT];
   float a = 0.f;
   {
-    const float* p = src + (int64_t)r0 * lds;
-    const int64_t step = (int64_t)rpi * lds;
-#pragma unroll
-    for (int k = 0; k < GNR_NIT; ++k) {
-      v[k] = f32x2{0.f, 0.f};
-      if (k < nit) v[k] = *(const f32x2*)(p + k * step);
+    if (SK != 0 && from1) {
+      GnPartLane l = {};
+      if (active) l = gn_part_lane(pp, row0, S, c);
+#pragma unroll
+      for (int k = 0; k < GNR_NIT; ++k) {
+        v[k] = f32x2{0.f, 0.f};
+        if (k < nit) v[k] = gn_part_value<SK>(pp, l, row0 + r0 + (int64_t)k * rpi, c, C1);
+      }
+    } else {
+      const float* p = src + (int64_t)r0 * lds;
+      const int64_t step = (int64_t)rpi * lds;
+#pragma unroll
+      for (int k = 0; k < GNR_NIT; ++k) {
+        v[k] = f32x2{0.f, 0.f};
+        if (k < nit) v[k] = *(const f32x2*)(p + k * step);
+      }
     }
 #pragma unroll
     for (int k = 0; k < GNR_NIT; ++k) a += v[k].x + v[k].y;
@@ -743,11 +815,63 @@
   return (size_t)(nb * ns * GN_G * 3 + nb * 3072 * 2) * sizeof(float);
 }
 
+static int gn_path(int C1, int C2, int64_t nb, int64_t S, int groups, bool colstats) {
+  const int C = C1 + C2;
+  const int cpg = C / groups;
+  {
+    static const int env_max = getenv("VGEN_GN_FUSED_MAX_MB") ? atoi(getenv("VGEN_GN_FUSED_MAX_MB")) : -1;
+    const int64_t fused_max = (int64_t)(env_max >= 0 ? env_max : (cpg >= 16 ? 96 : 24)) << 20;
+    if (nb * S * C * 4 <= fused_max && cpg % 2 == 0 && C1 % 2 == 0 && cpg / 2 <= GNF_THREADS && S * cpg <= GNF_LDS_FLOATS)
+      return 1;
+  }
+  {
+    static const int regs_on = getenv("VGEN_GN_REGS") ? atoi(getenv("VGEN_GN_REGS")) : 1;
+    const int I = cpg / 2;
+    if (regs_on && !colstats && cpg % 2 == 0 && C1 % 2 == 0 && I > 0 && I <= GNR_THREADS &&
+        (S + (GNR_THREADS / I) - 1) / (GNR_THREADS / I) <= GNR_NIT && nb * groups <= 1024 && S * cpg > GNF_LDS_FLOATS)
+      return 2;
+  }
+  return 0;
+}
+
+template <typename T, int SK>
+static int launch_gn_single(int path, const float* x1, int C1, const float* x2, int C2, int64_t nb, int64_t S, int groups,
+                            float eps, const float* gamma, const float* beta, int silu, void* y, void* raw, int raw_lo,
+                            const GnPart& pp, hipStream_t s) {
+  const dim3 fgrid((unsigned)groups, (unsigned)nb);
+  if (path == 1) {
+    const size_t lds = (size_t)S * ((C1 + C2) / groups) * sizeof(float);
+    static bool done[VGEN_MAX_DEVICES] = {false};
+    if (vgen_lds_optin((const void*)gn_fused_kernel<T, SK>, GNF_LDS_FLOATS * 4, done, "groupnorm")) return VGEN_E_BADARG;
+    hipLaunchKernelGGL((gn_fused_kernel<T, SK>), fgrid, dim3(GNF_THREADS), lds, s, x1, C1, x2, C2, S, groups, eps, gamma, beta,
+                       silu, (uint16_t*)y, (uint16_t*)raw, raw_lo, pp);
+    return vgen_check_launch("gn_fused");
+  }
+  hipLaunchKernelGGL((gn_regs_kernel<T, SK>), fgrid, dim3(GNR_THREADS), 0, s, x1, C1, x2, C2, S, groups, eps, gamma, beta, silu,
+                     (uint16_t*)y, (uint16_t*)raw, raw_lo, pp);
+  return vgen_check_launch("gn_regs");
+}
+
+template <typename T>
+static int dispatch_gn_single(int path, const float* x1, int C1, const float* x2, int C2, int64_t nb, int64_t S, int groups,
+                              float eps, const float* gamma, const float* beta, int silu, void* y, void* raw, int raw_lo,
+                              const GnPart* pp, hipStream_t s) {
+#define VGEN_GN_SINGLE(SK, P) launch_gn_single<T, SK>(path, x1, C1, x2, C2, nb, S, groups, eps, gamma, beta, silu, y, raw, raw_lo, P, s)
+  if (pp == nullptr) return VGEN_GN_SINGLE(0, GnPart{});
+  switch (pp->splitk) {
+    case 2: return VGEN_GN_SINGLE(2, *pp);
+    case 3: return VGEN_GN_SINGLE(3, *pp);
+    case 6: return VGEN_GN_SINGLE(6, *pp);
+    default: return VGEN_GN_SINGLE(-1, *pp);
+  }
+#undef VGEN_GN_SINGLE
+}
+
 static int groupnorm_impl(const float* x1, int32_t C1, const float* cs1, const float* x2, int32_t C2,
                           const float* cs2, int64_t nb, int64_t S, int32_t groups, float eps,
                           const float* gamma, const float* beta, int32_t silu, void* y,
                           void* raw, int32_t raw_split, int32_t dtype, float* ws, size_t ws_bytes,
-                          void* stream) {
+                          void* stream, const GnPart* pp = nullptr) {
   const int C = C1 + C2;
   const int raw_lo = (raw != nullptr && raw_split) ? C : 0;
   VGEN_REQUIRE(dtype == VGEN_BF16 || dtype == VGEN_F16, "groupnorm: dtype");
@@ -766,43 +890,16 @@
     return VGEN_E_WORKSPACE;
   }
   hipStream_t s = (hipStream_t)stream;
-  {
-    static const int env_max = getenv("VGEN_GN_FUSED_MAX_MB") ? atoi(getenv("VGEN_GN_FUSED_MAX_MB")) : -1;
-    const int64_t fused_max = (int64_t)(env_max >= 0 ? env_max : (C / groups >= 16 ? 96 : 24)) << 20;
-    const int cpg = C / groups;
-    if (nb * S * C * 4 <= fused_max && cpg % 2 == 0 && C1 % 2 == 0 && cpg / 2 <= GNF_THREADS && S * cpg <= GNF_LDS_FLOATS) {
-      const size_t lds = (size_t)S * cpg * sizeof(float);
-      static bool done_bf16[VGEN_MAX_DEVICES] = {false}, done_f16[VGEN_MAX_DEVICES] = {false};
-      if (vgen_lds_optin((const void*)gn_fused_kernel<BF16>, GNF_LDS_FLOATS * 4, done_bf16, "groupnorm") ||
-          vgen_lds_optin((const void*)gn_fused_kernel<F16>, GNF_LDS_FLOATS * 4, done_f16, "groupnorm"))
-        return VGEN_E_BADARG;
-      dim3 fgrid((unsigned)groups, (unsigned)nb);
-      if (dtype == VGEN_BF16) {
-        hipLaunchKernelGGL(gn_fused_kernel<BF16>, fgrid, dim3(GNF_THREADS), lds, s, x1, C1, x2, C2, S, groups, eps,
-                           gamma, beta, silu, (uint16_t*)y, (uint16_t*)raw, raw_lo);
-      } else {
-        hipLaunchKernelGGL(gn_fused_kernel<F16>, fgrid, dim3(GNF_THREADS), lds, s, x1, C1, x2, C2, S, groups, eps,
-                           gamma, beta, silu, (uint16_t*)y, (uint16_t*)raw, raw_lo);
-      }
-      return vgen_check_launch("gn_fused");
-    }
-  }
-  {
-    static const int regs_on = getenv("VGEN_GN_REGS") ? atoi(getenv("VGEN_GN_REGS")) : 1;
-    const int cpg = C / groups;
-    const int I = cpg / 2;
-    if (regs_on && cs1 == nullptr && cpg % 2 == 0 && C1 % 2 == 0 && I > 0 && I <= GNR_THREADS &&
-        (S + (GNR_THREADS / I) - 1) / (GNR_THREADS / I) <= GNR_NIT && nb * groups <= 1024 && S * cpg > GNF_LDS_FLOATS) {
-      dim3 fgrid((unsigned)groups, (unsigned)nb);
-      if (dtype == VGEN_BF16) {
-        hipLaunchKernelGGL(gn_regs_kernel<BF16>, fgrid, dim3(GNR_THREADS), 0, s, x1, C1, x2, C2, S, groups, eps, gamma, beta,
-                           silu, (uint16_t*)y, (uint16_t*)raw, raw_lo);
-      } else {
-        hipLaunchKernelGGL(gn_regs_kernel<F16>, fgrid, dim3(GNR_THREADS), 0, s, x1, C1, x2, C2, S, groups, eps, gamma, beta,
-                           silu, (uint16_t*)y, (uint16_t*)raw, raw_lo);
-      }
-      return vgen_check_launch("gn_regs");
-    }
+  const int path = gn_path(C1, C2, nb, S, groups, cs1 != nullptr);
+  if (pp != nullptr && path == 0) {
+    vgen_set_error("groupnorm_partials: [%lld x %lld x %d] takes the streaming pipeline, which reads a materialised tensor "
+                   "(vgen_groupnorm_path)", (long long)nb, (long long)S, C);
+    return VGEN_E_UNSUPPORTED;
+  }
+  if (path != 0) {
+    return dtype == VGEN_BF16
+               ? dispatch_gn_single<BF16>(path, x1, C1, x2, C2, nb, S, groups, eps, gamma, beta, silu, y, raw, raw_lo, pp, s)
+               : dispatch_gn_single<F16>(path, x1, C1, x2, C2, nb, S, groups, eps, gamma, beta, silu, y, raw, raw_lo, pp, s);
   }
   const int nslots = C / 4;
   const int rpb = nslots <= GN_THREADS ? GN_THREADS / nslots : 1;
@@ -862,6 +959,31 @@
                         ws, ws_bytes, stream);
 }
 
+extern "C" int vgen_groupnorm_path(int32_t C1, int32_t C2, int64_t nb, int64_t S, int32_t groups) {
+  if (groups <= 0 || C1 <= 0 || C2 < 0 || (C1 + C2) % groups != 0 || nb <= 0 || S <= 0) return 0;
+  return gn_path(C1, C2, nb, S, groups, false);
+}
+
+extern "C" int vgen_groupnorm_partials(const float* planes, int32_t splitk, int64_t plane_stride, int32_t C1,
+                                       const float* bias, const float* rowbias, int64_t rowbias_ld, int64_t rows_per_rb,
+                                       const float* residual, int64_t ldr, float* x_out, const float* x2, int32_t C2,
+                                       int64_t nb, int64_t S, int32_t groups, float eps, const float* gamma,
+                                       const float* beta, int32_t silu, void* y, void* raw, int32_t raw_split,
+                                       int32_t dtype, float* ws, size_t ws_bytes, void* stream) {
+  VGEN_REQUIRE(planes != nullptr && vgen_aligned16(planes) && splitk >= 2 && splitk <= 64,
+               "groupnorm_partials: planes / split count %d", (int)splitk);
+  VGEN_REQUIRE(nb > 0 && S > 0 && C1 > 0 && plane_stride >= nb * S * C1 && plane_stride % 4 == 0,
+               "groupnorm_partials: plane stride %lld", (long long)plane_stride);
+  VGEN_REQUIRE(vgen_aligned16(bias) && vgen_aligned16(residual) && vgen_aligned16(x_out) &&
+                   (residual == nullptr || (ldr >= C1 && ldr % 4 == 0)),
+               "groupnorm_partials: bias / residual / x_out alignment, ldr");
+  VGEN_REQUIRE(rowbias == nullptr || (vgen_aligned16(rowbias) && rows_per_rb > 0 && rowbias_ld >= C1 && rowbias_ld % 4 == 0),
+               "groupnorm_partials: rowbias alignment / rowbias_ld / rows_per_rb");
+  const GnPart pp = {planes, splitk, plane_stride, bias, rowbias, rowbias_ld, rows_per_rb, residual, ldr, x_out};
+  return groupnorm_impl(nullptr, C1, nullptr, x2, C2, nullptr, nb, S, groups, eps, gamma, beta, silu, y, raw, raw_split,
+                        dtype, ws, ws_bytes, stream, &pp);
+}
+
 extern "C" int vgen_layernorm(const float* x, int64_t M, int32_t d, float eps, const float* gamma,
                               const float* beta, void* y, int32_t dtype, void* stream) {
   VGEN_REQUIRE(dtype == VGEN_BF16 || dtype == VGEN_F16 || dtype == VGEN_F32, "layernorm: dtype");
diff --git a/vgen_amd/csrc/tapgemm.hip b/vgen_amd/csrc/tapgemm.hip
--- a/vgen_amd/csrc/tapgemm.hip
+++ b/vgen_amd/csrc/tapgemm.hip
@@ -736,7 +736,7 @@
 constexpr int STAGGER_MIN_ROUNDS = 2;
 
 template <typename T, int S, int BN, bool DW>
-int launch(const vgen_tapgemm_args& a, int splitk, hipStream_t stream) {
+int launch(const vgen_tapgemm_args& a, int splitk, hipStream_t stream, int* pending) {
   constexpr ShapeDesc d = kShapes[S];
   constexpr int BM = d.bm, BK = d.bk, WM = d.wm, WN = d.wn, STAGES = 3;
   constexpr int BPC = d.bpc;
@@ -786,6 +786,10 @@
                      ablate, stagger, cus * BPC);
   int rc = vgen_check_launch("tapgemm");
   if (rc || splitk == 1) return rc;
+  if (pending) {
+    *pending = splitk;
+    return 0;
+  }
   const int64_t threads = a.M * (tap_n_out(a) / 4);
   hipLaunchKernelGGL((splitk_reduce_kernel<T>), dim3((unsigned)((threads + 255) / 256)), dim3(256), 0,
                      stream, a, splitk, (const float*)a.ws);
@@ -793,26 +797,27 @@
 }
 
 template <typename T, int S, bool DW>
-int launch_bn(const vgen_tapgemm_args& a, const Plan& pl, hipStream_t s) {
+int launch_bn(const vgen_tapgemm_args& a, const Plan& pl, hipStream_t s, int* pending) {
   switch (pl.bn) {
-    case 128: return launch<T, S, 128, DW>(a, pl.splitk, s);
-    case 160: return launch<T, S, 160, DW>(a, pl.splitk, s);
-    default: return launch<T, S, 64, DW>(a, pl.splitk, s);
+    case 128: return launch<T, S, 128, DW>(a, pl.splitk, s, pending);
+    case 160: return launch<T, S, 160, DW>(a, pl.splitk, s, pending);
+    default: return launch<T, S, 64, DW>(a, pl.splitk, s, pending);
   }
 }
 
 template <typename T>
-int dispatch(const vgen_tapgemm_args& a, hipStream_t s) {
+int dispatch(const vgen_tapgemm_args& a, hipStream_t s, int* pending) {
   const Plan pl = full_plan(a);
   if (pl.shape == SHAPE_PANEL) return vgen_panel_launch(a, s);
   if (a.dualw)
-    return pl.shape == SHAPE_PP128 ? launch_bn<T, SHAPE_PP128, true>(a, pl, s) : launch_bn<T, SHAPE_PP, true>(a, pl, s);
+    return pl.shape == SHAPE_PP128 ? launch_bn<T, SHAPE_PP128, true>(a, pl, s, pending)
+                                   : launch_bn<T, SHAPE_PP, true>(a, pl, s, pending);
   switch (pl.shape) {
-    case SHAPE_PP: return launch_bn<T, SHAPE_PP, false>(a, pl, s);
-    case SHAPE_PP128: return launch_bn<T, SHAPE_PP128, false>(a, pl, s);
-    case SHAPE_PP256: return launch<T, SHAPE_PP256, 256, false>(a, pl.splitk, s);
-    case SHAPE_Q128: return launch_bn<T, SHAPE_Q128, false>(a, pl, s);
-    default: return launch_bn<T, SHAPE_DUAL, false>(a, pl, s);
+    case SHAPE_PP: return launch_bn<T, SHAPE_PP, false>(a, pl, s, pending);
+    case SHAPE_PP128: return launch_bn<T, SHAPE_PP128, false>(a, pl, s, pending);
+    case SHAPE_PP256: return launch<T, SHAPE_PP256, 256, false>(a, pl.splitk, s, pending);
+    case SHAPE_Q128: return launch_bn<T, SHAPE_Q128, false>(a, pl, s, pending);
+    default: return launch_bn<T, SHAPE_DUAL, false>(a, pl, s, pending);
   }
 }
 
@@ -825,5 +830,52 @@
   }
   if (const int rc = vgen_tapgemm_validate(*args)) return rc;
   hipStream_t s = (hipStream_t)stream;
-  return args->dtype == VGEN_BF16 ? dispatch<BF16>(*args, s) : dispatch<F16>(*args, s);
-}
+  return args->dtype == VGEN_BF16 ? dispatch<BF16>(*args, s, nullptr) : dispatch<F16>(*args, s, nullptr);
+}
+
+static int deferrable(const vgen_tapgemm_args& a, const char* who) {
+  if (a.epilogue != VGEN_EPI_NONE || a.out_dtype != VGEN_F32 || a.colstats != nullptr) {
+    vgen_set_error("%s: a pending split needs an fp32 output without GEGLU or column statistics", who);
+    return VGEN_E_BADARG;
+  }
+  return 0;
+}
+
+extern "C" int vgen_tapgemm_deferred(const vgen_tapgemm_args* args, int32_t* splitk_used, void* stream) {
+  if (!args || !splitk_used) {
+    vgen_set_error("tapgemm_deferred: null args");
+    return VGEN_E_BADARG;
+  }
+  if (const int rc = vgen_tapgemm_validate(*args)) return rc;
+  if (const int rc = deferrable(*args, "tapgemm_deferred")) return rc;
+  hipStream_t s = (hipStream_t)stream;
+  int pending = 1;
+  const int rc = args->dtype == VGEN_BF16 ? dispatch<BF16>(*args, s, &pending) : dispatch<F16>(*args, s, &pending);
+  *splitk_used = pending;
+  return rc;
+}
+
+extern "C" int vgen_splitk_materialize(const vgen_tapgemm_args* args, int32_t splitk, void* stream) {
+  if (!args) {
+    vgen_set_error("splitk_materialize: null args");
+    return VGEN_E_BADARG;
+  }
+  if (const int rc = vgen_tapgemm_validate(*args)) return rc;
+  if (const int rc = deferrable(*args, "splitk_materialize")) return rc;
+  const vgen_tapgemm_args& a = *args;
+  if (splitk < 2 || !tap_vec(a)) {
+    vgen_set_error("splitk_materialize: nothing pending (split %d) or an epilogue that is no whole 4-vector", (int)splitk);
+    return VGEN_E_BADARG;
+  }
+  if (a.ws == nullptr || a.ws_bytes < (size_t)splitk * a.M * a.N * sizeof(float)) {
+    vgen_set_error("splitk_materialize: workspace %zu < %zu", a.ws_bytes, (size_t)splitk * a.M * a.N * sizeof(float));
+    return VGEN_E_WORKSPACE;
+  }
+  const int64_t threads = a.M * (tap_n_out(a) / 4);
+  const dim3 grid((unsigned)((threads + 255) / 256));
+  if (a.dtype == VGEN_BF16)
+    hipLaunchKernelGGL((splitk_reduce_kernel<BF16>), grid, dim3(256), 0, (hipStream_t)stream, a, (int)splitk, (const float*)a.ws);
+  else
+    hipLaunchKernelGGL((splitk_reduce_kernel<F16>), grid, dim3(256), 0, (hipStream_t)stream, a, (int)splitk, (const float*)a.ws);
+  return vgen_check_launch("tapgemm(splitk reduce)");
+}
diff --git a/vgen_amd/lib.py b/vgen_amd/lib.py
--- a/vgen_amd/lib.py
+++ b/vgen_amd/lib.py
@@ -57,9 +57,14 @@
                                  _vp, _vp, _i32, _i32, _vp, _sz, _vp]),
     "vgen_groupnorm_cs": (C.c_int, [_vp, _i32, _vp, _vp, _i32, _vp, _i64, _i64, _i32, _f32, _vp, _vp, _i32,
                                     _vp, _vp, _i32, _i32, _vp, _sz, _vp]),
+    "vgen_groupnorm_path": (C.c_int, [_i32, _i32, _i64, _i64, _i32]),
+    "vgen_groupnorm_partials": (C.c_int, [_vp, _i32, _i64, _i32, _vp, _vp, _i64, _i64, _vp, _i64, _vp, _vp, _i32,
+                                          _i64, _i64, _i32, _f32, _vp, _vp, _i32, _vp, _vp, _i32, _i32, _vp, _sz, _vp]),
     "vgen_layernorm": (C.c_int, [_vp, _i64, _i32, _f32, _vp, _vp, _vp, _i32, _vp]),
     "vgen_tapgemm_ws_bytes": (_sz, [C.POINTER(TapGemmArgs)]),
     "vgen_tapgemm": (C.c_int, [C.POINTER(TapGemmArgs), _vp]),
+    "vgen_tapgemm_deferred": (C.c_int, [C.POINTER(TapGemmArgs), _vp, _vp]),
+    "vgen_splitk_materialize": (C.c_int, [C.POINTER(TapGemmArgs), _i32, _vp]),
     "vgen_tapgemm_query_plan": (C.c_int, [C.POINTER(TapGemmArgs), _vp]),
     "vgen_tapgemm_set_plans": (C.c_int, [_vp, _i32]),
     "vgen_attention": (C.c_int, [C.POINTER(AttnArgs), _vp]),
diff --git a/vgen_amd/ops.py b/vgen_amd/ops.py
--- a/vgen_amd/ops.py
+++ b/vgen_amd/ops.py
@@ -25,6 +25,28 @@
     if cs.shape != ((rows + CS_ROWS - 1) // CS_ROWS, 2, t.shape[1]) or t.shape[0] != rows:
         return None
     return cs
+
+
+SPLITK_DEFER = None
+SPLITK_DEFER_DEFAULT = "0"
+
+
+def splitk_defer_on():
+    if SPLITK_DEFER is not None:
+        return bool(SPLITK_DEFER)
+    return os.environ.get("VGEN_SPLITK_DEFER", SPLITK_DEFER_DEFAULT) != "0"
+
+
+class PendingSplit:
+    __slots__ = ("args", "splitk", "ws", "bias", "rowbias", "residual", "keep")
+
+    def __init__(self, args, splitk, ws, bias, rowbias, residual, keep):
+        self.args, self.splitk, self.ws, self.bias, self.rowbias, self.residual, self.keep = \
+            args, splitk, ws, bias, rowbias, residual, keep
+
+
+def pending_of(t):
+    return None if t is None else getattr(t, "vgen_pending", None)
 
 
 def drop_colstats(t):
@@ -65,6 +87,7 @@
     split_out: bool = False
     ws: Optional[torch.Tensor] = None
     alg_k: int = 0
+    defer = False
 
 
 @dataclass
@@ -147,10 +170,37 @@
                 self.rec.append((self.name, self.e0, self.e1, self.work, self.meta, self.extra))
             return False
 
+    def materialize(self, t):
+        p = pending_of(t)
+        if p is not None:
+            del t.vgen_pending
+            _lib.check(self.lib.vgen_splitk_materialize(C.byref(p.args), p.splitk, self._stream(t)), "vgen_splitk_materialize")
+        return t
+
+    def _ready(self, *ts):
+        for t in ts:
+            if t is None:
+                continue
+            if getattr(t, "vgen_pending", None) is not None:
+                self.materialize(t)
+            elif getattr(t, "vgen_never_written", False):
+                raise _lib.VgenHipError("this tensor was produced with TapGemm.defer=True (its GroupNorm is its only reader) "
+                                        "and was never written; produce it with defer=\"keep\"")
+
     def groupnorm(self, x1, x2, nb, S, groups, eps, gamma, beta, silu, want_raw, dt):
         C1 = x1.shape[1]
         C2 = 0 if x2 is None else x2.shape[1]
         rows = nb * S
+        pend = pending_of(x1)
+        if pend is not None and self.lib.vgen_groupnorm_path(C1, C2, nb, S, groups) != 0:
+            assert pend.args.M == rows and pend.args.N == C1
+            del x1.vgen_pending
+            if not pend.keep:
+                x1.vgen_never_written = True
+            self._ready(x2)
+        else:
+            pend = None
+            self._ready(x1, x2)
         assert x1.dtype == torch.float32 and x1.is_contiguous() and x1.shape[0] == rows
         assert x2 is None or (x2.dtype == torch.float32 and x2.is_contiguous() and x2.shape[0] == rows)
         y = torch.empty((rows, C1 + C2), dtype=dt, device=x1.device)
@@ -163,7 +213,13 @@
         use_cs = S % CS_ROWS == 0 and cs1 is not None and (x2 is None or cs2 is not None)
         nbytes_moved = rows * (C1 + C2) * ((4 if use_cs else 8) + 2 + ((4 if rsplit else 2) if want_raw else 0))
         with self._Prof("groupnorm", nbytes_moved, (nb, S, C1 + C2, int(bool(want_raw)) + int(rsplit))):
-            if use_cs:
+            if pend is not None:
+                a = pend.args
+                rc = self.lib.vgen_groupnorm_partials(
+                    a.ws, pend.splitk, rows * C1, C1, a.bias, a.rowbias, a.rowbias_ld, a.rows_per_rb, a.residual, a.ldr,
+                    _ptr(x1) if pend.keep else None, _ptr(x2), C2, nb, S, groups, float(eps), _ptr(gamma), _ptr(beta),
+                    int(bool(silu)), _ptr(y), _ptr(raw), int(rsplit), _ENUM[dt], _ptr(ws), nbytes, self._stream(x1))
+            elif use_cs:
                 rc = self.lib.vgen_groupnorm_cs(_ptr(x1), C1, _ptr(cs1), _ptr(x2), C2, _ptr(cs2), nb, S, groups,
                                                 float(eps), _ptr(gamma), _ptr(beta), int(bool(silu)), _ptr(y),
                                                 _ptr(raw), int(rsplit), _ENUM[dt], _ptr(ws), nbytes, self._stream(x1))
@@ -175,6 +231,7 @@
         return y, raw
 
     def layernorm(self, x, gamma, beta, eps, dt):
+        self._ready(x)
         assert x.dtype == torch.float32 and x.is_contiguous() and x.dim() == 2
         y = torch.empty(x.shape, dtype=dt, device=x.device)
         with self._Prof("layernorm", x.numel() * 6, tuple(x.shape)):
@@ -190,7 +247,11 @@
         return tuple(pl)
 
     def tapgemm(self, g: TapGemm):
+        self._ready(g.residual, g.rowbias)
         a, out, cs, A, W, dw, K, n_out, _keep = self._tapgemm_args(g)
+        for stale in ("vgen_pending", "vgen_never_written"):
+            if hasattr(out, stale):
+                delattr(out, stale)
         meta = (g.mode, g.M, g.N, K, g.epilogue, str(g.out_dtype) + ("+dw" if dw is not None else ""))
         if KERNEL_PROFILE is not None and PROFILE_PLANS:
             pl = (C.c_int32 * 3)()
@@ -202,11 +263,19 @@
                   float(g.M) * n_out * ((4 if g.out_dtype == torch.float32 else 2) + (4 if g.residual is not None else 0)))
         k_alg = g.alg_k or K
         assert 0 < k_alg <= K
+        defer = bool(g.defer) and splitk_defer_on() and cs is None and g.out_dtype == torch.float32 and \
+            g.epilogue == _lib.EPI_NONE and out.stride(0) == g.N and a.ws
+        sk = C.c_int32(1)
         with self._Prof("tapgemm", 2.0 * g.M * g.N * k_alg, meta, (abytes, 2.0 * g.M * g.N * K * (2 if dw is not None else 1))):
-            rc = self.lib.vgen_tapgemm(C.byref(a), self._stream(A))
+            if defer:
+                rc = self.lib.vgen_tapgemm_deferred(C.byref(a), C.byref(sk), self._stream(A))
+            else:
+                rc = self.lib.vgen_tapgemm(C.byref(a), self._stream(A))
         _lib.check(rc, "vgen_tapgemm")
         if cs is not None:
             out.vgen_cs = cs
+        if sk.value > 1:
+            out.vgen_pending = PendingSplit(a, sk.value, _keep, g.bias, g.rowbias, g.residual, g.defer == "keep")
         return out
 
     _PLAN_ONLY = 0x1000
@@ -305,6 +374,7 @@
         return g.out
 
     def softmax_rows(self, S, cols, scale, dt, out=None):
+        self._ready(S)
         S = _mat(S, "S")
         rows = S.shape[0]
         if out is None:
@@ -316,6 +386,7 @@
         return out
 
     def act_cast(self, x, act, dt):
+        self._ready(x)
         assert x.dtype == torch.float32 and x.is_contiguous()
         y = torch.empty(x.shape, dtype=dt, device=x.device)
         with self._Prof("act_cast", x.numel() * 6, (x.numel(),)):
@@ -324,6 +395,7 @@
         return y
 
     def cast_split(self, x, dt, out=None, col=0, lo_off=None):
+        self._ready(x)
         assert x.dtype == torch.float32 and x.dim() == 2 and x.stride(1) == 1
         M, Cc = x.shape
         lo_off = Cc if lo_off is None else lo_off
@@ -337,6 +409,7 @@
         return out
 
     def adapter(self, x, Wd, Wu, bu, hb, rows_per_hb, h, out=None):
+        self._ready(x, hb)
         x = _mat(x, "x")
         hb = _mat(hb, "hb")
         M, d = x.shape
@@ -394,6 +467,7 @@
         return out
 
     def dwconv_relu(self, x, n, H, W, w, k, dt, pool=False):
+        self._ready(x)
         x = _mat(x, "x")
         Cp = x.shape[1]
         assert x.dtype == torch.float32 and x.shape[0] == n * H * W
@@ -528,6 +602,7 @@
         return out
 
     def pointwise_small(self, src, nimg, Fi, Cin, H, W, s_strides, Wm, b, Cout, dst, d_strides):
+        self._ready(src)
         assert src.dtype == torch.float32 and dst.dtype == torch.float32
         assert Wm.dtype == torch.float32 and Wm.is_contiguous()
         rc = self.lib.vgen_pointwise_small(_ptr(src), nimg, Fi, Cin, H, W, *s_strides, _ptr(Wm),
@@ -589,6 +664,7 @@
         _lib.check(rc, "vgen_cfg_ddim_step_units")
 
     def lowfreq_filter(self, x, nimg, H, W, scale):
+        self._ready(x)
         assert x.dtype == torch.float32 and x.is_contiguous() and x.shape[0] == nimg * H * W
         C_ = x.shape[1]
         y = torch.empty_like(x)
@@ -599,6 +675,7 @@
         return y
 
     def scale_channels(self, x, c0, c1, s):
+        self._ready(x)
         assert x.dtype == torch.float32 and x.is_contiguous() and x.dim() == 2
         rc = self.lib.vgen_scale_channels(_ptr(x), x.shape[0], x.shape[1], c0, c1, float(s), self._stream(x))
         _lib.check(rc, "vgen_scale_channels")
@@ -606,6 +683,7 @@
         return x
 
     def frames_u8(self, x, mean, std):
+        self._ready(x)
         x = _mat(x, "x")
         assert x.dtype == torch.float32 and mean.dtype == torch.float32 and std.dtype == torch.float32
         out = torch.empty((x.shape[0], x.shape[1]), dtype=torch.uint8, device=x.device)
@@ -634,6 +712,7 @@
         return x0, eps
 
     def lincomb4(self, a, b, c, d, ca, cb, cc, cd):
+        self._ready(a, b, c, d)
         for t in (a, b, c, d):
             assert t is None or (t.dtype == torch.float32 and t.is_contiguous())
         out = torch.empty_like(a)
@@ -643,6 +722,7 @@
         return out
 
     def repeat_rows(self, t, G):
+        self._ready(t)
         assert t.is_contiguous() and (t.numel() * t.element_size()) % 16 == 0
         out = torch.empty((G * t.shape[0],) + tuple(t.shape[1:]), dtype=t.dtype, device=t.device)
         rc = self.lib.vgen_repeat_rows(_ptr(t), t.numel() * t.element_size(), int(G), _ptr(out), self._stream(t))
diff --git a/vgen_amd/unet.py b/vgen_amd/unet.py
--- a/vgen_amd/unet.py
+++ b/vgen_amd/unet.py
@@ -479,7 +479,10 @@
     def _linear(self, A, Wb, M, **kw):
         W, b = Wb if isinstance(Wb, tuple) else (Wb, None)
         kw["colstats"] = kw.get("colstats", False) and M >= ops.COLSTATS_MIN_ROWS
-        return ops.backend().tapgemm(TapGemm(A=A, W=W, M=M, N=W.shape[0], C1=A.shape[1], bias=b, **kw))
+        defer = kw.pop("defer", False)
+        g = TapGemm(A=A, W=W, M=M, N=W.shape[0], C1=A.shape[1], bias=b, **kw)
+        g.defer = defer
+        return ops.backend().tapgemm(g)
 
     def _conv3x3(self, A, Wb, nimg, Hi, Wi, C1, stride=1, ups=0, pad=(1, 1), crop=0, **kw):
         W, b = Wb
@@ -487,9 +490,11 @@
         Ho = (Hv + 2 * pad[0] - 3) // stride + 1
         Wo = (Wv + 2 * pad[1] - 3) // stride + 1
         kw["colstats"] = kw.get("colstats", False) and nimg * Ho * Wo >= ops.COLSTATS_MIN_ROWS
+        defer = kw.pop("defer", False)
         g = TapGemm(A=A, W=W, M=nimg * Ho * Wo, N=W.shape[0], C1=C1, mode=L.TAP_CONV3X3, taps=9,
                     Hi=Hi, Wi=Wi, Ho=Ho, Wo=Wo, stride=stride, pad_t=pad[0], pad_l=pad[1], ups=ups,
                     crop_t=crop, bias=b, **kw)
+        g.defer = defer
         return ops.backend().tapgemm(g), Ho, Wo
 
     def _resblock(self, rb: _ResBlockP, x1, x2, emb_all, B, F, H, W):
@@ -504,21 +509,23 @@
         c2 = 2 * rb.cin if self._asplit else rb.cin
         rowbias = emb_all[:, rb._emb_off: rb._emb_off + rb.cout]
         h, _, _ = self._conv3x3(a1, P["conv1"], B * F, H, W, rb.cin, rowbias=rowbias, rows_per_rb=F * S,
-                                colstats=True)
+                                colstats=True, defer=True)
         a2, _ = be.groupnorm(h, None, B * F, S, 32, 1e-5, *P["gn2"], True, False, dt)
         if has_skip:
             h, _, _ = self._conv3x3(a2, P["conv2"], B * F, H, W, rb.cout, A2=raw, C2=c2, colstats=True,
-                                    alg_k=9 * rb.cout + rb.cin)
+                                    alg_k=9 * rb.cout + rb.cin, defer="keep")
         else:
             assert x2 is None
-            h, _, _ = self._conv3x3(a2, P["conv2"], B * F, H, W, rb.cout, residual=x1, colstats=True)
+            h, _, _ = self._conv3x3(a2, P["conv2"], B * F, H, W, rb.cout, residual=x1, colstats=True, defer="keep")
         t = h
         for i in (1, 2, 3, 4):
             a, _ = be.groupnorm(t, None, B, F * S, 32, 1e-5, *P[f"tgn{i}"], True, False, dt)
             Wt, bt = P[f"tconv{i}"]
-            t = be.tapgemm(TapGemm(A=a, W=Wt, M=M, N=rb.cout, C1=rb.cout, mode=L.TAP_TEMPORAL3, taps=3,
-                                   F=F, S=S, bias=bt, residual=h if i == 4 else None,
-                                   colstats=M >= ops.COLSTATS_MIN_ROWS))
+            g = TapGemm(A=a, W=Wt, M=M, N=rb.cout, C1=rb.cout, mode=L.TAP_TEMPORAL3, taps=3,
+                        F=F, S=S, bias=bt, residual=h if i == 4 else None,
+                        colstats=M >= ops.COLSTATS_MIN_ROWS)
+            g.defer = "keep" if i == 4 else True
+            t = be.tapgemm(g)
         return t
 
     def _adapt(self, T, slot, tok, M, geom=None):
@@ -573,7 +580,7 @@
         be.attention(Attn(q=q, k=k, v=v, out=o, heads=heads, nq=N, nk=Lctx, nbatch=B * F, inner=F,
                           q_s=(d, F * N * d, N * d), k_s=kvs, v_s=kvs, o_s=(d, F * N * d, N * d), scale=scale))
         tok = self._linear(o, T["o2"], M, residual=self._adapt(T, "a2", tok, M))
-        return self._linear(self._ff(T, tok, M), P["pout"], M, residual=x, colstats=True, alg_k=d)
+        return self._linear(self._ff(T, tok, M), P["pout"], M, residual=x, colstats=True, alg_k=d, defer="keep")
 
     def _temporal_tx(self, tt: _TemporalTransformerP, x, B, F, H, W):
         be = ops.backend()
@@ -600,7 +607,7 @@
 
         tok = self._attn_branch(T, 1, tok, M, self_attn("qkv1"), geom)
         tok = self._attn_branch(T, 2, tok, M, self_attn("qkv2"), geom)
-        return self._linear(self._ff(T, tok, M, geom), P["pout"], M, residual=x, colstats=True, alg_k=d)
+        return self._linear(self._ff(T, tok, M, geom), P["pout"], M, residual=x, colstats=True, alg_k=d, defer="keep")
 
     def _prepare_units(self, shape, device, kwargs_list):
         if any(kw.get("y") is None for kw in kwargs_list):
@@ -757,7 +764,7 @@
             if isinstance(mod, _DownP):
                 a = be.act_cast(h, 0, dt)
                 o, Ho, Wo = self._conv3x3(a, P[mod._pname], nB * F, H, W, h.shape[1], stride=2, pad=mod.pad,
-                                          colstats=True)
+                                          colstats=True, defer="keep")
                 return o, Ho, Wo
             if isinstance(mod, _UpP):
                 a = be.act_cast(h, 0, dt)
```

Result: no change. 32.74 (-0.3%).
